# fishaudio/fish-diffusion

Measured on NVIDIA H100. Metric: mel_frames_per_sec_100step_ddpm, higher is better.
Workload: dtype f32 (3x fp16 split-product wgmma, fp32 accumulate)

## Files before the change

### fish_diffusion_b200/_native.py

```python
from __future__ import annotations

import ctypes
import os
import threading
from ctypes import POINTER, c_char_p, c_float, c_int, c_longlong, c_size_t, c_ubyte, c_ulonglong, c_void_p

import torch

_HERE = os.path.dirname(os.path.abspath(__file__))
LIB_PATH = os.environ.get("FISHDIFF_B200_LIB") or os.path.join(_HERE, "libfishdiff_b200.so")

PREC_F16, PREC_BF16 = 0, 1
PREC_SINGLE = 0x10
BACKEND_TC, BACKEND_SIMT = 0, 1
ACT_NONE, ACT_RELU, ACT_LRELU = 0, 1, 2
ABI_VERSION = 3


class NativeError(RuntimeError):
    pass


class ConvDesc(ctypes.Structure):
    _fields_ = [
        ("in_planes", c_void_p), ("w_planes", c_void_p), ("bias", c_void_p), ("addend", c_void_p),
        ("res_f32", c_void_p), ("res_planes", c_void_p), ("row_mask", c_void_p), ("out_f32", c_void_p),
        ("out_planes", c_void_p),
        ("B", c_int), ("T", c_int), ("Cin", c_int), ("N", c_int), ("ntaps", c_int), ("shifts", c_int * 16),
        ("w_inv_scale", c_float), ("post_scale", c_float), ("planes_scale", c_float), ("act_slope", c_float),
        ("out_accum", c_int), ("act", c_int), ("prec", c_int), ("backend", c_int),
    ]


class GemmDesc(ctypes.Structure):
    _fields_ = [
        ("src", c_void_p * 2), ("src_C", c_int * 2), ("w", c_void_p), ("n_total", c_int), ("k_total", c_int),
        ("w_kshift", c_int), ("B", c_int), ("T", c_int), ("num_seg", c_int), ("seg_src", c_int * 16),
        ("seg_shift", c_int * 16), ("seg_coff", c_int * 16), ("seg_klen", c_int * 16),
        ("bias", c_void_p), ("addend", c_void_p), ("res_f32", c_void_p), ("res_planes", c_void_p),
        ("row_mask", c_void_p), ("out_f32", c_void_p), ("out_planes", c_void_p),
        ("w_inv_scale", c_float), ("res_scale", c_float), ("post_scale", c_float), ("planes_scale", c_float),
        ("act_slope", c_float), ("out_accum", c_int), ("act", c_int), ("prec", c_int), ("backend", c_int),
        ("bias_bstride", c_int),
        ("gate_y", c_void_p), ("gate_cs", c_void_p), ("gate_cs_edge", c_void_p), ("gate_cs_scale", c_float),
        ("gate_tile", c_int), ("gate_dil", c_int),
    ]


class ResPairDesc(ctypes.Structure):
    _fields_ = [
        ("in_planes", c_void_p), ("w1", c_void_p), ("w2", c_void_p), ("b1", c_void_p), ("b2", c_void_p),
        ("out_planes", c_void_p),
        ("B", c_int), ("T", c_int), ("C", c_int), ("k1", c_int), ("d1", c_int), ("k2", c_int),
        ("w1_inv_scale", c_float), ("w2_inv_scale", c_float), ("in_slope", c_float), ("out_slope", c_float),
        ("planes_scale", c_float), ("prec", c_int), ("kmask1", c_ulonglong), ("kmask2", c_ulonglong),
    ]


class WaveNetFwdDesc(ctypes.Structure):
    _fields_ = [
        ("x_planes", c_void_p), ("cond_planes", c_void_p), ("steps", c_void_p), ("x_mask", c_void_p), ("out", c_void_p),
        ("w_in", c_void_p), ("b_in", c_void_p), ("w_in_inv", c_float),
        ("mlp_w0", c_void_p), ("mlp_b0", c_void_p), ("mlp_w1", c_void_p), ("mlp_b1", c_void_p),
        ("wd", c_void_p), ("bd", c_void_p), ("w1p_f32", c_void_p), ("bias_sum", c_void_p),
        ("w1", c_void_p), ("w1_lstride", c_longlong), ("w2", c_void_p), ("w2_lstride", c_longlong),
        ("b2", c_void_p), ("b2_lstride", c_longlong),
        ("w_skip", c_void_p), ("b_skip", c_void_p), ("w_skip_inv", c_float),
        ("w_out", c_void_p), ("b_out", c_void_p), ("w_out_inv", c_float),
        ("w1_inv", c_float * 64), ("w2_inv", c_float * 64), ("dilation", c_int * 64),
        ("xr", c_void_p), ("z", c_void_p), ("skip_planes", c_void_p), ("skip_f32", c_void_p),
        ("s", c_void_p), ("mlp_ws", c_void_p), ("gb", c_void_p), ("gb_ws", c_void_p),
        ("B", c_int), ("T", c_int), ("M", c_int), ("C", c_int), ("E", c_int), ("L", c_int), ("Bs", c_int),
        ("gate_tile", c_int), ("prec", c_int), ("backend", c_int),
        ("cond_proj", c_void_p),
    ]


class WaveNetBwdDesc(ctypes.Structure):
    _fields_ = [
        ("x_planes", c_void_p), ("y_planes", c_void_p), ("z_planes", c_void_p), ("cond_planes", c_void_p),
        ("dx_next", c_void_p), ("dskip", c_void_p), ("w2t", c_void_p), ("w1t", c_void_p), ("wct", c_void_p),
        ("w2t_inv", c_float), ("w1t_inv", c_float), ("wct_inv", c_float),
        ("dx_out", c_void_p), ("dx_f32", c_void_p), ("d_cond", c_void_p), ("gw1", c_void_p), ("gw2", c_void_p),
        ("cs_dy", c_void_p), ("cs_edge", c_void_p), ("cs_dx", c_void_p), ("dy", c_void_p),
        ("part1", c_void_p), ("part2", c_void_p), ("splits1", c_int), ("splits2", c_int),
        ("B", c_int), ("T", c_int), ("C", c_int), ("E", c_int), ("dilation", c_int), ("gate_tile", c_int),
        ("inv_S", c_float), ("prec", c_int), ("backend", c_int),
    ]


class WgradDesc(ctypes.Structure):
    _fields_ = [
        ("row_src", c_void_p * 2), ("row_C", c_int * 2), ("col_src", c_void_p * 2), ("col_C", c_int * 2),
        ("num_row_seg", c_int), ("row_seg_src", c_int * 2), ("row_seg_coff", c_int * 2), ("row_seg_width", c_int * 2),
        ("num_col_seg", c_int), ("col_seg_src", c_int * 8), ("col_seg_shift", c_int * 8), ("col_seg_coff", c_int * 8),
        ("col_seg_width", c_int * 8),
        ("B", c_int), ("T", c_int), ("splits", c_int), ("part", c_void_p), ("acc_scale", c_float), ("prec", c_int),
        ("backend", c_int),
    ]


_SIGS = {
    "fd_gemm_cl_fwd": (c_int, [POINTER(GemmDesc), c_void_p]),
    "fd_wavenet_pack_layers": (c_int, [c_void_p] * 10 + [c_int, c_int, c_int, c_int, c_int, c_void_p]),
    "fd_wgrad_cl": (c_int, [POINTER(WgradDesc), c_void_p]),
    "fd_wavenet_block_bwd": (c_int, [POINTER(WaveNetBwdDesc), c_void_p]),
    "fd_wavenet_block_fwd_train": (c_int, [c_void_p] * 10 + [c_int, c_void_p, c_void_p, c_void_p, c_float] +
                                   [c_int] * 6 + [c_float, c_float, c_int, c_int, c_int, c_void_p]),
    "fd_wavenet_gate_bias_from_d": (c_int, [c_void_p] * 6 + [c_int, c_int, c_int, c_int, c_void_p]),
    "fd_relu_bwd": (c_int, [c_void_p] * 3 + [c_longlong, c_float, c_int, c_void_p]),
    "fd_lrelu_bwd": (c_int, [c_void_p] * 5 + [c_longlong, c_float, c_float, c_int, c_void_p]),
    "fd_colsum": (c_int, [c_void_p] * 3 + [c_int, c_int, c_int, c_float, c_int, c_void_p]),
    "fd_reduce_batch": (c_int, [c_void_p, c_void_p, c_int, c_longlong, c_float, c_void_p]),
    "fd_abi_version": (c_int, []),
    "fd_last_error": (c_char_p, []),
    "fd_set_device": (None, [c_int]),
    "fd_launch_count": (c_longlong, []),
    "fd_tc_supported_linear": (c_int, [c_int, c_int, c_int]),
    "fd_prof_enable": (None, [c_int]),
    "fd_prof_collect": (c_int, [POINTER(ctypes.c_double), POINTER(c_longlong), c_int]),
    "fd_split_ncw": (c_int, [c_void_p, c_void_p, c_void_p, c_int, c_int, c_int, c_int, c_void_p]),
    "fd_split_nwc": (c_int, [c_void_p, c_void_p, c_void_p, c_int, c_int, c_int, c_float, c_int, c_void_p]),
    "fd_mrf_finish": (c_int, [POINTER(c_void_p), c_int, c_void_p, c_longlong, c_float, c_float, c_float, c_int, c_void_p]),
    "fd_transpose_nwc_to_ncw": (c_int, [c_void_p, c_void_p, c_int, c_int, c_int, c_void_p]),
    "fd_transpose_ncw_to_nwc": (c_int, [c_void_p, c_void_p, c_int, c_int, c_int, c_void_p]),
    "fd_pack_weight": (c_int, [c_void_p, c_void_p, c_longlong, c_float, c_int, c_void_p]),
    "fd_wavenet_step_mlp": (c_int, [c_void_p] * 7 + [c_int, c_int, c_void_p]),
    "fd_wavenet_gate_bias": (c_int, [c_void_p] * 9 + [c_int, c_int, c_int, c_int, c_void_p]),
    "fd_wavenet_block_fwd": (c_int, [c_void_p] * 8 + [c_int, c_void_p, c_void_p, c_void_p, c_float] + [c_int] * 6 +
                             [c_float, c_float, c_int, c_int, c_int, c_void_p]),
    "fd_wavenet_fwd": (c_int, [POINTER(WaveNetFwdDesc), c_void_p]),
    "fd_wavenet_cond_proj": (c_int, [POINTER(WaveNetFwdDesc), c_void_p]),
    "fd_conv_cl_fwd": (c_int, [POINTER(ConvDesc), c_void_p]),
    "fd_respair_supported": (c_int, [c_int, c_int, c_int, c_int]),
    "fd_respair_fwd": (c_int, [POINTER(ResPairDesc), c_void_p]),
    "fd_ddpm_step": (c_int, [c_void_p] * 5 + [c_longlong] + [c_float] * 7 + [c_ulonglong, c_ulonglong, c_ulonglong, c_int,
                                                                               c_void_p]),
    "fd_lincomb": (c_int, [c_void_p, c_void_p, POINTER(c_void_p), POINTER(c_float), c_int, c_longlong, c_int, c_void_p]),
    "fd_affine_cl": (c_int, [c_void_p] * 4 + [c_int, c_longlong, c_int, c_void_p]),
    "fd_q_sample": (c_int, [c_void_p] * 5 + [c_int, c_longlong, c_void_p]),
    "fd_randn": (c_int, [c_void_p, c_longlong, c_ulonglong, c_ulonglong, c_ulonglong, c_void_p]),
    "fd_sinegen_ws_bytes": (c_size_t, [c_int, c_longlong]),
    "fd_sinegen_fwd": (c_int, [c_void_p] * 7 + [c_int, c_int, c_int, c_int, c_float, c_float, c_float, c_ulonglong,
                                                c_void_p]),
    "fd_source_conv_fwd": (c_int, [c_void_p] * 4 + [c_int, c_longlong, c_int, c_int, c_int, c_int, c_void_p]),
    "fd_conv_post_fwd": (c_int, [c_void_p] * 4 + [c_int, c_longlong, c_int, c_int, c_int, c_void_p]),
    "fd_reflect_pad_split": (c_int, [c_void_p, c_void_p, c_int, c_longlong, c_int, c_int, c_void_p]),
    "fd_stft_mag_fwd": (c_int, [c_void_p] * 3 + [c_int, c_longlong, c_int, c_int, c_int, c_int, c_float, c_float, c_int,
                                                 c_int, c_void_p]),
    "fd_stft_mag_eps_fwd": (c_int, [c_void_p] * 3 + [c_int, c_longlong, c_int, c_int, c_int, c_int, c_float, c_float, c_float,
                                                     c_int, c_int, c_void_p]),
    "fd_log_clamp": (c_int, [c_void_p, c_void_p, c_longlong, c_float, c_float, c_void_p]),
    "fd_resample_out_len": (c_longlong, [c_longlong, c_int, c_int]),
    "fd_resample_fwd": (c_int, [c_void_p] * 6 + [c_int, c_longlong, c_longlong, c_int, c_int, c_int, c_int, c_void_p]),
}

EXPORTS = tuple(_SIGS)
_lib = None


def lib():
    global _lib
    if _lib is None:
        if not os.path.exists(LIB_PATH):
            raise NativeError(
                f"{LIB_PATH} not found: build it with `python -c 'import __graft_entry__ as g; g.build()'` "
                "(nvcc, sm_90a).  fish_diffusion_b200 has no CPU or PyTorch fallback.")
        l = ctypes.CDLL(LIB_PATH)
        for name, (res, args) in _SIGS.items():
            fn = getattr(l, name)
            fn.restype = res
            fn.argtypes = args
        if l.fd_abi_version() != ABI_VERSION:
            raise NativeError(f"ABI mismatch: library {l.fd_abi_version()} != binding {ABI_VERSION}")
        _lib = l
    return _lib


def last_error() -> str:
    return (lib().fd_last_error() or b"").decode("utf-8", "replace")


def check(rc: int, what: str):
    if rc != 0:
        raise NativeError(f"{what} failed (rc={rc}): {last_error()}")


def ptr(t):
    if t is None:
        return None
    assert t.is_contiguous(), "native kernels need contiguous tensors"
    return t.data_ptr()


_tls = threading.local()


def stream_ptr(device=None):
    if device is None or getattr(device, "index", None) is None:
        idx = torch.cuda.current_device()
    else:
        idx = device.index
    if getattr(_tls, "dev", None) != idx:
        lib().fd_set_device(idx)
        _tls.dev = idx
    return torch.cuda.current_stream(idx).cuda_stream


def require_cuda(t, name="tensor"):
    if not t.is_cuda:
        raise NativeError(f"{name} is on {t.device}: fish_diffusion_b200 runs on CUDA (sm_90a) only, there is no CPU path")


def launch_count() -> int:
    return int(lib().fd_launch_count())


def prec_code(precision: str) -> int:
    p = precision.lower()
    if p.endswith("x1"):
        p = p[:-2]
    if p in ("f16", "fp16", "half"):
        return PREC_F16
    if p in ("bf16", "bfloat16"):
        return PREC_BF16
    raise ValueError(f"unknown precision {precision!r} (use 'f16', 'bf16', 'f16x1' or 'bf16x1')")

# ... 200 lines not shown
```

### fish_diffusion_b200/csrc/fd_api.cu

```cuda
#include <atomic>
#include <cstdarg>
#include <cstdio>
#include <cmath>
#include <cstring>
#include "fd_common.cuh"
#include "fd_host.h"

namespace {
thread_local char g_err[1024] = "";
std::atomic<long long> g_launches{0};

void set_prec(FdTapGemm& p, int prec) { p.prec = prec & 0xF; p.single = (prec & FD_SINGLE) ? 1 : 0; }
void init_desc(FdTapGemm& p) { memset(&p, 0, sizeof(p)); p.acc_scale = 1.f; p.post_scale = 1.f; p.planes_scale = 1.f; p.res_scale = 1.f; }

void set_src(FdTapGemm& p, int i, const uint16_t* ptr, int C) {
  p.src[i] = ptr;
  p.src_C[i] = C;
  p.src_rs[i] = C;
  p.src_bs[i] = (long long)p.T * C;
  p.src_ps[i] = (long long)p.B * p.T * C;
}

constexpr int PROF_MAX = 1 << 16;
bool g_prof_on = false;
int g_prof_n = 0;
cudaEvent_t* g_prof_ev = nullptr;
int g_prof_kind[PROF_MAX];

}

void fd_prof_begin(int kind, cudaStream_t st) {
  if (!g_prof_on || g_prof_n >= PROF_MAX) return;
  if (g_prof_ev == nullptr) {
    g_prof_ev = new cudaEvent_t[2 * PROF_MAX];
    for (int i = 0; i < 2 * PROF_MAX; ++i) g_prof_ev[i] = nullptr;
  }
  if (g_prof_ev[2 * g_prof_n] == nullptr) {
    cudaEventCreate(&g_prof_ev[2 * g_prof_n]);
    cudaEventCreate(&g_prof_ev[2 * g_prof_n + 1]);
  }
  g_prof_kind[g_prof_n] = kind;
  cudaEventRecord(g_prof_ev[2 * g_prof_n], st);
}
void fd_prof_end(cudaStream_t st) {
  if (!g_prof_on || g_prof_n >= PROF_MAX) return;
  cudaEventRecord(g_prof_ev[2 * g_prof_n + 1], st);
  ++g_prof_n;
}

namespace {

int run(const FdTapGemm& p, int backend, cudaStream_t st) {
  int rc;
  fd_prof_begin(p.epi * 2 + (backend == FD_BACKEND_TC ? 0 : 1), st);
  if (backend == FD_BACKEND_TC) {
    rc = fd_tapgemm_tc_launch(p, st);
  } else if (backend == FD_BACKEND_SIMT) {
    rc = fd_tapgemm_simt_launch(p, st);
  } else {
    fd_set_error("unknown backend %d", backend);
    return -2;
  }
  fd_prof_end(st);
  if (rc == 0) fd_count_launch(1);
  return rc;
}
}

void fd_count_launch(int n) { g_launches.fetch_add(n, std::memory_order_relaxed); }

namespace { thread_local int g_target_dev = -1; int g_sms[FD_MAX_DEVICES] = {0}; }

FdDeviceGuard::FdDeviceGuard() {
  if (g_target_dev < 0) return;
  if (cudaGetDevice(&prev) != cudaSuccess) { prev = -1; return; }
  if (prev != g_target_dev && cudaSetDevice(g_target_dev) == cudaSuccess) switched = true;
}
FdDeviceGuard::~FdDeviceGuard() {
  if (switched) cudaSetDevice(prev);
}
int fd_current_device() {
  int dev = 0;
  if (cudaGetDevice(&dev) != cudaSuccess || dev < 0 || dev >= FD_MAX_DEVICES) dev = 0;
  return dev;
}
int fd_device_sms(int dev) {
  if (g_sms[dev] == 0) {
    int n = 0;
    if (cudaDeviceGetAttribute(&n, cudaDevAttrMultiProcessorCount, dev) != cudaSuccess || n <= 0) n = 132;
    g_sms[dev] = n;
  }
  return g_sms[dev];
}

extern "C" {

void fd_set_error(const char* fmt, ...) {
  va_list ap;
  va_start(ap, fmt);
  vsnprintf(g_err, sizeof(g_err), fmt, ap);
  va_end(ap);
}

const char* fd_last_error(void) { return g_err; }
void fd_set_device(int device) { g_target_dev = (device >= 0 && device < FD_MAX_DEVICES) ? device : -1; }
int fd_abi_version(void) { return FD_ABI_VERSION; }
long long fd_launch_count(void) { return g_launches.load(std::memory_order_relaxed); }

void fd_prof_enable(int on) {
  g_prof_on = on != 0;
  g_prof_n = 0;
}

int fd_prof_collect(double* ms_sum, long long* count, int nkinds) {
  FD_CHECK_CUDA(cudaDeviceSynchronize());
  for (int k = 0; k < nkinds; ++k) { ms_sum[k] = 0.0; count[k] = 0; }
  for (int i = 0; i < g_prof_n; ++i) {
    float ms = 0.f;
    FD_CHECK_CUDA(cudaEventElapsedTime(&ms, g_prof_ev[2 * i], g_prof_ev[2 * i + 1]));
    const int k = g_prof_kind[i];
    if (k < nkinds) { ms_sum[k] += ms; count[k] += 1; }
  }
  const int n = g_prof_n;
  g_prof_n = 0;
  return n >= PROF_MAX ? 1 : 0;
}

int fd_tc_supported_linear(int n_total, int k_seg, int num_seg) {
  FdTapGemm p;
  init_desc(p);
  p.B = 1; p.T = 128; p.n_total = n_total; p.num_seg = num_seg; p.k_total = k_seg * num_seg;
  p.epi = FD_EPI_LINEAR;
  if (num_seg < 1 || num_seg > FD_MAX_SEG) return 0;
  for (int s = 0; s < num_seg; ++s) { p.seg[s].src = 0; p.seg[s].k_len = k_seg; }
  set_src(p, 0, reinterpret_cast<const uint16_t*>(16), k_seg);
  return fd_tapgemm_tc_supported(p);
}

static int wavenet_block(const uint16_t* x_planes, uint16_t* x_out_planes, const uint16_t* cond_planes,
                         const float* cond_proj, uint16_t* z_planes, uint16_t* y_planes, const uint16_t* w1,
                         const uint16_t* w2,
                         const float* gb_full, const float* gb_lo, const float* gb_hi, int gb_bstride, const float* b2,
                         float* skip_f32, uint16_t* skip_planes, float skip_scale, int B, int T, int C, int E,
                         int dilation, int gate_tile, float w1_inv_scale, float w2_inv_scale, int flags, int prec,
                         int backend, void* stream);

int fd_wavenet_block_fwd(uint16_t* x_planes, const uint16_t* cond_planes, uint16_t* z_planes, const uint16_t* w1,
                         const uint16_t* w2, const float* gb_full, const float* gb_lo, const float* gb_hi,
                         int gb_bstride, const float* b2, float* skip_f32, uint16_t* skip_planes, float skip_scale,
                         int B, int T, int C, int E, int dilation, int gate_tile, float w1_inv_scale,
                         float w2_inv_scale, int flags, int prec, int backend, void* stream) {
  FD_DEVICE_GUARD();
  return wavenet_block(x_planes, nullptr, cond_planes, nullptr, z_planes, nullptr, w1, w2, gb_full, gb_lo, gb_hi, gb_bstride, b2,
                       skip_f32, skip_planes, skip_scale, B, T, C, E, dilation, gate_tile, w1_inv_scale, w2_inv_scale,
                       flags, prec, backend, stream);
}

int fd_wavenet_block_fwd_train(const uint16_t* x_planes, uint16_t* x_out_planes, const uint16_t* cond_planes,
                               uint16_t* z_planes, uint16_t* y_planes, const uint16_t* w1, const uint16_t* w2,
                               const float* gb_full, const float* gb_lo, const float* gb_hi, int gb_bstride,
                               const float* b2, float* skip_f32, uint16_t* skip_planes, float skip_scale, int B, int T,
                               int C, int E, int dilation, int gate_tile, float w1_inv_scale, float w2_inv_scale,
                               int flags, int prec, int backend, void* stream) {
  FD_DEVICE_GUARD();
  FD_REQUIRE(x_out_planes != nullptr && y_planes != nullptr, "fd_wavenet_block_fwd_train: x_out / y planes required");
  return wavenet_block(x_planes, x_out_planes, cond_planes, nullptr, z_planes, y_planes, w1, w2, gb_full, gb_lo, gb_hi,
                       gb_bstride, b2, skip_f32, skip_planes, skip_scale, B, T, C, E, dilation, gate_tile, w1_inv_scale,
                       w2_inv_scale, flags, prec, backend, stream);
}

static int wavenet_block(const uint16_t* x_planes, uint16_t* x_out_planes, const uint16_t* cond_planes,
                         const float* cond_proj, uint16_t* z_planes, uint16_t* y_planes, const uint16_t* w1,
                         const uint16_t* w2,
                         const float* gb_full, const float* gb_lo, const float* gb_hi, int gb_bstride, const float* b2,
                         float* skip_f32, uint16_t* skip_planes, float skip_scale, int B, int T, int C, int E,
                         int dilation, int gate_tile, float w1_inv_scale, float w2_inv_scale, int flags, int prec,
                         int backend, void* stream) {
  FD_REQUIRE(B > 0 && T > 0 && C > 0 && E > 0 && dilation > 0, "fd_wavenet_block_fwd: bad shape");
  FD_REQUIRE(C % 8 == 0 && E % 8 == 0, "fd_wavenet_block_fwd: C=%d, E=%d must be multiples of 8", C, E);
  cudaStream_t st = (cudaStream_t)stream;
  FdTapGemm p;
  init_desc(p);
  p.B = B; p.T = T; set_prec(p, prec);
  p.n_total = 2 * C; p.k_total = 3 * C + E; p.num_seg = cond_proj != nullptr ? 3 : 4;
  p.seg[0] = FdSeg{0, -dilation, 0, C};
  p.seg[1] = FdSeg{0, 0, 0, C};
  p.seg[2] = FdSeg{0, dilation, 0, C};
  p.seg[3] = FdSeg{1, 0, 0, E};
  set_src(p, 0, x_planes, C);
  if (cond_proj == nullptr) set_src(p, 1, cond_planes, E);
  p.addend = cond_proj;
  p.w = w1; p.acc_scale = w1_inv_scale;
  p.epi = FD_EPI_GATE;
  p.gbias_full = gb_full; p.gbias_lo = gb_lo; p.gbias_hi = gb_hi; p.gbias_bstride = gb_bstride;
  p.dil = dilation; p.gate_tile = gate_tile; p.C = C;
  p.out_planes = z_planes;
  p.y_planes = y_planes;
  int rc = run(p, backend, st);
  if (rc) return rc;
  FdTapGemm q;
  init_desc(q);
  q.B = B; q.T = T; set_prec(q, prec);
  q.n_total = 2 * C; q.k_total = C; q.num_seg = 1;
  q.seg[0] = FdSeg{0, 0, 0, C};
  set_src(q, 0, z_planes, C);
  q.w = w2; q.acc_scale = w2_inv_scale;
  q.epi = FD_EPI_RES_SKIP;
  q.bias = b2; q.bias_bstride = 0;
  q.x_planes = const_cast<uint16_t*>(x_planes); q.x_out_planes = x_out_planes; q.skip_f32 = skip_f32; q.skip_planes = skip_planes; q.skip_scale = skip_scale;
  q.first_layer = flags & 1; q.last_layer = (flags >> 1) & 1; q.C = C;
  return run(q, backend, st);
}

int fd_wavenet_fwd(const fd_wavenet_fwd_desc* d, void* stream) {
  FD_DEVICE_GUARD();
  FD_REQUIRE(d != nullptr, "fd_wavenet_fwd: null descriptor");
  FD_REQUIRE(d->L >= 1 && d->L <= 64, "fd_wavenet_fwd: L=%d out of range (1..64)", d->L);
  FD_REQUIRE(d->Bs == 1 || d->Bs == d->B, "fd_wavenet_fwd: Bs=%d must be 1 or B=%d", d->Bs, d->B);
  const int B = d->B, T = d->T, M = d->M, C = d->C, E = d->E, L = d->L, Bs = d->Bs;
  int rc = fd_wavenet_step_mlp(d->steps, d->mlp_w0, d->mlp_b0, d->mlp_w1, d->mlp_b1, d->s, d->mlp_ws, Bs, C, stream);
  if (rc) return rc;
  float* gb_full = d->gb;
  float* gb_lo = d->gb + (size_t)L * Bs * 2 * C;
  float* gb_hi = d->gb + (size_t)2 * L * Bs * 2 * C;
  rc = fd_wavenet_gate_bias(d->s, d->wd, d->bd, d->w1p_f32, d->bias_sum, gb_full, gb_lo, gb_hi, d->gb_ws, L, Bs, C,
                            3 * C + E, stream);
  if (rc) return rc;
  fd_conv_desc cd;
  memset(&cd, 0, sizeof(cd));
  cd.B = B; cd.T = T; cd.ntaps = 1; cd.shifts[0] = 0;
  cd.post_scale = 1.f; cd.planes_scale = 1.f; cd.prec = d->prec; cd.backend = d->backend;
  cd.in_planes = d->x_planes; cd.w_planes = d->w_in; cd.bias = d->b_in; cd.row_mask = d->x_mask;
  cd.out_planes = d->xr; cd.Cin = M; cd.N = C; cd.w_inv_scale = d->w_in_inv; cd.act = 1;
  rc = fd_conv_cl_fwd(&cd, stream);
  if (rc) return rc;
  const int gb_stride = Bs > 1 ? 2 * C : 0;
  const float skip_scale = 1.f / sqrtf((float)L);
  for (int l = 0; l < L; ++l) {
    const int flags = (l == 0 ? 1 : 0) | (l == L - 1 ? 2 : 0);
    const size_t go = (size_t)l * Bs * 2 * C;
    const float* cp = d->cond_proj != nullptr ? d->cond_proj + (size_t)l * B * T * 2 * C : nullptr;
    rc = wavenet_block(d->xr, nullptr, d->cond_planes, cp, d->z, nullptr, d->w1 + (size_t)l * d->w1_lstride,
                       d->w2 + (size_t)l * d->w2_lstride, gb_full + go, gb_lo + go, gb_hi + go, gb_stride,
                       d->b2 + (size_t)l * d->b2_lstride, d->skip_f32, d->skip_planes, skip_scale, B, T, C, E,
                       d->dilation[l], d->gate_tile, d->w1_inv[l], d->w2_inv[l], flags, d->prec, d->backend, stream);
    if (rc) return rc;
  }
  cd.in_planes = d->skip_planes; cd.w_planes = d->w_skip; cd.bias = d->b_skip; cd.row_mask = nullptr;
  cd.out_planes = d->z; cd.out_f32 = nullptr; cd.Cin = C; cd.N = C; cd.w_inv_scale = d->w_skip_inv; cd.act = 1;
  rc = fd_conv_cl_fwd(&cd, stream);
  if (rc) return rc;
  cd.in_planes = d->z; cd.w_planes = d->w_out; cd.bias = d->b_out; cd.row_mask = d->x_mask;
  cd.out_planes = nullptr; cd.out_f32 = d->out; cd.Cin = C; cd.N = M; cd.w_inv_scale = d->w_out_inv; cd.act = 0;
  return fd_conv_cl_fwd(&cd, stream);
}

int fd_wavenet_cond_proj(const fd_wavenet_fwd_desc* d, void* stream) {
  FD_DEVICE_GUARD();
  FD_REQUIRE(d != nullptr, "fd_wavenet_cond_proj: null descriptor");
  FD_REQUIRE(d->cond_proj != nullptr && d->cond_planes != nullptr && d->w1 != nullptr,
             "fd_wavenet_cond_proj: cond_proj, cond_planes and w1 are required");
  FD_REQUIRE(d->L >= 1 && d->L <= 64, "fd_wavenet_cond_proj: L=%d out of range (1..64)", d->L);
  FD_REQUIRE(d->B > 0 && d->T > 0 && d->C > 0 && d->E > 0, "fd_wavenet_cond_proj: bad shape");
  FD_REQUIRE(d->C % 8 == 0 && d->E % 8 == 0, "fd_wavenet_cond_proj: C=%d, E=%d must be multiples of 8", d->C, d->E);
  const int B = d->B, T = d->T, C = d->C, E = d->E;
  FD_REQUIRE((long long)B * T * 2 * C < (1ll << 32),
             "fd_wavenet_cond_proj: B*T*2C = %lld exceeds the 32-bit element offsets of the epilogue",
             (long long)B * T * 2 * C);
  FdTapGemm p;
  init_desc(p);
  p.B = B; p.T = T; set_prec(p, d->prec);
  p.n_total = 2 * C; p.k_total = 3 * C + E; p.num_seg = 1;
  p.seg[0] = FdSeg{0, 0, 0, E};
  set_src(p, 0, d->cond_planes, E);
  p.w_kshift = 3 * C;
  p.epi = FD_EPI_LINEAR;
  for (int l = 0; l < d->L; ++l) {
    p.w = d->w1 + (size_t)l * d->w1_lstride;
    p.acc_scale = d->w1_inv[l];
    p.out_f32 = d->cond_proj + (size_t)l * B * T * 2 * C;
    const int rc = run(p, d->backend, (cudaStream_t)stream);
    if (rc) return rc;
  }
  return 0;
}

int fd_conv_cl_fwd(const fd_conv_desc* d, void* stream) {
  FD_DEVICE_GUARD();
  FD_REQUIRE(d != nullptr, "fd_conv_cl_fwd: null descriptor");
  FD_REQUIRE(d->ntaps >= 1 && d->ntaps <= FD_MAX_SEG, "fd_conv_cl_fwd: ntaps=%d out of range", d->ntaps);
  FD_REQUIRE(d->B > 0 && d->T > 0 && d->Cin > 0 && d->N > 0, "fd_conv_cl_fwd: bad shape");
  FdTapGemm p;
  init_desc(p);
  p.B = d->B; p.T = d->T; set_prec(p, d->prec);
  p.n_total = d->N; p.k_total = d->ntaps * d->Cin; p.num_seg = d->ntaps;
  for (int j = 0; j < d->ntaps; ++j) p.seg[j] = FdSeg{0, d->shifts[j], 0, d->Cin};
  set_src(p, 0, d->in_planes, d->Cin);
  p.w = d->w_planes; p.acc_scale = d->w_inv_scale;
  p.epi = FD_EPI_LINEAR;
  p.bias = d->bias; p.bias_bstride = 0;
  p.addend = d->addend; p.res_f32 = d->res_f32; p.res_planes = d->res_planes;
  p.post_scale = d->post_scale; p.out_f32 = d->out_f32; p.out_accum = d->out_accum;
  p.out_planes = d->out_planes; p.planes_scale = d->planes_scale; p.act = d->act; p.act_slope = d->act_slope;
  p.row_mask = d->row_mask;
  return run(p, d->backend, (cudaStream_t)stream);
}

int fd_stft_mag_eps_fwd(const uint16_t* padded, const uint16_t* dft_w, uint16_t* mag_planes, int B, long long Np,
                    int n_fft, int hop, int frames, int NB, float w_inv_scale, float mag_scale, float mag_eps, int prec,
                    int backend, void* stream) {
  FD_DEVICE_GUARD();
  FD_REQUIRE(n_fft % 64 == 0 && hop % 8 == 0 && NB % 128 == 0, "fd_stft_mag_fwd: n_fft=%d hop=%d NB=%d unsupported",
             n_fft, hop, NB);
  const long long pitch = (Np + 7) / 8 * 8;
  FD_REQUIRE((long long)(frames - 1) * hop + n_fft <= Np, "fd_stft_mag_fwd: frames exceed the padded signal");
  FdTapGemm p;
  init_desc(p);
  p.B = B; p.T = frames; set_prec(p, prec);
  p.n_total = 2 * NB; p.k_total = n_fft; p.num_seg = 1;
  p.seg[0] = FdSeg{0, 0, 0, n_fft};
  p.src[0] = padded; p.src_C[0] = n_fft;
  p.src_rs[0] = hop; p.src_bs[0] = pitch; p.src_ps[0] = (long long)B * pitch;
  p.w = dft_w; p.acc_scale = w_inv_scale;
  p.epi = FD_EPI_MAG; p.gate_tile = 256; p.C = NB; p.mag_scale = mag_scale; p.mag_eps = mag_eps;
  p.out_planes = mag_planes;
  return run(p, backend, (cudaStream_t)stream);
}

int fd_stft_mag_fwd(const uint16_t* padded, const uint16_t* dft_w, uint16_t* mag_planes, int B, long long Np,
                    int n_fft, int hop, int frames, int NB, float w_inv_scale, float mag_scale, int prec,
                    int backend, void* stream) {
  return fd_stft_mag_eps_fwd(padded, dft_w, mag_planes, B, Np, n_fft, hop, frames, NB, w_inv_scale, mag_scale, 1e-9f, prec,
                             backend, stream);
}

int fd_gemm_cl_fwd(const fd_gemm_desc* d, void* stream) {
  FD_DEVICE_GUARD();
  FD_REQUIRE(d != nullptr, "fd_gemm_cl_fwd: null descriptor");
  FD_REQUIRE(d->num_seg >= 1 && d->num_seg <= FD_MAX_SEG, "fd_gemm_cl_fwd: num_seg=%d out of range", d->num_seg);
  FD_REQUIRE(d->B > 0 && d->T > 0 && d->n_total > 0 && d->k_total > 0, "fd_gemm_cl_fwd: bad shape");
  FdTapGemm p;
  init_desc(p);
  p.B = d->B; p.T = d->T; set_prec(p, d->prec);
  p.n_total = d->n_total; p.k_total = d->k_total; p.num_seg = d->num_seg;
  for (int j = 0; j < d->num_seg; ++j) {
    FD_REQUIRE(d->seg_src[j] == 0 || d->seg_src[j] == 1, "fd_gemm_cl_fwd: segment %d has bad source", j);
    p.seg[j] = FdSeg{d->seg_src[j], d->seg_shift[j], d->seg_coff[j], d->seg_klen[j]};
  }
  for (int i = 0; i < 2; ++i)
    if (d->src[i] != nullptr) set_src(p, i, d->src[i], d->src_C[i]);
  FD_REQUIRE(p.src[0] != nullptr, "fd_gemm_cl_fwd: src[0] is null");
  int k_sum = 0;
  for (int j = 0; j < d->num_seg; ++j) k_sum += d->seg_klen[j];
  FD_REQUIRE(d->w_kshift >= 0 && d->w_kshift + k_sum <= d->k_total,
             "fd_gemm_cl_fwd: w_kshift=%d + K=%d exceeds the W row pitch k_total=%d", d->w_kshift, k_sum, d->k_total);
  p.w = d->w; p.acc_scale = d->w_inv_scale; p.w_kshift = d->w_kshift;
  p.epi = FD_EPI_LINEAR;
  p.bias = d->bias; p.bias_bstride = d->bias_bstride;
  if (d->gate_y != nullptr) {
    FD_REQUIRE(d->out_planes != nullptr && d->gate_tile > 0 && d->gate_tile % 8 == 0 && d->n_total % 4 == 0 &&
                   d->n_total % (d->gate_tile / 2) == 0,
               "fd_gemm_cl_fwd: gate backward needs out_planes and a gate tile (n_total=%d, gate_tile=%d)", d->n_total,
               d->gate_tile);
  }
  p.addend = d->addend; p.res_f32 = d->res_f32; p.res_planes = d->res_planes; p.res_scale = d->res_scale;
  p.post_scale = d->post_scale; p.out_f32 = d->out_f32; p.out_accum = d->out_accum;
  p.out_planes = d->out_planes; p.planes_scale = d->planes_scale; p.act = d->act; p.act_slope = d->act_slope;
  p.row_mask = d->row_mask;
  if (d->gate_y != nullptr) {
    p.epi = FD_EPI_GATE_BWD;
    p.y_planes = const_cast<uint16_t*>(d->gate_y); p.gate_tile = d->gate_tile; p.dil = d->gate_dil; p.C = d->n_total;
    p.cs = d->gate_cs; p.cs_edge = d->gate_cs_edge; p.cs_scale = d->gate_cs_scale;
  }
  return run(p, d->backend, (cudaStream_t)stream);
}

}
```

### fish_diffusion_b200/csrc/fd_common.cuh

```cuda
#pragma once
#include <cuda_runtime.h>
#include <cuda_fp16.h>
#include <cuda_bf16.h>
#include <stdint.h>

#define FD_F16 0
#define FD_BF16 1
#define FD_SINGLE 0x10

#define FD_MAX_SEG 16

#define FD_EPI_LINEAR 0
#define FD_EPI_GATE 1
#define FD_EPI_RES_SKIP 2
#define FD_EPI_MAG 3
#define FD_EPI_GATE_BWD 4

#define FD_ACT_NONE 0
#define FD_ACT_RELU 1
#define FD_ACT_LRELU 2

struct FdSeg {
  int src;
  int shift;
  int c_off;
  int k_len;
};

struct FdTapGemm {
  int B, T;
  int n_total;
  int k_total;
  int num_seg;
  int prec;
  int single;
  FdSeg seg[FD_MAX_SEG];
  const uint16_t* src[2];
  int src_C[2];
  long long src_rs[2], src_bs[2], src_ps[2];
  const uint16_t* w;
  float acc_scale;
  int w_kshift;
  int epi;

  const float* bias;
  int bias_bstride;
  const float* addend;
  const float* res_f32;
  const uint16_t* res_planes;
  float res_scale;
  float post_scale;
  float* out_f32;
  int out_accum;
  uint16_t* out_planes;
  float planes_scale;
  int act;
  float act_slope;
  const uint8_t* row_mask;

  const float* gbias_full;
  const float* gbias_lo;
  const float* gbias_hi;
  int gbias_bstride;
  int dil;
  int gate_tile;

  float mag_scale;
  float mag_eps;

  uint16_t* x_planes;
  uint16_t* x_out_planes;
  uint16_t* y_planes;
  float* skip_f32;
  uint16_t* skip_planes;
  float skip_scale;
  int first_layer, last_layer;
  int C;

  float* cs;
  float* cs_edge;
  float cs_scale;
};

#define FD_WGRAD_MAX_COL_SEG 8
struct FdWgradK {
  int B, T, R, Cc;
  int splits, items_per_split;
  int m_tiles, n_tiles;
  int num_row_seg, num_col_seg;
  int row_src[2], row_coff[2], row_start[2], row_width[2];
  int col_src[FD_WGRAD_MAX_COL_SEG], col_shift[FD_WGRAD_MAX_COL_SEG], col_coff[FD_WGRAD_MAX_COL_SEG],
      col_start[FD_WGRAD_MAX_COL_SEG], col_width[FD_WGRAD_MAX_COL_SEG];
  int row_C[2], col_C[2];
  float* part;
  float acc_scale;
};

__device__ __forceinline__ void fd_split(float v, int prec, uint16_t& hi, uint16_t& lo) {
  if (prec == FD_F16) {
    v = fminf(fmaxf(v, -65504.f), 65504.f);
    __half h = __float2half_rn(v);
    __half l = __float2half_rn(v - __half2float(h));
    hi = __half_as_ushort(h);
    lo = __half_as_ushort(l);
  } else {
    __nv_bfloat16 h = __float2bfloat16_rn(v);
    __nv_bfloat16 l = __float2bfloat16_rn(v - __bfloat162float(h));
    hi = __bfloat16_as_ushort(h);
    lo = __bfloat16_as_ushort(l);
  }
}

__device__ __forceinline__ float fd_h2f(uint16_t u, int prec) {
  if (prec == FD_F16) return __half2float(__ushort_as_half(u));
  return __uint_as_float(((uint32_t)u) << 16);
}

__device__ __forceinline__ float fd_combine(uint16_t hi, uint16_t lo, int prec) {
  return fd_h2f(hi, prec) + fd_h2f(lo, prec);
}

__device__ __forceinline__ void fd_combine2(uint32_t hi2, uint32_t lo2, int prec, float& a, float& b) {
  if (prec == FD_F16) {
    const float2 h = __half22float2(*reinterpret_cast<const __half2*>(&hi2));
    const float2 l = __half22float2(*reinterpret_cast<const __half2*>(&lo2));
    a = h.x + l.x; b = h.y + l.y;
  } else {
    a = __uint_as_float(hi2 << 16) + __uint_as_float(lo2 << 16);
    b = __uint_as_float(hi2 & 0xffff0000u) + __uint_as_float(lo2 & 0xffff0000u);
  }
}

__device__ __forceinline__ float fd_act(float w, float slope) { return fmaf(slope, fminf(w, 0.f), fmaxf(w, 0.f)); }

__device__ __forceinline__ float fd_sigmoid(float x) { return __fdividef(1.f, 1.f + __expf(-x)); }
__device__ __forceinline__ float fd_tanh(float x) {
  float ax = fabsf(x);
  if (ax < 0.04f) { float x2 = x * x; return x * (1.f - x2 * (0.33333333f - 0.13333333f * x2)); }
  float e = __expf(2.f * ax);
  float r = 1.f - __fdividef(2.f, e + 1.f);
  return copysignf(r, x);
}

__device__ __forceinline__ void fd_dgate(float dz, float g, float f, float& dg, float& df) {
  const float sg = fd_sigmoid(g), th = fd_tanh(f);
  dg = dz * th * sg * (1.f - sg);
  df = dz * sg * (1.f - th * th);
}

template <int V> struct FdVec16;
template <> struct FdVec16<4> { uint2 v; };
template <> struct FdVec16<8> { uint4 v; };

__device__ __forceinline__ void fd_split2(float a, float b, int prec, uint32_t& hi2, uint32_t& lo2) {
  if (prec == FD_F16) {
    asm("cvt.rn.satfinite.f16x2.f32 %0, %1, %2;" : "=r"(hi2) : "f"(b), "f"(a));
    const float2 hf = __half22float2(*reinterpret_cast<const __half2*>(&hi2));
    asm("cvt.rn.satfinite.f16x2.f32 %0, %1, %2;" : "=r"(lo2) : "f"(b - hf.y), "f"(a - hf.x));
  } else {
    asm("cvt.rn.satfinite.bf16x2.f32 %0, %1, %2;" : "=r"(hi2) : "f"(b), "f"(a));
    const float ha = __uint_as_float(hi2 << 16), hb = __uint_as_float(hi2 & 0xffff0000u);
    asm("cvt.rn.satfinite.bf16x2.f32 %0, %1, %2;" : "=r"(lo2) : "f"(b - hb), "f"(a - ha));
  }
}

template <int V>
__device__ __forceinline__ void fd_store_planes(uint16_t* planes, size_t plane_elems, size_t off,
                                                const float (&y)[V], int prec) {
  uint32_t hi[V / 2], lo[V / 2];
#pragma unroll
  for (int i = 0; i < V / 2; ++i) fd_split2(y[2 * i], y[2 * i + 1], prec, hi[i], lo[i]);
  if (V == 4) {
    *reinterpret_cast<uint2*>(planes + off) = make_uint2(hi[0], hi[1]);
    *reinterpret_cast<uint2*>(planes + plane_elems + off) = make_uint2(lo[0], lo[1]);
  } else {
    *reinterpret_cast<uint4*>(planes + off) = make_uint4(hi[0], hi[1], hi[2 % (V / 2)], hi[3 % (V / 2)]);
    *reinterpret_cast<uint4*>(planes + plane_elems + off) = make_uint4(lo[0], lo[1], lo[2 % (V / 2)], lo[3 % (V / 2)]);
  }
}

template <int V>
__device__ __forceinline__ void fd_load_planes(const uint16_t* planes, size_t plane_elems, size_t off,
                                               float (&y)[V], int prec) {
  uint16_t hi[8], lo[8];
  if (V == 4) {
    uint2 a = *reinterpret_cast<const uint2*>(planes + off);
    uint2 b = *reinterpret_cast<const uint2*>(planes + plane_elems + off);
    hi[0] = a.x & 0xffff; hi[1] = a.x >> 16; hi[2] = a.y & 0xffff; hi[3] = a.y >> 16;
    lo[0] = b.x & 0xffff; lo[1] = b.x >> 16; lo[2] = b.y & 0xffff; lo[3] = b.y >> 16;
  } else {
    uint4 a = *reinterpret_cast<const uint4*>(planes + off);
    uint4 b = *reinterpret_cast<const uint4*>(planes + plane_elems + off);
    hi[0] = a.x & 0xffff; hi[1] = a.x >> 16; hi[2] = a.y & 0xffff; hi[3] = a.y >> 16;
    hi[4] = a.z & 0xffff; hi[5] = a.z >> 16; hi[6] = a.w & 0xffff; hi[7] = a.w >> 16;
    lo[0] = b.x & 0xffff; lo[1] = b.x >> 16; lo[2] = b.y & 0xffff; lo[3] = b.y >> 16;
    lo[4] = b.z & 0xffff; lo[5] = b.z >> 16; lo[6] = b.w & 0xffff; lo[7] = b.w >> 16;
  }
#pragma unroll
  for (int i = 0; i < V; ++i) y[i] = fd_combine(hi[i], lo[i], prec);
}

__device__ __forceinline__ void fd_load_hi8(const uint16_t* planes, size_t off, float (&y)[8], int prec) {
  const uint4 a = *reinterpret_cast<const uint4*>(planes + off);
  const uint32_t w[4] = {a.x, a.y, a.z, a.w};
#pragma unroll
  for (int i = 0; i < 4; ++i) {
    y[2 * i] = fd_h2f((uint16_t)(w[i] & 0xffff), prec);
    y[2 * i + 1] = fd_h2f((uint16_t)(w[i] >> 16), prec);
  }
}

__device__ __forceinline__ void fd_unpack8(const uint4& a, const uint4& b, int prec, float (&y)[8]) {
  const uint32_t ha[4] = {a.x, a.y, a.z, a.w}, lb[4] = {b.x, b.y, b.z, b.w};
#pragma unroll
  for (int i = 0; i < 4; ++i) {
    y[2 * i] = fd_combine((uint16_t)(ha[i] & 0xffff), (uint16_t)(lb[i] & 0xffff), prec);
    y[2 * i + 1] = fd_combine((uint16_t)(ha[i] >> 16), (uint16_t)(lb[i] >> 16), prec);
  }
}
__device__ __forceinline__ void fd_pack8(const float (&y)[8], int prec, uint4& a, uint4& b) {
  uint16_t hi[8], lo[8];
#pragma unroll
  for (int i = 0; i < 8; ++i) fd_split(y[i], prec, hi[i], lo[i]);
  a.x = hi[0] | ((uint32_t)hi[1] << 16); a.y = hi[2] | ((uint32_t)hi[3] << 16);
  a.z = hi[4] | ((uint32_t)hi[5] << 16); a.w = hi[6] | ((uint32_t)hi[7] << 16);
  b.x = lo[0] | ((uint32_t)lo[1] << 16); b.y = lo[2] | ((uint32_t)lo[3] << 16);
  b.z = lo[4] | ((uint32_t)lo[5] << 16); b.w = lo[6] | ((uint32_t)lo[7] << 16);
}

template <int V>
__device__ __forceinline__ void fd_load_f32(const float* p, float (&y)[V]) {
#pragma unroll
  for (int i = 0; i < V; i += 4) {
    float4 q = *reinterpret_cast<const float4*>(p + i);
    y[i] = q.x; y[i + 1] = q.y; y[i + 2] = q.z; y[i + 3] = q.w;
  }
}
template <int V>
__device__ __forceinline__ void fd_store_f32(float* p, const float (&y)[V]) {
#pragma unroll
  for (int i = 0; i < V; i += 4)
    *reinterpret_cast<float4*>(p + i) = make_float4(y[i], y[i + 1], y[i + 2], y[i + 3]);
}

template <int V, int PREC = -1>
__device__ __forceinline__ void fd_epi_linear(const FdTapGemm& p, int b, int t, int n0,
                                              const float (&acc)[V], const float* bias_tile ,
                                              int tile_n0) {
  const int prec = PREC < 0 ? p.prec : PREC;
  const size_t row = (size_t)b * p.T + t;
  const size_t off = row * p.n_total + n0;
  const size_t plane_elems = (size_t)p.B * p.T * p.n_total;
  float y[V];
  const bool masked = p.row_mask != nullptr && p.row_mask[row] != 0;
#pragma unroll
  for (int i = 0; i < V; ++i) y[i] = acc[i] * p.acc_scale;
  if (bias_tile != nullptr) {
#pragma unroll
    for (int i = 0; i < V; ++i) y[i] += bias_tile[n0 - tile_n0 + i];
  }
  if (p.addend != nullptr) {
    float a[V]; fd_load_f32<V>(p.addend + off, a);
#pragma unroll
    for (int i = 0; i < V; ++i) y[i] += a[i];
  }
  if (p.res_f32 != nullptr) {
    float a[V]; fd_load_f32<V>(p.res_f32 + off, a);
#pragma unroll
    for (int i = 0; i < V; ++i) y[i] += a[i];
  }
  if (p.res_planes != nullptr) {
    float a[V]; fd_load_planes<V>(p.res_planes, plane_elems, off, a, prec);
#pragma unroll
    for (int i = 0; i < V; ++i) y[i] += a[i] * p.res_scale;
  }
#pragma unroll
  for (int i = 0; i < V; ++i) y[i] *= p.post_scale;
  if (p.out_f32 != nullptr) {
    if (p.out_accum) {
      float a[V]; fd_load_f32<V>(p.out_f32 + off, a);
#pragma unroll
      for (int i = 0; i < V; ++i) y[i] += a[i];
    }
    if (masked) {
#pragma unroll
      for (int i = 0; i < V; ++i) y[i] = 0.f;
    }
    fd_store_f32<V>(p.out_f32 + off, y);
  }
  if (p.out_planes != nullptr) {
#pragma unroll
    for (int i = 0; i < V; ++i) {
      float v = y[i] * p.planes_scale;
      if (p.act == FD_ACT_RELU) v = fmaxf(v, 0.f);
      else if (p.act == FD_ACT_LRELU) v = v > 0.f ? v : v * p.act_slope;
      y[i] = masked ? 0.f : v;
    }
    fd_store_planes<V>(p.out_planes, plane_elems, off, y, prec);
  }
}

template <int V, int PREC = -1>
__device__ __forceinline__ void fd_epi_gate(const FdTapGemm& p, int b, int t, int zc0, int n_g, int n_f,
                                            const float (&g)[V], const float (&f)[V],
                                            const float* full_g, const float* full_f,
                                            const float* lo_g, const float* lo_f,
                                            const float* hi_g, const float* hi_f) {
  const int prec = PREC < 0 ? p.prec : PREC;
  float z[V], yg8[V], yf8[V], ag[V], af[V];
  const bool e_lo = t < p.dil, e_hi = t + p.dil >= p.T;
  if (p.addend != nullptr) {
    const size_t arow = ((size_t)b * p.T + t) * p.n_total;
    fd_load_f32<V>(p.addend + arow + n_g, ag);
    fd_load_f32<V>(p.addend + arow + n_f, af);
  }
#pragma unroll
  for (int i = 0; i < V; ++i) {
    float yg = g[i] * p.acc_scale + full_g[i];
    float yf = f[i] * p.acc_scale + full_f[i];
    if (p.addend != nullptr) { yg += ag[i]; yf += af[i]; }
    if (e_lo) { yg -= lo_g[i]; yf -= lo_f[i]; }
    if (e_hi) { yg -= hi_g[i]; yf -= hi_f[i]; }
    yg8[i] = yg; yf8[i] = yf;
    z[i] = fd_sigmoid(yg) * fd_tanh(yf);
  }
  if (p.y_planes != nullptr) {
    const int half = p.gate_tile / 2;
    const int ng = (zc0 / half) * p.gate_tile + (zc0 % half);
    const size_t yplane = (size_t)p.B * p.T * p.n_total;
    const size_t yoff = ((size_t)b * p.T + t) * p.n_total;
    fd_store_planes<V>(p.y_planes, yplane, yoff + ng, yg8, prec);
    fd_store_planes<V>(p.y_planes, yplane, yoff + ng + half, yf8, prec);
  }
  const size_t plane_elems = (size_t)p.B * p.T * p.C;
  const size_t off = ((size_t)b * p.T + t) * p.C + zc0;
  fd_store_planes<V>(p.out_planes, plane_elems, off, z, prec);
}

template <int V, int PREC = -1>
__device__ __forceinline__ void fd_epi_mag(const FdTapGemm& p, int b, int t, int zc0,
                                           const float (&re)[V], const float (&im)[V]) {
  const int prec = PREC < 0 ? p.prec : PREC;
  float z[V];
#pragma unroll
  for (int i = 0; i < V; ++i) {
    const float r = re[i] * p.acc_scale, q = im[i] * p.acc_scale;
    z[i] = sqrtf(r * r + q * q + p.mag_eps) * p.mag_scale;
  }
  const size_t plane_elems = (size_t)p.B * p.T * p.C;
  const size_t off = ((size_t)b * p.T + t) * p.C + zc0;
  fd_store_planes<V>(p.out_planes, plane_elems, off, z, prec);
}

template <int V, int PREC = -1>
__device__ __forceinline__ void fd_epi_res_skip(const FdTapGemm& p, int b, int t, int n0,
                                                const float (&acc)[V], const float* bias ) {
  const int prec = PREC < 0 ? p.prec : PREC;
  const size_t row = (size_t)b * p.T + t;
  const size_t plane_elems = (size_t)p.B * p.T * p.C;
  float y[V];
#pragma unroll
  for (int i = 0; i < V; ++i) y[i] = acc[i] * p.acc_scale + bias[i];
  if (n0 < p.C) {
    if (p.last_layer) return;
    const size_t off = row * p.C + n0;
    float x[V];
    fd_load_planes<V>(p.x_planes, plane_elems, off, x, prec);
#pragma unroll
    for (int i = 0; i < V; ++i) x[i] = (x[i] + y[i]) * 0.70710678118654752440f;
    fd_store_planes<V>(p.x_out_planes != nullptr ? p.x_out_planes : p.x_planes, plane_elems, off, x, prec);
  } else {
    const size_t off = row * p.C + (n0 - p.C);
    if (!p.first_layer) {
      float s[V]; fd_load_f32<V>(p.skip_f32 + off, s);
#pragma unroll
      for (int i = 0; i < V; ++i) y[i] += s[i];
    }
    if (p.last_layer) {
#pragma unroll
      for (int i = 0; i < V; ++i) y[i] *= p.skip_scale;
      fd_store_planes<V>(p.skip_planes, plane_elems, off, y, prec);
    } else {
      fd_store_f32<V>(p.skip_f32 + off, y);
    }
  }
}

#ifdef __cplusplus
extern "C" {
#endif
void fd_set_error(const char* fmt, ...);
#ifdef __cplusplus
}
#endif

#define FD_CHECK_CUDA(expr)                                                                    \
  do {                                                                                         \
    cudaError_t _e = (expr);                                                                   \
    if (_e != cudaSuccess) {                                                                   \
      fd_set_error("%s:%d CUDA error %d (%s) in %s", __FILE__, __LINE__, (int)_e,              \
                   cudaGetErrorString(_e), #expr);                                             \
      return -1;                                                                               \
    }                                                                                          \
  } while (0)

#define FD_REQUIRE(cond, ...)                                                                  \
  do {                                                                                         \
    if (!(cond)) {                                                                             \
      fd_set_error(__VA_ARGS__);                                                               \
      return -2;                                                                               \
    }                                                                                          \
  } while (0)

int fd_tapgemm_simt_launch(const FdTapGemm& p, cudaStream_t stream);
int fd_tapgemm_tc_launch(const FdTapGemm& p, cudaStream_t stream);
int fd_tapgemm_tc_supported(const FdTapGemm& p);
int fd_wgrad_simt_launch(const FdWgradK& p, const uint16_t* const* row_ptr, const uint16_t* const* col_ptr, int prec,
                         cudaStream_t stream);
```

### fish_diffusion_b200/csrc/fd_tapgemm_simt.cu

```cuda
#include "fd_common.cuh"

namespace {

constexpr int BM = 128;
constexpr int BK = 16;
constexpr int APITCH = BM + 4;

template <int RUN, int EPI>
__global__ void __launch_bounds__(256) fd_tapgemm_simt_kernel(const FdTapGemm p) {
  constexpr int BN = 2 * RUN;
  constexpr int TXC = RUN / 4;
  constexpr int TYC = 256 / TXC;
  constexpr int RM = BM / TYC;
  constexpr int BPITCH = BN + 4;

  __shared__ float As[BK][APITCH];
  __shared__ float Bs[BK][BPITCH];

  const int tid = threadIdx.x;
  const int tx = tid % TXC, ty = tid / TXC;
  const int tiles_t = (p.T + BM - 1) / BM;
  const int m_tile = blockIdx.x;
  const int b = m_tile / tiles_t;
  const int t0 = (m_tile % tiles_t) * BM;
  const int j = blockIdx.y;

  int run0, run1;
  if (EPI == FD_EPI_GATE || EPI == FD_EPI_MAG) {
    const int half = p.gate_tile / 2;
    const int zc0 = j * RUN;
    run0 = (zc0 / half) * p.gate_tile + (zc0 % half);
    run1 = run0 + half;
  } else {
    run0 = j * BN;
    run1 = run0 + RUN;
  }

  float acc[RM][8];
#pragma unroll
  for (int r = 0; r < RM; ++r)
#pragma unroll
    for (int c = 0; c < 8; ++c) acc[r][c] = 0.f;

  const size_t w_plane = (size_t)p.n_total * p.k_total;
  int koff = 0;
  for (int s = 0; s < p.num_seg; ++s) {
    const FdSeg sg = p.seg[s];
    const uint16_t* src = p.src[sg.src];
    const size_t a_plane = (size_t)p.src_ps[sg.src];
    const size_t a_rs = (size_t)p.src_rs[sg.src], a_bs = (size_t)p.src_bs[sg.src];
    for (int k0 = 0; k0 < sg.k_len; k0 += BK) {
      {
        const int row = tid % BM, kh = tid / BM;
        const int t = t0 + row + sg.shift;
        float v[8];
        const int kk = k0 + kh * 8;
        if (t >= 0 && t < p.T && t0 + row < p.T && kk < sg.k_len) {
          const size_t off = (size_t)b * a_bs + (size_t)t * a_rs + sg.c_off + kk;
          if (p.single) fd_load_hi8(src, off, v, p.prec);
          else fd_load_planes<8>(src, a_plane, off, v, p.prec);
        } else {
#pragma unroll
          for (int i = 0; i < 8; ++i) v[i] = 0.f;
        }
#pragma unroll
        for (int i = 0; i < 8; ++i) As[kh * 8 + i][row] = v[i];
      }
      if (tid < BN * 2) {
        const int nl = tid % BN, kh = tid / BN;
        const int n = nl < RUN ? run0 + nl : run1 + (nl - RUN);
        const int kk = k0 + kh * 8;
        float v[8];
        if (n < p.n_total && kk < sg.k_len) {
          const size_t off = (size_t)n * p.k_total + koff + kk + p.w_kshift;
          if (p.single) fd_load_hi8(p.w, off, v, p.prec);
          else fd_load_planes<8>(p.w, w_plane, off, v, p.prec);
        } else {
#pragma unroll
          for (int i = 0; i < 8; ++i) v[i] = 0.f;
        }
#pragma unroll
        for (int i = 0; i < 8; ++i) Bs[kh * 8 + i][nl] = v[i];
      }
      __syncthreads();
#pragma unroll
      for (int k = 0; k < BK; ++k) {
        float a[RM], bv[8];
#pragma unroll
        for (int r = 0; r < RM; ++r) a[r] = As[k][ty * RM + r];
        float4 b0 = *reinterpret_cast<const float4*>(&Bs[k][tx * 4]);
        float4 b1 = *reinterpret_cast<const float4*>(&Bs[k][RUN + tx * 4]);
        bv[0] = b0.x; bv[1] = b0.y; bv[2] = b0.z; bv[3] = b0.w;
        bv[4] = b1.x; bv[5] = b1.y; bv[6] = b1.z; bv[7] = b1.w;
#pragma unroll
        for (int r = 0; r < RM; ++r)
#pragma unroll
          for (int c = 0; c < 8; ++c) acc[r][c] = fmaf(a[r], bv[c], acc[r][c]);
      }
      __syncthreads();
    }
    koff += sg.k_len;
  }

  if constexpr (EPI == FD_EPI_GATE_BWD) {
    const int half = p.gate_tile / 2;
    const size_t W2 = 2 * (size_t)p.C, plane = (size_t)p.B * p.T * W2;
    const bool edge0 = t0 < p.dil, edge1 = t0 + BM + p.dil > p.T;
#pragma unroll
    for (int h = 0; h < 2; ++h) {
      const int n = (h == 0 ? run0 : run1) + tx * 4;
      const int pg = (n / half) * p.gate_tile + n % half;
      float cs[8] = {}, e0[8] = {}, e1[8] = {};
#pragma unroll
      for (int r = 0; r < RM; ++r) {
        const int t = t0 + ty * RM + r;
        if (t >= p.T || n >= p.n_total) continue;
        const size_t off = ((size_t)b * p.T + t) * W2 + pg;
        float g[4], f[4], dg[4], df[4];
        fd_load_planes<4>(p.y_planes, plane, off, g, p.prec);
        fd_load_planes<4>(p.y_planes, plane, off + half, f, p.prec);
#pragma unroll
        for (int i = 0; i < 4; ++i) fd_dgate(acc[r][4 * h + i] * p.acc_scale, g[i], f[i], dg[i], df[i]);
        fd_store_planes<4>(p.out_planes, plane, off, dg, p.prec);
        fd_store_planes<4>(p.out_planes, plane, off + half, df, p.prec);
#pragma unroll
        for (int i = 0; i < 4; ++i) {
          cs[i] += dg[i]; cs[4 + i] += df[i];
          if (t < p.dil) { e0[i] += dg[i]; e0[4 + i] += df[i]; }
          if (t + p.dil >= p.T) { e1[i] += dg[i]; e1[4 + i] += df[i]; }
        }
      }
#pragma unroll
      for (int o = TXC; o < 32; o *= 2)
#pragma unroll
        for (int i = 0; i < 8; ++i) {
          cs[i] += __shfl_xor_sync(0xffffffffu, cs[i], o);
          if (edge0) e0[i] += __shfl_xor_sync(0xffffffffu, e0[i], o);
          if (edge1) e1[i] += __shfl_xor_sync(0xffffffffu, e1[i], o);
        }
      if (tid % 32 >= TXC || n >= p.n_total) continue;
      const size_t co = (size_t)b * W2 + pg;
#pragma unroll
      for (int i = 0; i < 8; ++i) {
        const size_t c = co + (i < 4 ? i : half + i - 4);
        if (p.cs != nullptr) atomicAdd(p.cs + c, cs[i] * p.cs_scale);
        if (p.cs_edge != nullptr && edge0) atomicAdd(p.cs_edge + c, e0[i] * p.cs_scale);
        if (p.cs_edge != nullptr && edge1) atomicAdd(p.cs_edge + (size_t)p.B * W2 + c, e1[i] * p.cs_scale);
      }
    }
  } else {
#pragma unroll
    for (int r = 0; r < RM; ++r) {
      const int t = t0 + ty * RM + r;
      if (t >= p.T) continue;
      float v0[4] = {acc[r][0], acc[r][1], acc[r][2], acc[r][3]};
      float v1[4] = {acc[r][4], acc[r][5], acc[r][6], acc[r][7]};
      const int n_a = run0 + tx * 4, n_b = run1 + tx * 4;
      if (EPI == FD_EPI_LINEAR) {
        const float* bias = p.bias ? p.bias + (size_t)b * p.bias_bstride : nullptr;
        if (n_a < p.n_total) fd_epi_linear<4>(p, b, t, n_a, v0, bias, 0);
        if (n_b < p.n_total) fd_epi_linear<4>(p, b, t, n_b, v1, bias, 0);
      } else if (EPI == FD_EPI_GATE) {
        if (n_a < p.n_total) {
          const size_t bo = (size_t)b * p.gbias_bstride;
          fd_epi_gate<4>(p, b, t, j * RUN + tx * 4, n_a, n_b, v0, v1,
                         p.gbias_full + bo + n_a, p.gbias_full + bo + n_b,
                         p.gbias_lo + bo + n_a, p.gbias_lo + bo + n_b,
                         p.gbias_hi + bo + n_a, p.gbias_hi + bo + n_b);
        }
      } else if (EPI == FD_EPI_MAG) {
        if (n_a < p.n_total) fd_epi_mag<4>(p, b, t, j * RUN + tx * 4, v0, v1);
      } else {
        const float* bias = p.bias + (size_t)b * p.bias_bstride;
        if (n_a < p.n_total) fd_epi_res_skip<4>(p, b, t, n_a, v0, bias + n_a);
        if (n_b < p.n_total) fd_epi_res_skip<4>(p, b, t, n_b, v1, bias + n_b);
      }
    }
  }
}

template <int RUN>
int launch_run(const FdTapGemm& p, cudaStream_t stream) {
  const int tiles_t = (p.T + BM - 1) / BM;
  dim3 grid(p.B * tiles_t, 1, 1), block(256);
  if (p.epi == FD_EPI_GATE) {
    grid.y = (p.n_total / 2 + RUN - 1) / RUN;
    fd_tapgemm_simt_kernel<RUN, FD_EPI_GATE><<<grid, block, 0, stream>>>(p);
  } else if (p.epi == FD_EPI_MAG) {
    grid.y = (p.n_total / 2 + RUN - 1) / RUN;
    fd_tapgemm_simt_kernel<RUN, FD_EPI_MAG><<<grid, block, 0, stream>>>(p);
  } else if (p.epi == FD_EPI_RES_SKIP) {
    grid.y = (p.n_total + 2 * RUN - 1) / (2 * RUN);
    fd_tapgemm_simt_kernel<RUN, FD_EPI_RES_SKIP><<<grid, block, 0, stream>>>(p);
  } else if (p.epi == FD_EPI_GATE_BWD) {
    grid.y = (p.n_total + 2 * RUN - 1) / (2 * RUN);
    fd_tapgemm_simt_kernel<RUN, FD_EPI_GATE_BWD><<<grid, block, 0, stream>>>(p);
  } else {
    grid.y = (p.n_total + 2 * RUN - 1) / (2 * RUN);
    fd_tapgemm_simt_kernel<RUN, FD_EPI_LINEAR><<<grid, block, 0, stream>>>(p);
  }
  FD_CHECK_CUDA(cudaGetLastError());
  return 0;
}

constexpr int WG_R = 64, WG_C = 64, WG_T = 16;

__global__ void __launch_bounds__(256) fd_wgrad_simt_kernel(const FdWgradK p, const uint16_t* row0,
                                                            const uint16_t* row1, const uint16_t* col0,
                                                            const uint16_t* col1, int prec, int single) {
  static_assert(WG_R == WG_C, "rows and columns share the staging code");
  __shared__ __align__(16) float Rs[WG_T][WG_R + 4];
  __shared__ __align__(16) float Cs[WG_T][WG_C + 4];
  const int tid = threadIdx.x;
  const int s = blockIdx.z, r0 = blockIdx.y * WG_R, c0 = blockIdx.x * WG_C;

  const bool is_col = tid >= 128;
  const int grp = tid % 8, tl = (tid % 128) / 8;
  const int i = (is_col ? c0 : r0) + grp * 8;
  const uint16_t* src = nullptr;
  int C = 0, ch = 0, shift = 0;
  if (!is_col) {
    for (int g = 0; g < p.num_row_seg; ++g)
      if (i >= p.row_start[g] && i < p.row_start[g] + p.row_width[g]) {
        src = p.row_src[g] == 0 ? row0 : row1;
        C = p.row_C[p.row_src[g]]; ch = p.row_coff[g] + (i - p.row_start[g]);
      }
  } else {
    for (int g = 0; g < p.num_col_seg; ++g)
      if (i >= p.col_start[g] && i < p.col_start[g] + p.col_width[g]) {
        src = p.col_src[g] == 0 ? col0 : col1;
        C = p.col_C[p.col_src[g]]; ch = p.col_coff[g] + (i - p.col_start[g]); shift = p.col_shift[g];
      }
  }
  const size_t plane = (size_t)p.B * p.T * C;
  float* const dst = is_col ? &Cs[tl][grp * 8] : &Rs[tl][grp * 8];

  const int tx = tid % 16, ty = tid / 16;
  float acc[4][4];
#pragma unroll
  for (int r = 0; r < 4; ++r)
#pragma unroll
    for (int c = 0; c < 4; ++c) acc[r][c] = 0.f;

  const int b_end = min(p.B, (s + 1) * p.items_per_split);
  for (int b = s * p.items_per_split; b < b_end; ++b) {
    for (int t0 = 0; t0 < p.T; t0 += WG_T) {
      const int t = t0 + tl, ts = t + shift;
      float v[8];
      if (src != nullptr && t < p.T && ts >= 0 && ts < p.T) {
        const size_t off = ((size_t)b * p.T + ts) * C + ch;
        if (single) fd_load_hi8(src, off, v, prec);
        else fd_load_planes<8>(src, plane, off, v, prec);
      } else {
#pragma unroll
        for (int k = 0; k < 8; ++k) v[k] = 0.f;
      }
      *reinterpret_cast<float4*>(dst) = make_float4(v[0], v[1], v[2], v[3]);
      *reinterpret_cast<float4*>(dst + 4) = make_float4(v[4], v[5], v[6], v[7]);
      __syncthreads();
#pragma unroll
      for (int k = 0; k < WG_T; ++k) {
        const float4 a = *reinterpret_cast<const float4*>(&Rs[k][ty * 4]);
        const float4 c = *reinterpret_cast<const float4*>(&Cs[k][tx * 4]);
        const float av[4] = {a.x, a.y, a.z, a.w}, cv[4] = {c.x, c.y, c.z, c.w};
#pragma unroll
        for (int r = 0; r < 4; ++r)
#pragma unroll
          for (int cc = 0; cc < 4; ++cc) acc[r][cc] = fmaf(av[r], cv[cc], acc[r][cc]);
      }
      __syncthreads();
    }
  }

  const int col = c0 + tx * 4;
  if (col >= p.Cc) return;
  float* const out = p.part + (size_t)s * p.R * p.Cc;
#pragma unroll
  for (int r = 0; r < 4; ++r) {
    const int row = r0 + ty * 4 + r;
    if (row < p.R)
      *reinterpret_cast<float4*>(out + (size_t)row * p.Cc + col) = make_float4(
          acc[r][0] * p.acc_scale, acc[r][1] * p.acc_scale, acc[r][2] * p.acc_scale, acc[r][3] * p.acc_scale);
  }
}

}

int fd_tapgemm_simt_launch(const FdTapGemm& p, cudaStream_t stream) {
  FD_REQUIRE(p.n_total % 4 == 0, "tapgemm(simt): n_total=%d must be a multiple of 4", p.n_total);
  FD_REQUIRE(p.k_total % 8 == 0 && p.w_kshift % 8 == 0,
             "tapgemm(simt): k_total=%d and w_kshift=%d must be multiples of 8", p.k_total, p.w_kshift);
  for (int s = 0; s < p.num_seg; ++s) {
    FD_REQUIRE(p.seg[s].k_len % 8 == 0 && p.seg[s].c_off % 8 == 0 && p.src_rs[p.seg[s].src] % 8 == 0 &&
                   p.src_bs[p.seg[s].src] % 8 == 0 && p.src_ps[p.seg[s].src] % 8 == 0,
               "tapgemm(simt): segment %d needs k_len/c_off/strides multiples of 8", s);
  }
  if (p.epi == FD_EPI_GATE || p.epi == FD_EPI_MAG) {
    const int half = p.gate_tile / 2;
    FD_REQUIRE(half > 0 && p.n_total % p.gate_tile == 0, "tapgemm(simt): bad gate_tile %d", p.gate_tile);
    if (half % 64 == 0) return launch_run<64>(p, stream);
    FD_REQUIRE(half % 16 == 0, "tapgemm(simt): gate_tile/2=%d must be a multiple of 16", half);
    return launch_run<16>(p, stream);
  }
  if (p.epi == FD_EPI_RES_SKIP) {
    FD_REQUIRE(p.C % 4 == 0 && p.n_total == 2 * p.C, "tapgemm(simt): res/skip needs n_total == 2C");
  }
  if (p.n_total >= 96) return launch_run<64>(p, stream);
  return launch_run<16>(p, stream);
}

int fd_wgrad_simt_launch(const FdWgradK& p, const uint16_t* const* row_ptr, const uint16_t* const* col_ptr, int prec,
                         cudaStream_t stream) {
  dim3 grid((p.Cc + WG_C - 1) / WG_C, (p.R + WG_R - 1) / WG_R, p.splits);
  fd_wgrad_simt_kernel<<<grid, 256, 0, stream>>>(p, row_ptr[0], row_ptr[1], col_ptr[0], col_ptr[1], prec & 0xF,
                                                 (prec & FD_SINGLE) != 0);
  FD_CHECK_CUDA(cudaGetLastError());
  return 0;
}
```

### fish_diffusion_b200/csrc/fd_tapgemm_tc.cu

```cuda
#include <cuda.h>
#include "fd_common.cuh"
#include "fd_host.h"
#include "fd_tc_ptx.cuh"

namespace {

constexpr int BLOCK_M = 128;

constexpr int ring_stages(int stage_bytes, int bias_floats) {
  return fd_tc_ring_stages(1024  + bias_floats * 4 + 2 * FD_TC_MAX_STAGES * 8 + FD_TC_SCRATCH_BYTES,
                           stage_bytes);
}

template <int BLOCK_N, int BLOCK_K, int EPI, int NPL>
struct Cfg {
  static constexpr bool PP = EPI == FD_EPI_GATE || EPI == FD_EPI_RES_SKIP;
  static constexpr int ROWS = PP ? 64 : BLOCK_M;
  static constexpr int A_BYTES = ROWS * BLOCK_K * 2;
  static constexpr int W_BYTES = BLOCK_N * BLOCK_K * 2;
  static constexpr int GROUP = BLOCK_K >= 64 || PP ? 1 : 64 / BLOCK_K;
  static constexpr int SUB_BYTES = NPL * (A_BYTES + W_BYTES);
  static constexpr int STAGE_BYTES = GROUP * SUB_BYTES;
  static constexpr int TX_BYTES = SUB_BYTES;
  static constexpr int SWIZZLE_BYTES = BLOCK_K * 2;
  static constexpr uint32_t SWIZZLE_MODE = swizzle_mode_for(SWIZZLE_BYTES);
  static constexpr uint32_t SBO = 8 * SWIZZLE_BYTES;
  static constexpr int BIAS_FLOATS = (EPI == FD_EPI_GATE ? 3 : 1) * BLOCK_N;
  static constexpr int BIAS_TOTAL = (PP ? 2 : 1) * BIAS_FLOATS;
  static constexpr int NUM_STAGES = ring_stages(STAGE_BYTES, BIAS_TOTAL);
  static constexpr int SMEM_BYTES = 1024  + NUM_STAGES * STAGE_BYTES + BIAS_TOTAL * 4 +
                                    2 * NUM_STAGES * 8 + FD_TC_SCRATCH_BYTES;
  static_assert(NUM_STAGES >= 2, "pipeline needs at least two stages");
  static_assert(SMEM_BYTES <= FD_TC_SMEM_BUDGET, "shared memory");
};

template <int BLOCK_N, int EPI>
__device__ __forceinline__ void stage_bias(const FdTapGemm& p, int b, int n0, float* bias_s, int i0, int step) {
  if (EPI == FD_EPI_GATE) {
    const size_t bo = (size_t)b * p.gbias_bstride + n0;
    for (int i = i0; i < BLOCK_N; i += step) {
      bias_s[i] = p.gbias_full[bo + i];
      bias_s[BLOCK_N + i] = p.gbias_lo[bo + i];
      bias_s[2 * BLOCK_N + i] = p.gbias_hi[bo + i];
    }
  } else {
    for (int i = i0; i < BLOCK_N; i += step)
      bias_s[i] = p.bias ? p.bias[(size_t)b * p.bias_bstride + n0 + i] : 0.f;
  }
}
template <int EPI>
__device__ __forceinline__ long long bias_key(const FdTapGemm& p, int b, int n0) {
  return EPI == FD_EPI_GATE ? (long long)b * p.gbias_bstride + n0 : (long long)b * p.bias_bstride + n0;
}

template <int BLOCK_N, int EPI, int PREC>
__device__ __forceinline__ void tile_epilogue(const FdTapGemm& p, const float* acc, int b, int n_tile, int rw0,
                                              const float* bias_s, uint32_t my_scratch, int lane) {
  const int n0 = n_tile * BLOCK_N;
  if (EPI == FD_EPI_GATE || EPI == FD_EPI_MAG) {
    constexpr int HALF = BLOCK_N / 2;
    const uint32_t sb = smem_u32(bias_s);
    const int r = lane >> 1, sub = lane & 1;
    const int t = rw0 + r;
    const bool valid = t < p.T;
    const bool e_lo = t < p.dil, e_hi = t + p.dil >= p.T;
    const bool edge_any = __any_sync(0xffffffffu, valid && (e_lo || e_hi));
    const size_t zplane = (size_t)p.B * p.T * p.C, zrow = ((size_t)b * p.T + t) * p.C + (size_t)n_tile * HALF;
    const size_t yplane = (size_t)p.B * p.T * p.n_total, yrow = ((size_t)b * p.T + t) * p.n_total;
    const int halfg = p.gate_tile / 2;
#pragma unroll
    for (int c = 0; c < HALF; c += 16) {
      frag_to_scratch<16>(my_scratch, acc, c, 0, lane);
      frag_to_scratch<16>(my_scratch, acc, HALF + c, 16, lane);
      __syncwarp();
      float g[8], f[8];
      {
        const float4 g0 = scratch_ld4(my_scratch, r, 2 * sub), g1 = scratch_ld4(my_scratch, r, 2 * sub + 1);
        const float4 f0 = scratch_ld4(my_scratch, r, 4 + 2 * sub), f1 = scratch_ld4(my_scratch, r, 5 + 2 * sub);
        g[0] = g0.x; g[1] = g0.y; g[2] = g0.z; g[3] = g0.w; g[4] = g1.x; g[5] = g1.y; g[6] = g1.z; g[7] = g1.w;
        f[0] = f0.x; f[1] = f0.y; f[2] = f0.z; f[3] = f0.w; f[4] = f1.x; f[5] = f1.y; f[6] = f1.z; f[7] = f1.w;
      }
      __syncwarp();
      const int cc = c + 8 * sub;
      if (valid) {
        if (EPI == FD_EPI_MAG) {
          fd_epi_mag<8, PREC>(p, b, t, n_tile * HALF + cc, g, f);
        } else {
          float yg[8], yf[8], z[8];
          {
            float4 c0, c1, d0, d1;
            if (p.addend != nullptr) {
              const float* ad = p.addend + yrow + n0 + cc;
              c0 = __ldcs(reinterpret_cast<const float4*>(ad));
              c1 = __ldcs(reinterpret_cast<const float4*>(ad + 4));
              d0 = __ldcs(reinterpret_cast<const float4*>(ad + HALF));
              d1 = __ldcs(reinterpret_cast<const float4*>(ad + HALF + 4));
            }
            const float4 a0 = lds128(sb + 4u * cc), a1 = lds128(sb + 4u * cc + 16u);
            const float4 b0 = lds128(sb + 4u * (HALF + cc)), b1 = lds128(sb + 4u * (HALF + cc) + 16u);
            const float bg[8] = {a0.x, a0.y, a0.z, a0.w, a1.x, a1.y, a1.z, a1.w};
            const float bf[8] = {b0.x, b0.y, b0.z, b0.w, b1.x, b1.y, b1.z, b1.w};
#pragma unroll
            for (int i = 0; i < 8; ++i) {
              yg[i] = g[i] * p.acc_scale + bg[i];
              yf[i] = f[i] * p.acc_scale + bf[i];
            }
            if (p.addend != nullptr) {
              const float cg[8] = {c0.x, c0.y, c0.z, c0.w, c1.x, c1.y, c1.z, c1.w};
              const float cf[8] = {d0.x, d0.y, d0.z, d0.w, d1.x, d1.y, d1.z, d1.w};
#pragma unroll
              for (int i = 0; i < 8; ++i) { yg[i] += cg[i]; yf[i] += cf[i]; }
            }
          }
          if (edge_any) {
#pragma unroll
            for (int e = 0; e < 2; ++e) {
              if (e == 0 ? e_lo : e_hi) {
                const uint32_t eb = sb + 4u * ((1 + e) * BLOCK_N + cc);
                const float4 a0 = lds128(eb), a1 = lds128(eb + 16u);
                const float4 b0 = lds128(eb + 4u * HALF), b1 = lds128(eb + 4u * HALF + 16u);
                const float eg[8] = {a0.x, a0.y, a0.z, a0.w, a1.x, a1.y, a1.z, a1.w};
                const float ef[8] = {b0.x, b0.y, b0.z, b0.w, b1.x, b1.y, b1.z, b1.w};
#pragma unroll
                for (int i = 0; i < 8; ++i) { yg[i] -= eg[i]; yf[i] -= ef[i]; }
              }
            }
          }
#pragma unroll
          for (int i = 0; i < 8; ++i) z[i] = fd_sigmoid(yg[i]) * fd_tanh(yf[i]);
          if (p.y_planes != nullptr) {
            const int zc0 = n_tile * HALF + cc;
            const int ng = p.gate_tile == BLOCK_N ? n_tile * BLOCK_N + cc : (zc0 / halfg) * p.gate_tile + (zc0 % halfg);
            fd_store_planes<8>(p.y_planes, yplane, yrow + ng, yg, PREC);
            fd_store_planes<8>(p.y_planes, yplane, yrow + ng + halfg, yf, PREC);
          }
          fd_store_planes<8>(p.out_planes, zplane, zrow + cc, z, PREC);
        }
      }
    }
  } else if (BLOCK_N >= 64) {
    const uint32_t bias_addr = smem_u32(bias_s);
    const int j4 = (lane & 7) * 4, rsub = lane >> 3;
    const int rbase = rw0 + rsub;
    const int nrows = rbase < p.T ? min(4, (p.T - rbase + 3) / 4) : 0;
    const uint32_t rowbase = (uint32_t)b * (uint32_t)p.T;
#pragma unroll
    for (int c = 0; c < BLOCK_N; c += 32) {
      const int col = c + j4;
      const int n = n0 + col;
      frag_to_scratch<32>(my_scratch, acc, c, 0, lane);
      __syncwarp();
      float4 a[4];
#pragma unroll
      for (int pp = 0; pp < 4; ++pp) a[pp] = scratch_ld4(my_scratch, 4 * pp + rsub, lane & 7);
      __syncwarp();
      if (EPI == FD_EPI_GATE_BWD) {
        const int half_g = p.gate_tile / 2;
        const uint32_t pg = (uint32_t)((n / half_g) * p.gate_tile + (n % half_g));
        const uint32_t W2 = 2u * (uint32_t)p.C;
        const size_t yplane = (size_t)p.B * p.T * W2;
        const uint16_t* const y_lo = p.y_planes + yplane;
        uint16_t* const o_lo = p.out_planes + yplane;
        float sg4[4] = {0.f, 0.f, 0.f, 0.f}, sf4[4] = {0.f, 0.f, 0.f, 0.f};
        float e0g[4] = {0.f, 0.f, 0.f, 0.f}, e0f[4] = {0.f, 0.f, 0.f, 0.f}, e1g[4] = {0.f, 0.f, 0.f, 0.f}, e1f[4] = {0.f, 0.f, 0.f, 0.f};
        uint2 gh[4], gl[4], fh[4], fl[4];
        uint32_t eo4[4];
#pragma unroll
        for (int pp = 0; pp < 4; ++pp) {
          eo4[pp] = (rowbase + (uint32_t)min(rbase + pp * 4, p.T - 1)) * W2 + pg;
          gh[pp] = *reinterpret_cast<const uint2*>(p.y_planes + eo4[pp]);
          gl[pp] = *reinterpret_cast<const uint2*>(y_lo + eo4[pp]);
          fh[pp] = *reinterpret_cast<const uint2*>(p.y_planes + eo4[pp] + half_g);
          fl[pp] = *reinterpret_cast<const uint2*>(y_lo + eo4[pp] + half_g);
        }
#pragma unroll
        for (int pp = 0; pp < 4; ++pp) {
          if (pp >= nrows) break;
          float g[4], f[4];
          fd_combine2(gh[pp].x, gl[pp].x, PREC, g[0], g[1]);
          fd_combine2(gh[pp].y, gl[pp].y, PREC, g[2], g[3]);
          fd_combine2(fh[pp].x, fl[pp].x, PREC, f[0], f[1]);
          fd_combine2(fh[pp].y, fl[pp].y, PREC, f[2], f[3]);
          const float dzv[4] = {a[pp].x * p.acc_scale, a[pp].y * p.acc_scale, a[pp].z * p.acc_scale, a[pp].w * p.acc_scale};
          float dg[4], df[4];
#pragma unroll
          for (int i = 0; i < 4; ++i) fd_dgate(dzv[i], g[i], f[i], dg[i], df[i]);
          uint32_t h0, l0, h1, l1;
          fd_split2(dg[0], dg[1], PREC, h0, l0);
          fd_split2(dg[2], dg[3], PREC, h1, l1);
          *reinterpret_cast<uint2*>(p.out_planes + eo4[pp]) = make_uint2(h0, h1);
          *reinterpret_cast<uint2*>(o_lo + eo4[pp]) = make_uint2(l0, l1);
          fd_split2(df[0], df[1], PREC, h0, l0);
          fd_split2(df[2], df[3], PREC, h1, l1);
          *reinterpret_cast<uint2*>(p.out_planes + eo4[pp] + half_g) = make_uint2(h0, h1);
          *reinterpret_cast<uint2*>(o_lo + eo4[pp] + half_g) = make_uint2(l0, l1);
          if (p.cs != nullptr) {
            const int tt = rbase + pp * 4;
            const bool in0 = tt < p.dil, in1 = tt + p.dil >= p.T;
#pragma unroll
            for (int i = 0; i < 4; ++i) {
              sg4[i] += dg[i]; sf4[i] += df[i];
              if (in0) { e0g[i] += dg[i]; e0f[i] += df[i]; }
              if (in1) { e1g[i] += dg[i]; e1f[i] += df[i]; }
            }
          }
        }
        if (p.cs != nullptr) {
          const bool edge0 = rw0 < p.dil, edge1 = rw0 + 16 + p.dil > p.T;
#pragma unroll
          for (int i = 0; i < 4; ++i) {
            sg4[i] += __shfl_xor_sync(0xffffffffu, sg4[i], 8); sg4[i] += __shfl_xor_sync(0xffffffffu, sg4[i], 16);
            sf4[i] += __shfl_xor_sync(0xffffffffu, sf4[i], 8); sf4[i] += __shfl_xor_sync(0xffffffffu, sf4[i], 16);
            if (edge0) {
              e0g[i] += __shfl_xor_sync(0xffffffffu, e0g[i], 8); e0g[i] += __shfl_xor_sync(0xffffffffu, e0g[i], 16);
              e0f[i] += __shfl_xor_sync(0xffffffffu, e0f[i], 8); e0f[i] += __shfl_xor_sync(0xffffffffu, e0f[i], 16);
            }
            if (edge1) {
              e1g[i] += __shfl_xor_sync(0xffffffffu, e1g[i], 8); e1g[i] += __shfl_xor_sync(0xffffffffu, e1g[i], 16);
              e1f[i] += __shfl_xor_sync(0xffffffffu, e1f[i], 8); e1f[i] += __shfl_xor_sync(0xffffffffu, e1f[i], 16);
            }
// ... 27 lines not shown
          eo[pp] = (rowbase + (uint32_t)min(rbase + pp * 4, p.T - 1)) * (uint32_t)p.C + cn;
        if (is_res) {
          if (!p.last_layer) {
            const uint16_t* const xlo = p.x_planes + plane;
            uint16_t* const xo = p.x_out_planes != nullptr ? p.x_out_planes : p.x_planes;
            uint16_t* const xo_lo = xo + plane;
            uint2 h2[4], l2[4];
#pragma unroll
            for (int pp = 0; pp < 4; ++pp) {
              h2[pp] = *reinterpret_cast<const uint2*>(p.x_planes + eo[pp]);
              l2[pp] = *reinterpret_cast<const uint2*>(xlo + eo[pp]);
            }
#pragma unroll
            for (int pp = 0; pp < 4; ++pp) {
              if (pp >= nrows) break;
              float x0, x1, x2, x3;
              fd_combine2(h2[pp].x, l2[pp].x, PREC, x0, x1);
              fd_combine2(h2[pp].y, l2[pp].y, PREC, x2, x3);
              x0 = (x0 + (a[pp].x * p.acc_scale + bias4.x)) * 0.70710678118654752440f;
              x1 = (x1 + (a[pp].y * p.acc_scale + bias4.y)) * 0.70710678118654752440f;
              x2 = (x2 + (a[pp].z * p.acc_scale + bias4.z)) * 0.70710678118654752440f;
              x3 = (x3 + (a[pp].w * p.acc_scale + bias4.w)) * 0.70710678118654752440f;
              uint32_t h0, l0, h1, l1;
              fd_split2(x0, x1, PREC, h0, l0);
              fd_split2(x2, x3, PREC, h1, l1);
              *reinterpret_cast<uint2*>(xo + eo[pp]) = make_uint2(h0, h1);
              *reinterpret_cast<uint2*>(xo_lo + eo[pp]) = make_uint2(l0, l1);
            }
          }
        } else {
          float4 sk[4];
          if (!p.first_layer) {
#pragma unroll
            for (int pp = 0; pp < 4; ++pp) sk[pp] = *reinterpret_cast<const float4*>(p.skip_f32 + eo[pp]);
          }
          uint16_t* const sk_lo = p.skip_planes + plane;
#pragma unroll
          for (int pp = 0; pp < 4; ++pp) {
            if (pp >= nrows) break;
            float y0 = a[pp].x * p.acc_scale + bias4.x, y1 = a[pp].y * p.acc_scale + bias4.y;
            float y2 = a[pp].z * p.acc_scale + bias4.z, y3 = a[pp].w * p.acc_scale + bias4.w;
            if (!p.first_layer) { y0 += sk[pp].x; y1 += sk[pp].y; y2 += sk[pp].z; y3 += sk[pp].w; }
            if (p.last_layer) {
              uint32_t h0, l0, h1, l1;
              fd_split2(y0 * p.skip_scale, y1 * p.skip_scale, PREC, h0, l0);
              fd_split2(y2 * p.skip_scale, y3 * p.skip_scale, PREC, h1, l1);
              *reinterpret_cast<uint2*>(p.skip_planes + eo[pp]) = make_uint2(h0, h1);
              *reinterpret_cast<uint2*>(sk_lo + eo[pp]) = make_uint2(l0, l1);
            } else {
              *reinterpret_cast<float4*>(p.skip_f32 + eo[pp]) = make_float4(y0, y1, y2, y3);
            }
          }
        }
      } else {
        const float4 bias4 = lds128(bias_addr + 4u * col);
        uint32_t eo[4];
#pragma unroll
        for (int pp = 0; pp < 4; ++pp)
          eo[pp] = (rowbase + (uint32_t)min(rbase + pp * 4, p.T - 1)) * (uint32_t)p.n_total + (uint32_t)n;
        float4 pre[4];
#pragma unroll
        for (int pp = 0; pp < 4; ++pp) pre[pp] = make_float4(0.f, 0.f, 0.f, 0.f);
        if (p.addend != nullptr) {
#pragma unroll
          for (int pp = 0; pp < 4; ++pp) {
            const float4 t4 = *reinterpret_cast<const float4*>(p.addend + eo[pp]);
            pre[pp].x += t4.x; pre[pp].y += t4.y; pre[pp].z += t4.z; pre[pp].w += t4.w;
          }
        }
        if (p.res_f32 != nullptr) {
#pragma unroll
          for (int pp = 0; pp < 4; ++pp) {
            const float4 t4 = *reinterpret_cast<const float4*>(p.res_f32 + eo[pp]);
            pre[pp].x += t4.x; pre[pp].y += t4.y; pre[pp].z += t4.z; pre[pp].w += t4.w;
          }
        }
        if (p.res_planes != nullptr) {
          const uint16_t* const lo_base = p.res_planes + (size_t)p.B * p.T * p.n_total;
#pragma unroll
          for (int pp = 0; pp < 4; ++pp) {
            const uint2 h2 = *reinterpret_cast<const uint2*>(p.res_planes + eo[pp]);
            const uint2 l2 = *reinterpret_cast<const uint2*>(lo_base + eo[pp]);
            float r0, r1, r2, r3;
            fd_combine2(h2.x, l2.x, PREC, r0, r1);
            fd_combine2(h2.y, l2.y, PREC, r2, r3);
            pre[pp].x += p.res_scale * r0; pre[pp].y += p.res_scale * r1;
            pre[pp].z += p.res_scale * r2; pre[pp].w += p.res_scale * r3;
          }
        }
        uint32_t mkbits = 0;
        if (p.row_mask != nullptr) {
#pragma unroll
          for (int pp = 0; pp < 4; ++pp)
            if (p.row_mask[rowbase + (uint32_t)min(rbase + pp * 4, p.T - 1)] != 0) mkbits |= 1u << pp;
        }
#pragma unroll
        for (int pp = 0; pp < 4; ++pp) {
          a[pp].x = (a[pp].x * p.acc_scale + bias4.x + pre[pp].x) * p.post_scale;
          a[pp].y = (a[pp].y * p.acc_scale + bias4.y + pre[pp].y) * p.post_scale;
          a[pp].z = (a[pp].z * p.acc_scale + bias4.z + pre[pp].z) * p.post_scale;
          a[pp].w = (a[pp].w * p.acc_scale + bias4.w + pre[pp].w) * p.post_scale;
        }
        if (p.out_f32 != nullptr && p.out_accum) {
#pragma unroll
          for (int pp = 0; pp < 4; ++pp) {
            const float4 o4 = *reinterpret_cast<const float4*>(p.out_f32 + eo[pp]);
            a[pp].x += o4.x; a[pp].y += o4.y; a[pp].z += o4.z; a[pp].w += o4.w;
          }
        }
        const float slope = p.act == FD_ACT_NONE ? 1.f : p.act == FD_ACT_RELU ? 0.f : p.act_slope;
        uint16_t* const out_lo = p.out_planes + (size_t)p.B * p.T * p.n_total;
#pragma unroll
        for (int pp = 0; pp < 4; ++pp) {
          if (pp >= nrows) break;
          if ((mkbits >> pp) & 1u) a[pp] = make_float4(0.f, 0.f, 0.f, 0.f);
          if (p.out_f32 != nullptr) *reinterpret_cast<float4*>(p.out_f32 + eo[pp]) = a[pp];
          if (p.out_planes != nullptr) {
            uint32_t h0, l0, h1, l1;
            fd_split2(fd_act(a[pp].x * p.planes_scale, slope), fd_act(a[pp].y * p.planes_scale, slope), PREC, h0, l0);
            fd_split2(fd_act(a[pp].z * p.planes_scale, slope), fd_act(a[pp].w * p.planes_scale, slope), PREC, h1, l1);
            *reinterpret_cast<uint2*>(p.out_planes + eo[pp]) = make_uint2(h0, h1);
            *reinterpret_cast<uint2*>(out_lo + eo[pp]) = make_uint2(l0, l1);
          }
        }
      }
    }
  } else {
    constexpr int PER = BLOCK_N / 2;
    frag_to_scratch<BLOCK_N>(my_scratch, acc, 0, 0, lane);
    __syncwarp();
    const int r = lane >> 1, sub = lane & 1;
    float v[PER];
#pragma unroll
    for (int q4 = 0; q4 < PER / 4; ++q4) {
      const float4 x = scratch_ld4(my_scratch, r, sub * (PER / 4) + q4);
      v[4 * q4] = x.x; v[4 * q4 + 1] = x.y; v[4 * q4 + 2] = x.z; v[4 * q4 + 3] = x.w;
    }
    __syncwarp();
    const int t = rw0 + r;
    if (t < p.T) {
#pragma unroll
      for (int h = 0; h < PER / 8; ++h) {
        float v8[8];
#pragma unroll
        for (int i = 0; i < 8; ++i) v8[i] = v[h * 8 + i];
        const int cc = sub * PER + h * 8;
        if (EPI == FD_EPI_LINEAR) fd_epi_linear<8, PREC>(p, b, t, n0 + cc, v8, bias_s, n0);
        else fd_epi_res_skip<8, PREC>(p, b, t, n0 + cc, v8, bias_s + cc);
      }
    }
  }
}

template <int BLOCK_N, int BLOCK_K, int EPI, int PREC, int NPL>
__global__ void __launch_bounds__(FD_TC_THREADS, 1)
fd_tapgemm_tc_kernel(const __grid_constant__ CUtensorMap tm_src0, const __grid_constant__ CUtensorMap tm_src1,
                     const __grid_constant__ CUtensorMap tm_w, const FdTapGemm p) {
  using C = Cfg<BLOCK_N, BLOCK_K, EPI, NPL>;
  static_assert(!C::PP, "GATE / RES_SKIP run the ping-pong schedule");
  using MMA = Wgmma<BLOCK_N, PREC>;
  extern __shared__ uint8_t smem_raw[];
  uint8_t* smem = reinterpret_cast<uint8_t*>((reinterpret_cast<uintptr_t>(smem_raw) + 1023) & ~(uintptr_t)1023);
  uint8_t* stage_base = smem;
  float* bias_s = reinterpret_cast<float*>(smem + C::NUM_STAGES * C::STAGE_BYTES);
  uint64_t* full_bar = reinterpret_cast<uint64_t*>(bias_s + C::BIAS_TOTAL);
  uint64_t* empty_bar = full_bar + C::NUM_STAGES;
  float* scratch_s = reinterpret_cast<float*>(empty_bar + C::NUM_STAGES);

  const int warp = threadIdx.x / 32;
  const int lane = threadIdx.x % 32;

  const int tiles_t = (p.T + BLOCK_M - 1) / BLOCK_M;
  const int num_m_tiles = p.B * tiles_t;
  const int num_n_tiles = p.n_total / BLOCK_N;
  const int num_tiles = num_m_tiles * num_n_tiles;
  int total_k_blocks = 0;
  for (int sI = 0; sI < p.num_seg; ++sI) total_k_blocks += p.seg[sI].k_len / BLOCK_K;

  if (threadIdx.x == 0) {
    for (int i = 0; i < C::NUM_STAGES; ++i) { mbar_init(&full_bar[i], 1); mbar_init(&empty_bar[i], FD_TC_CONSUMER_THREADS / 32); }
    fence_barrier_init();
  }
  if (warp == FD_TC_PRODUCER_WARP && lane == 0) {
    prefetch_tmap(&tm_src0);
    prefetch_tmap(&tm_src1);
    prefetch_tmap(&tm_w);
  }
  __syncthreads();

  if (warp >= FD_TC_PRODUCER_WARP) {
    producer_regs();
    if (warp == FD_TC_PRODUCER_WARP && lane == 0) {
      int stage = 0; uint32_t phase = 0;
      for (int tile = blockIdx.x; tile < num_tiles; tile += gridDim.x) {
        const int m_tile = tile / num_n_tiles;
        const int n_tile = (tile % num_n_tiles + m_tile) % num_n_tiles;
        const int b = m_tile / tiles_t, t0 = (m_tile % tiles_t) * BLOCK_M;
        const int n0 = n_tile * BLOCK_N;
        int s = 0, k0 = 0, koff = 0;
        for (int kb = 0; kb < total_k_blocks; kb += C::GROUP) {
          const int nb = min(C::GROUP, total_k_blocks - kb);
          mbar_wait(&empty_bar[stage], phase ^ 1);
          uint8_t* st = stage_base + stage * C::STAGE_BYTES;
          mbar_expect_tx(&full_bar[stage], nb * C::TX_BYTES);
          for (int g = 0; g < nb; ++g) {
            const FdSeg sg = p.seg[s];
            const CUtensorMap* tm = sg.src == 0 ? &tm_src0 : &tm_src1;
            uint8_t* sub = st + g * C::SUB_BYTES;
            tma_load_4d(sub, tm, &full_bar[stage], sg.c_off + k0, t0 + sg.shift, b, 0);
            const int kw = koff + k0 + p.w_kshift;
            tma_load_3d(sub + NPL * C::A_BYTES, &tm_w, &full_bar[stage], kw, n0, 0);
            k0 += BLOCK_K;
            if (k0 >= sg.k_len) { koff += sg.k_len; k0 = 0; ++s; }
          }
          if (++stage == C::NUM_STAGES) { stage = 0; phase ^= 1; }
        }
      }
    }
    return;
  }

  consumer_regs();
  const int wg = warp / 4;
  const int wq = warp % 4;
  const uint32_t my_scratch = smem_u32(scratch_s) + warp * FD_TC_SCRATCH_WARP_BYTES;
  float acc[BLOCK_N / 2];
  int stage = 0; uint32_t phase = 0;
  long long staged_key = -1;
  for (int tile = blockIdx.x; tile < num_tiles; tile += gridDim.x) {
    const int m_tile = tile / num_n_tiles;
    const int n_tile = (tile % num_n_tiles + m_tile) % num_n_tiles;
    const int b = m_tile / tiles_t, t0 = (m_tile % tiles_t) * BLOCK_M;
    const int n0 = n_tile * BLOCK_N;

    if (EPI == FD_EPI_LINEAR && bias_key<EPI>(p, b, n0) != staged_key) {
      staged_key = bias_key<EPI>(p, b, n0);
      asm volatile("bar.sync 1, %0;" ::"r"(FD_TC_CONSUMER_THREADS) : "memory");
      stage_bias<BLOCK_N, EPI>(p, b, n0, bias_s, threadIdx.x, FD_TC_CONSUMER_THREADS);
      asm volatile("bar.sync 1, %0;" ::"r"(FD_TC_CONSUMER_THREADS) : "memory");
    }

#pragma unroll
    for (int i = 0; i < BLOCK_N / 2; ++i) acc[i] = 0.f;
    int prev_stage = -1;
    for (int kb = 0; kb < total_k_blocks; kb += C::GROUP) {
      const int nb = min(C::GROUP, total_k_blocks - kb);
      mbar_wait(&full_bar[stage], phase);
      wg_fence_operand(acc);
      wg_fence();
      for (int g = 0; g < nb; ++g) {
        const uint32_t st = smem_u32(stage_base + stage * C::STAGE_BYTES + g * C::SUB_BYTES);
        const uint32_t wg_a = wg * 64 * C::SWIZZLE_BYTES;
        const uint64_t a_hi = make_smem_desc(st + wg_a, 16, C::SBO, C::SWIZZLE_MODE);
        const uint64_t a_lo = make_smem_desc(st + C::A_BYTES + wg_a, 16, C::SBO, C::SWIZZLE_MODE);
        const uint64_t w_hi = make_smem_desc(st + NPL * C::A_BYTES, 16, C::SBO, C::SWIZZLE_MODE);
        const uint64_t w_lo = make_smem_desc(st + NPL * C::A_BYTES + C::W_BYTES, 16, C::SBO, C::SWIZZLE_MODE);
#pragma unroll
        for (int k = 0; k < BLOCK_K / 16; ++k) {
          const uint64_t adv = (uint64_t)((k * 32) >> 4);
          if (NPL == 2) {
            MMA::template ss<0, 0>(acc, a_lo + adv, w_hi + adv, 1u);
            MMA::template ss<0, 0>(acc, a_hi + adv, w_lo + adv, 1u);
            MMA::template ss<0, 0>(acc, a_hi + adv, w_hi + adv, 1u);
          } else {
            MMA::template ss<0, 0>(acc, a_hi + adv, w_hi + adv, 1u);
          }
        }
      }
      wg_commit();
      wg_wait<1>();
      wg_fence_operand(acc);
      if (prev_stage >= 0 && lane == 0) mbar_arrive(&empty_bar[prev_stage]);
      prev_stage = stage;
      if (++stage == C::NUM_STAGES) { stage = 0; phase ^= 1; }
    }
    wg_wait<0>();
    wg_fence_operand(acc);
    if (prev_stage >= 0 && lane == 0) mbar_arrive(&empty_bar[prev_stage]);

    tile_epilogue<BLOCK_N, EPI, PREC>(p, acc, b, n_tile, t0 + wg * 64 + wq * 16, bias_s, my_scratch, lane);
  }
}

template <int BLOCK_N, int BLOCK_K, int EPI, int PREC, int NPL>
__global__ void __launch_bounds__(FD_TC_THREADS, 1)
fd_tapgemm_pp_kernel(const __grid_constant__ CUtensorMap tm_src0, const __grid_constant__ CUtensorMap tm_src1,
                     const __grid_constant__ CUtensorMap tm_w, const FdTapGemm p) {
  using C = Cfg<BLOCK_N, BLOCK_K, EPI, NPL>;
  static_assert(C::PP && C::GROUP == 1, "ping-pong schedule: GATE / RES_SKIP, one k-block per stage");
  using MMA = Wgmma<BLOCK_N, PREC>;
  extern __shared__ uint8_t smem_raw[];
  uint8_t* smem = reinterpret_cast<uint8_t*>((reinterpret_cast<uintptr_t>(smem_raw) + 1023) & ~(uintptr_t)1023);
  uint8_t* stage_base = smem;
  float* bias_s = reinterpret_cast<float*>(smem + C::NUM_STAGES * C::STAGE_BYTES);
  uint64_t* full_bar = reinterpret_cast<uint64_t*>(bias_s + C::BIAS_TOTAL);
  uint64_t* empty_bar = full_bar + C::NUM_STAGES;
  float* scratch_s = reinterpret_cast<float*>(empty_bar + C::NUM_STAGES);

  const int warp = threadIdx.x / 32;
  const int lane = threadIdx.x % 32;
  const int rank = (int)cluster_ctarank();
  const int pair = blockIdx.x / 2, num_pairs = gridDim.x / 2;

  const int tiles_t = (p.T + 63) / 64;
  const int num_m_tiles = p.B * tiles_t;
  const int num_n_tiles = p.n_total / BLOCK_N;
  const int num_units = (num_m_tiles + 1) / 2 * num_n_tiles;
  int total_k_blocks = 0;
  for (int sI = 0; sI < p.num_seg; ++sI) total_k_blocks += p.seg[sI].k_len / BLOCK_K;

  if (threadIdx.x == 0) {
    for (int i = 0; i < C::NUM_STAGES; ++i) { mbar_init(&full_bar[i], 1); mbar_init(&empty_bar[i], 2 * 4); }
    fence_barrier_init();
  }
  if (warp == FD_TC_PRODUCER_WARP && lane == 0) {
    prefetch_tmap(&tm_src0);
    prefetch_tmap(&tm_src1);
    prefetch_tmap(&tm_w);
  }
  cluster_sync();

  if (warp >= FD_TC_PRODUCER_WARP) {
    producer_regs();
    if (warp == FD_TC_PRODUCER_WARP && lane == 0) {
      int stage = 0; uint32_t phase = 0;
      for (int u = pair; u < num_units; u += num_pairs) {
        const int m_pair = u / num_n_tiles;
        const int n_tile = (u % num_n_tiles + m_pair) % num_n_tiles;
        const int m_tile = min(2 * m_pair + rank, num_m_tiles - 1);
        const int b = m_tile / tiles_t, t0 = (m_tile % tiles_t) * 64;
        const int n0 = n_tile * BLOCK_N;
        int s = 0, k0 = 0, koff = 0;
#pragma unroll 1
        for (int kb = 0; kb < total_k_blocks; ++kb) {
          mbar_wait(&empty_bar[stage], phase ^ 1);
          uint8_t* st = stage_base + stage * C::STAGE_BYTES;
          mbar_expect_tx(&full_bar[stage], C::TX_BYTES);
          const FdSeg sg = p.seg[s];
          tma_load_4d(st, sg.src == 0 ? &tm_src0 : &tm_src1, &full_bar[stage], sg.c_off + k0, t0 + sg.shift, b, 0);
          tma_load_3d_multicast(st + NPL * C::A_BYTES + rank * (NPL * C::W_BYTES / 2), &tm_w, &full_bar[stage],
                                koff + k0 + p.w_kshift, n0 + (NPL == 1 ? rank * (BLOCK_N / 2) : 0),
                                NPL == 2 ? rank : 0, 0x3);
          k0 += BLOCK_K;
          if (k0 >= sg.k_len) { koff += sg.k_len; k0 = 0; ++s; }
          if (++stage == C::NUM_STAGES) { stage = 0; phase ^= 1; }
        }
      }
    }
  } else {
    consumer_regs();
    const int wg = warp / 4;
    const int wq = warp % 4;
    const uint32_t my_scratch = smem_u32(scratch_s) + warp * FD_TC_SCRATCH_WARP_BYTES;
    float* my_bias = bias_s + wg * C::BIAS_FLOATS;
    float acc[BLOCK_N / 2];
    int stage = 0; uint32_t phase = 0;
    auto advance = [&](int n) {
      stage += n;
      phase ^= (uint32_t)(stage / C::NUM_STAGES) & 1u;
      stage %= C::NUM_STAGES;
    };
    auto release = [&](int st) {
      if (lane == 0) { mbar_arrive_cluster(&empty_bar[st], 0); mbar_arrive_cluster(&empty_bar[st], 1); }
    };
    if (wg == 1) advance(total_k_blocks);
    long long staged_key = -1;
    for (int u = pair + wg * num_pairs; u < num_units; u += 2 * num_pairs) {
      const int m_pair = u / num_n_tiles;
      const int n_tile = (u % num_n_tiles + m_pair) % num_n_tiles;
      const int m_tile = 2 * m_pair + rank;
      const bool valid = m_tile < num_m_tiles;
      const int b = m_tile / tiles_t, t0 = (m_tile % tiles_t) * 64;
      const int n0 = n_tile * BLOCK_N;

      if (valid && bias_key<EPI>(p, b, n0) != staged_key) {
        staged_key = bias_key<EPI>(p, b, n0);
        wg == 0 ? named_bar_sync<3, 128>() : named_bar_sync<4, 128>();
        stage_bias<BLOCK_N, EPI>(p, b, n0, my_bias, threadIdx.x % 128, 128);
        wg == 0 ? named_bar_sync<3, 128>() : named_bar_sync<4, 128>();
      }

      if (u != pair) wg == 0 ? named_bar_sync<1, 256>() : named_bar_sync<2, 256>();
      const bool pass = u + num_pairs < num_units;
#pragma unroll
      for (int i = 0; i < BLOCK_N / 2; ++i) acc[i] = 0.f;
      int prev_stage = -1;
      for (int kb = 0; kb < total_k_blocks; ++kb) {
        mbar_wait(&full_bar[stage], phase);
        wg_fence_operand(acc);
        wg_fence();
        const uint32_t st = smem_u32(stage_base + stage * C::STAGE_BYTES);
        const uint64_t a_hi = make_smem_desc(st, 16, C::SBO, C::SWIZZLE_MODE);
        const uint64_t a_lo = make_smem_desc(st + C::A_BYTES, 16, C::SBO, C::SWIZZLE_MODE);
        const uint64_t w_hi = make_smem_desc(st + NPL * C::A_BYTES, 16, C::SBO, C::SWIZZLE_MODE);
        const uint64_t w_lo = make_smem_desc(st + NPL * C::A_BYTES + C::W_BYTES, 16, C::SBO, C::SWIZZLE_MODE);
#pragma unroll
        for (int k = 0; k < BLOCK_K / 16; ++k) {
          const uint64_t adv = (uint64_t)((k * 32) >> 4);
          if (NPL == 2) {
            MMA::template ss<0, 0>(acc, a_lo + adv, w_hi + adv, 1u);
            MMA::template ss<0, 0>(acc, a_hi + adv, w_lo + adv, 1u);
            MMA::template ss<0, 0>(acc, a_hi + adv, w_hi + adv, 1u);
          } else {
            MMA::template ss<0, 0>(acc, a_hi + adv, w_hi + adv, 1u);
          }
        }
        wg_commit();
        if (kb == total_k_blocks - 1 && pass)
          wg == 0 ? named_bar_arrive<2, 256>() : named_bar_arrive<1, 256>();
        wg_wait<1>();
        wg_fence_operand(acc);
        if (prev_stage >= 0) release(prev_stage);
        prev_stage = stage;
        advance(1);
      }
      wg_wait<0>();
      wg_fence_operand(acc);
      if (prev_stage >= 0) release(prev_stage);
      advance(total_k_blocks);

      if (valid) tile_epilogue<BLOCK_N, EPI, PREC>(p, acc, b, n_tile, t0 + wq * 16, my_bias, my_scratch, lane);
    }
  }
  __syncwarp();
  cluster_sync();
}

template <int BLOCK_T>
struct GateTCfg {
  static constexpr int BLOCK_K = 32;
  static constexpr int ROW_BYTES = BLOCK_K * 2;
  static constexpr int ACT_ROWS = BLOCK_T + 16;
  static constexpr int MAX_DIL = (ACT_ROWS - BLOCK_T) / 2;
  static constexpr int ACT_PLANE = ACT_ROWS * ROW_BYTES;
  static constexpr int W_PLANE = 64 * ROW_BYTES;
  static constexpr int W_OFF = 2 * ACT_PLANE;
  static constexpr int STAGE_BYTES = W_OFF + 3 * 2 * W_PLANE;
  static constexpr uint32_t SWIZZLE_MODE = swizzle_mode_for(ROW_BYTES);
  static constexpr uint32_t SBO = 8 * ROW_BYTES;
  static constexpr int NUM_STAGES =
      fd_tc_ring_stages(1024  + 2 * FD_TC_MAX_STAGES * 8 + FD_TC_SCRATCH_BYTES, STAGE_BYTES);
  static constexpr int SMEM_BYTES = 1024 + NUM_STAGES * STAGE_BYTES + 2 * NUM_STAGES * 8 + FD_TC_SCRATCH_BYTES;
  static_assert(ACT_ROWS <= 256, "one TMA box per plane");
  static_assert(ACT_PLANE % 512 == 0 && STAGE_BYTES % 1024 == 0, "planes start on 64 B swizzle atoms");
  static_assert(NUM_STAGES >= 3, "ring depth");
  static_assert(SMEM_BYTES <= FD_TC_SMEM_BUDGET, "shared memory");
};

template <int BLOCK_T, int PREC>
__device__ __forceinline__ void gate_t_epilogue(const FdTapGemm& p, const float* acc, int b, int t0, int ch,
                                                uint32_t my_scratch, int lane) {
  const int half = p.gate_tile / 2;
  const int e = lane >> 2, q4 = lane & 3;
  const int n_g = (ch / half) * p.gate_tile + ch % half + e, n_f = n_g + half;
  const size_t bo = (size_t)b * p.gbias_bstride;
  const float bg = p.gbias_full[bo + n_g], bf = p.gbias_full[bo + n_f];
  const float lg = p.gbias_lo[bo + n_g], lf = p.gbias_lo[bo + n_f];
  const float hg = p.gbias_hi[bo + n_g], hf = p.gbias_hi[bo + n_f];
  const size_t row0 = (size_t)b * p.T;
  const size_t zplane = (size_t)p.B * p.T * p.C;
  constexpr int NG = BLOCK_T / 8;
  auto load_addend = [&](int c0, float (&a)[16]) {
#pragma unroll
    for (int i = 0; i < 16; ++i) a[i] = 0.f;
    if (p.addend == nullptr) return;
#pragma unroll
    for (int ci = 0; ci < 4; ++ci) {
      if (c0 + ci < NG) {
#pragma unroll
        for (int s = 0; s < 2; ++s) {
          const int t = min(t0 + 8 * (c0 + ci) + 2 * q4 + s, p.T - 1);
          const float* ad = p.addend + (row0 + t) * p.n_total;
          a[4 * ci + 2 * s] = __ldcs(ad + n_g);
          a[4 * ci + 2 * s + 1] = __ldcs(ad + n_f);
        }
      }
    }
  };
  float a_next[16];
  load_addend(0, a_next);
#pragma unroll
  for (int c0 = 0; c0 < NG; c0 += 4) {
    float a_cur[16];
#pragma unroll
    for (int i = 0; i < 16; ++i) a_cur[i] = a_next[i];
    if (c0 + 4 < NG) load_addend(c0 + 4, a_next);
#pragma unroll
    for (int ci = 0; ci < 4; ++ci) {
      if (c0 + ci < NG) {
#pragma unroll
        for (int s = 0; s < 2; ++s) {
          const int tl = 8 * ci + 2 * q4 + s;
          const int t = t0 + 8 * c0 + tl;
          float yg = acc[4 * (c0 + ci) + s] * p.acc_scale + bg + a_cur[4 * ci + 2 * s];
          float yf = acc[4 * (c0 + ci) + 2 + s] * p.acc_scale + bf + a_cur[4 * ci + 2 * s + 1];
          if (t < p.dil) { yg -= lg; yf -= lf; }
          if (t + p.dil >= p.T) { yg -= hg; yf -= hf; }
          sts32(my_scratch + 4u * (tl * 8 + (((e >> 2) ^ ((tl >> 2) & 1)) << 2) + (e & 3)),
                fd_sigmoid(yg) * fd_tanh(yf));
        }
      }
    }
    __syncwarp();
    const int t = t0 + 8 * c0 + lane;
    if (lane < 8 * min(4, NG - c0) && t < p.T) {
      const uint32_t sw = (uint32_t)((lane >> 2) & 1);
      const float4 z0 = lds128(my_scratch + 4u * (lane * 8 + (sw << 2)));
      const float4 z1 = lds128(my_scratch + 4u * (lane * 8 + ((sw ^ 1u) << 2)));
      const float z[8] = {z0.x, z0.y, z0.z, z0.w, z1.x, z1.y, z1.z, z1.w};
      fd_store_planes<8>(p.out_planes, zplane, (row0 + t) * p.C + ch, z, PREC);
    }
    __syncwarp();
  }
}

template <int BLOCK_T, int PREC>
__global__ void __launch_bounds__(FD_TC_THREADS, 1)
fd_gate_t_kernel(const __grid_constant__ CUtensorMap tm_x, const __grid_constant__ CUtensorMap tm_w, const FdTapGemm p) {
  using C = GateTCfg<BLOCK_T>;
  using MMA = Wgmma<BLOCK_T, PREC>;
  extern __shared__ uint8_t smem_raw[];
  uint8_t* smem = reinterpret_cast<uint8_t*>((reinterpret_cast<uintptr_t>(smem_raw) + 1023) & ~(uintptr_t)1023);
  uint8_t* stage_base = smem;
  uint64_t* full_bar = reinterpret_cast<uint64_t*>(smem + C::NUM_STAGES * C::STAGE_BYTES);
  uint64_t* empty_bar = full_bar + C::NUM_STAGES;
  float* scratch_s = reinterpret_cast<float*>(empty_bar + C::NUM_STAGES);

  const int warp = threadIdx.x / 32;
  const int lane = threadIdx.x % 32;
  const int rank = (int)cluster_ctarank();
  const int pair = blockIdx.x / 2, num_pairs = gridDim.x / 2;

  const int d = p.dil;
  const int tiles_t = (p.T + BLOCK_T - 1) / BLOCK_T;
  const int num_wp = p.n_total / 128;
  const int num_units = p.B * tiles_t * num_wp;
  const int k_blocks = p.C / C::BLOCK_K;

  if (threadIdx.x == 0) {
    for (int i = 0; i < C::NUM_STAGES; ++i) { mbar_init(&full_bar[i], 1); mbar_init(&empty_bar[i], 2 * 4); }
    fence_barrier_init();
  }
  if (warp == FD_TC_PRODUCER_WARP && lane == 0) {
    prefetch_tmap(&tm_x);
    prefetch_tmap(&tm_w);
  }
  cluster_sync();

  if (warp >= FD_TC_PRODUCER_WARP) {
    producer_regs();
    if (warp == FD_TC_PRODUCER_WARP && lane == 0) {
      const uint32_t tx = 2u * (uint32_t)(BLOCK_T + 2 * d) * C::ROW_BYTES + 3 * 2 * C::W_PLANE;
      const int half = p.gate_tile / 2;
      int stage = 0; uint32_t phase = 0;
      for (int u = pair; u < num_units; u += num_pairs) {
        const int tt = u / num_wp, wt = 2 * (u % num_wp) + rank;
        const int b = tt / tiles_t, t0 = (tt % tiles_t) * BLOCK_T;
        const int ch = wt * 32;
        const int g0 = ((ch / half) * p.gate_tile + ch % half) / 8;
#pragma unroll 1
        for (int kb = 0; kb < k_blocks; ++kb) {
          mbar_wait(&empty_bar[stage], phase ^ 1);
          uint8_t* st = stage_base + stage * C::STAGE_BYTES;
          mbar_expect_tx(&full_bar[stage], tx);
          tma_load_4d_multicast(st + rank * C::ACT_PLANE, &tm_x, &full_bar[stage], kb * C::BLOCK_K, t0 - d, b, rank,
                                0x3);
#pragma unroll 1
          for (int j = 0; j < 3; ++j)
            tma_load_5d(st + C::W_OFF + j * 2 * C::W_PLANE, &tm_w, &full_bar[stage], j * p.C + kb * C::BLOCK_K, 0, 0,
                        g0, 0);
          if (++stage == C::NUM_STAGES) { stage = 0; phase ^= 1; }
        }
      }
    }
  } else {
    consumer_regs();
    const int wg = warp / 4;
    const int wq = warp % 4;
    const uint32_t my_scratch = smem_u32(scratch_s) + warp * FD_TC_SCRATCH_WARP_BYTES;
    float acc[BLOCK_T / 2];
    int stage = 0; uint32_t phase = 0;
    auto advance = [&](int n) {
      stage += n;
      phase ^= (uint32_t)(stage / C::NUM_STAGES) & 1u;
      stage %= C::NUM_STAGES;
    };
    auto release = [&](int st) {
      if (lane == 0) { mbar_arrive_cluster(&empty_bar[st], 0); mbar_arrive_cluster(&empty_bar[st], 1); }
    };
    if (wg == 1) advance(k_blocks);
    for (int u = pair + wg * num_pairs; u < num_units; u += 2 * num_pairs) {
      const int tt = u / num_wp, wt = 2 * (u % num_wp) + rank;
      const int b = tt / tiles_t, t0 = (tt % tiles_t) * BLOCK_T;

      if (u != pair) wg == 0 ? named_bar_sync<1, 256>() : named_bar_sync<2, 256>();
      const bool pass = u + num_pairs < num_units;
#pragma unroll
      for (int i = 0; i < BLOCK_T / 2; ++i) acc[i] = 0.f;
      int prev_stage = -1;
      for (int kb = 0; kb < k_blocks; ++kb) {
        mbar_wait(&full_bar[stage], phase);
        wg_fence_operand(acc);
        wg_fence();
        const uint32_t st = smem_u32(stage_base + stage * C::STAGE_BYTES);
#pragma unroll
        for (int j = 0; j < 3; ++j) {
          const uint32_t xa = st + (uint32_t)(j * d * C::ROW_BYTES);
          const uint64_t x_hi = make_smem_desc(xa, 16, C::SBO, C::SWIZZLE_MODE);
          const uint64_t x_lo = make_smem_desc(xa + C::ACT_PLANE, 16, C::SBO, C::SWIZZLE_MODE);
          const uint32_t wa = st + C::W_OFF + j * 2 * C::W_PLANE;
          const uint64_t w_hi = make_smem_desc(wa, 16, C::SBO, C::SWIZZLE_MODE);
          const uint64_t w_lo = make_smem_desc(wa + C::W_PLANE, 16, C::SBO, C::SWIZZLE_MODE);
#pragma unroll
          for (int k = 0; k < C::BLOCK_K / 16; ++k) {
            const uint64_t adv = (uint64_t)((k * 32) >> 4);
            MMA::template ss<0, 0>(acc, w_hi + adv, x_lo + adv, 1u);
            MMA::template ss<0, 0>(acc, w_lo + adv, x_hi + adv, 1u);
            MMA::template ss<0, 0>(acc, w_hi + adv, x_hi + adv, 1u);
          }
        }
        wg_commit();
        if (kb == k_blocks - 1 && pass) wg == 0 ? named_bar_arrive<2, 256>() : named_bar_arrive<1, 256>();
        wg_wait<1>();
        wg_fence_operand(acc);
        if (prev_stage >= 0) release(prev_stage);
        prev_stage = stage;
        advance(1);
      }
      wg_wait<0>();
      wg_fence_operand(acc);
      if (prev_stage >= 0) release(prev_stage);
      advance(k_blocks);

      gate_t_epilogue<BLOCK_T, PREC>(p, acc, b, t0, wt * 32 + wq * 8, my_scratch, lane);
    }
  }
  __syncwarp();
  cluster_sync();
}

int gate_t_block(const FdTapGemm& p) {
  if (p.epi != FD_EPI_GATE || p.single || p.y_planes != nullptr || p.num_seg != 3 || p.w_kshift != 0) return 0;
  if (p.C % GateTCfg<200>::BLOCK_K != 0 || p.n_total != 2 * p.C || p.src_C[0] != p.C) return 0;
  if ((p.gate_tile != 256 && p.gate_tile != 128) || p.n_total % p.gate_tile != 0) return 0;
  for (int s = 0; s < 3; ++s)
    if (p.seg[s].src != 0 || p.seg[s].shift != (s - 1) * p.dil || p.seg[s].c_off != 0 || p.seg[s].k_len != p.C)
      return 0;
  int best = 0;
  long long best_pad = 0;
  for (const int bt : {200, 240}) {
    if (p.dil > (bt == 200 ? GateTCfg<200>::MAX_DIL : GateTCfg<240>::MAX_DIL)) continue;
    const long long pad = (long long)(p.T + bt - 1) / bt * bt;
    if (best == 0 || pad < best_pad || (pad == best_pad && bt > best)) { best = bt; best_pad = pad; }
  }
  return best;
}

template <int BLOCK_T, int PREC>
int launch_gate_t(const FdTapGemm& p, cudaStream_t stream) {
  using C = GateTCfg<BLOCK_T>;
  CUtensorMap tmx, tmw;
  int rc = planes_map(&tmx, p.src[0], p.src_C[0], p.T, p.B, p.src_rs[0], p.src_bs[0], p.src_ps[0], C::BLOCK_K,
                      BLOCK_T + 2 * p.dil, 1, "gate_t x");
  if (rc) return rc;
  const int half = p.gate_tile / 2;
  const cuuint64_t K = (cuuint64_t)p.k_total;
  const cuuint64_t dims[5] = {K, 8, 2, (cuuint64_t)p.n_total / 8, 2};
  const cuuint64_t strides[4] = {K * 2, (cuuint64_t)half * K * 2, 8 * K * 2, (cuuint64_t)p.n_total * K * 2};
  const cuuint32_t box[5] = {(cuuint32_t)C::BLOCK_K, 8, 2, 4, 2};
  rc = encode_tiled(&tmw, p.w, 5, dims, strides, box, "gate_t w");
  if (rc) return rc;
  const int units = p.B * ((p.T + BLOCK_T - 1) / BLOCK_T) * (p.n_total / 128);
  return fd_tc_launch<fd_gate_t_kernel<BLOCK_T, PREC>>(C::SMEM_BYTES, 2 * units, stream, false, 2, tmx, tmw, p);
}

template <int BLOCK_N, int BLOCK_K, int EPI, int PREC, int NPL>
int launch_inst(const FdTapGemm& p, cudaStream_t stream) {
  using C = Cfg<BLOCK_N, BLOCK_K, EPI, NPL>;
  CUtensorMap tm0, tm1, tmw;
  int rc = planes_map(&tm0, p.src[0], p.src_C[0], p.T, p.B, p.src_rs[0], p.src_bs[0], p.src_ps[0], BLOCK_K, C::ROWS,
                      NPL, "tapgemm src0");
  if (rc) return rc;
  if (p.src[1] != nullptr) {
    rc = planes_map(&tm1, p.src[1], p.src_C[1], p.T, p.B, p.src_rs[1], p.src_bs[1], p.src_ps[1], BLOCK_K, C::ROWS, NPL,
                    "tapgemm src1");
    if (rc) return rc;
  } else {
    tm1 = tm0;
  }
  const int m_tiles = p.B * ((p.T + C::ROWS - 1) / C::ROWS), n_tiles = p.n_total / BLOCK_N;
  if constexpr (C::PP) {
    rc = weights_map(&tmw, p.w, p.n_total, p.k_total, BLOCK_K, NPL == 2 ? BLOCK_N : BLOCK_N / 2, 1, "tapgemm w");
    if (rc) return rc;
    return fd_tc_launch<fd_tapgemm_pp_kernel<BLOCK_N, BLOCK_K, EPI, PREC, NPL>>(
        C::SMEM_BYTES, 2 * ((m_tiles + 1) / 2 * n_tiles), stream, false, 2, tm0, tm1, tmw, p);
  } else {
    rc = weights_map(&tmw, p.w, p.n_total, p.k_total, BLOCK_K, BLOCK_N, NPL, "tapgemm w");
    if (rc) return rc;
    return fd_tc_launch<fd_tapgemm_tc_kernel<BLOCK_N, BLOCK_K, EPI, PREC, NPL>>(C::SMEM_BYTES, m_tiles * n_tiles,
                                                                              stream, false, 1, tm0, tm1, tmw, p);
  }
}

template <int BLOCK_N, int BLOCK_K, int EPI>
int launch_cfg(const FdTapGemm& p, cudaStream_t stream) {
  if (p.single) {
    return p.prec == FD_F16 ? launch_inst<BLOCK_N, BLOCK_K, EPI, FD_F16, 1>(p, stream)
                            : launch_inst<BLOCK_N, BLOCK_K, EPI, FD_BF16, 1>(p, stream);
  }
  return p.prec == FD_F16 ? launch_inst<BLOCK_N, BLOCK_K, EPI, FD_F16, 2>(p, stream)
                          : launch_inst<BLOCK_N, BLOCK_K, EPI, FD_BF16, 2>(p, stream);
}

template <int BLOCK_N, int BLOCK_K>
int launch_epi(const FdTapGemm& p, cudaStream_t stream) {
  if (p.epi == FD_EPI_GATE) return launch_cfg<BLOCK_N, BLOCK_K, FD_EPI_GATE>(p, stream);
  if (p.epi == FD_EPI_MAG) return launch_cfg<BLOCK_N, BLOCK_K, FD_EPI_MAG>(p, stream);
  if (p.epi == FD_EPI_RES_SKIP) return launch_cfg<BLOCK_N, BLOCK_K, FD_EPI_RES_SKIP>(p, stream);
  if (p.epi == FD_EPI_GATE_BWD) return launch_cfg<BLOCK_N, BLOCK_K, FD_EPI_GATE_BWD>(p, stream);
  return launch_cfg<BLOCK_N, BLOCK_K, FD_EPI_LINEAR>(p, stream);
}

void pick_cfg(const FdTapGemm& p, int* bn, int* bk) {
  *bn = 0; *bk = 0;
  bool all64 = true, all32 = true, all16 = true;
  for (int s = 0; s < p.num_seg; ++s) {
    if (p.seg[s].c_off % 16 != 0) return;
    all64 &= p.seg[s].k_len % 64 == 0;
    all32 &= p.seg[s].k_len % 32 == 0;
    all16 &= p.seg[s].k_len % 16 == 0;
  }
  const int k = all64 ? 64 : all32 ? 32 : all16 ? 16 : 0;
  if (k == 0) return;
  const int npl = p.single ? 1 : 2;
  auto wavenet_bk = [&](int n) {
    return ring_stages(npl * (64 + n) * 64 * 2, 2 * (p.epi == FD_EPI_GATE ? 3 : 1) * n) < 3 ? 32 : 64;
  };
  if (p.epi == FD_EPI_GATE || p.epi == FD_EPI_MAG) {
    const int n = p.gate_tile;
    if ((n != 256 && n != 128) || p.n_total % n != 0 || k != 64) return;
    *bn = n; *bk = p.epi == FD_EPI_GATE ? wavenet_bk(n) : 64;
    return;
  }
  int n = 256;
  while (n >= 16 && (p.n_total % n != 0 || (p.epi == FD_EPI_RES_SKIP && p.C % n != 0))) n >>= 1;
  if (n < 16) return;
  if (k == 64) {
    if (n < 64) return;
    *bn = n; *bk = p.epi == FD_EPI_RES_SKIP ? wavenet_bk(n) : 64;
  } else if (k == 32) {
    if (p.epi != FD_EPI_LINEAR || n < 32) return;
    *bn = n > 64 ? 64 : n; *bk = 32;
  } else {
    if (p.epi != FD_EPI_LINEAR) return;
    *bn = n > 32 ? 32 : n; *bk = 16;
  }
}

}

int fd_tapgemm_tc_supported(const FdTapGemm& p) {
  int bn, bk;
  pick_cfg(p, &bn, &bk);
  if (bn == 0) return 0;
  for (int s = 0; s < 2; ++s)
    if (p.src[s] != nullptr && (p.src_rs[s] % 8 != 0 || p.src_bs[s] % 8 != 0 || p.src_ps[s] % 8 != 0)) return 0;
  if (p.k_total % 8 != 0) return 0;
  return 1;
}

int fd_tapgemm_tc_launch(const FdTapGemm& p, cudaStream_t stream) {
  int bn, bk;
  pick_cfg(p, &bn, &bk);
  const long long width = p.epi == FD_EPI_GATE_BWD ? 2ll * p.n_total : p.n_total;
  FD_REQUIRE((long long)p.B * p.T * width < (1ll << 32),
             "tapgemm(tc): B*T*%lld = %lld exceeds the 32-bit element offsets of the epilogue", width,
             (long long)p.B * p.T * width);
  FD_REQUIRE(bn != 0 && fd_tapgemm_tc_supported(p),
             "tapgemm(tc): no tensor-core instantiation for n_total=%d k_total=%d epi=%d", p.n_total, p.k_total,
             p.epi);
  if (const int bt = gate_t_block(p)) {
    if (bt == 200) return p.prec == FD_F16 ? launch_gate_t<200, FD_F16>(p, stream) : launch_gate_t<200, FD_BF16>(p, stream);
    return p.prec == FD_F16 ? launch_gate_t<240, FD_F16>(p, stream) : launch_gate_t<240, FD_BF16>(p, stream);
  }
  if (bk == 64) {
    if (bn == 256) return launch_epi<256, 64>(p, stream);
    if (bn == 128) return launch_epi<128, 64>(p, stream);
    if (p.epi == FD_EPI_GATE_BWD) return launch_cfg<64, 64, FD_EPI_GATE_BWD>(p, stream);
    if (p.epi == FD_EPI_RES_SKIP) return launch_cfg<64, 64, FD_EPI_RES_SKIP>(p, stream);
    return launch_cfg<64, 64, FD_EPI_LINEAR>(p, stream);
  }
  if (p.epi == FD_EPI_GATE || p.epi == FD_EPI_RES_SKIP) {
    FD_REQUIRE(bk == 32 && bn == 256 && !p.single, "tapgemm(tc): no BLOCK_K=%d instantiation of epi=%d", bk, p.epi);
    if (p.epi == FD_EPI_GATE)
      return p.prec == FD_F16 ? launch_inst<256, 32, FD_EPI_GATE, FD_F16, 2>(p, stream)
                              : launch_inst<256, 32, FD_EPI_GATE, FD_BF16, 2>(p, stream);
    return p.prec == FD_F16 ? launch_inst<256, 32, FD_EPI_RES_SKIP, FD_F16, 2>(p, stream)
                            : launch_inst<256, 32, FD_EPI_RES_SKIP, FD_BF16, 2>(p, stream);
  }
  if (bk == 32) {
    FD_REQUIRE(p.epi == FD_EPI_LINEAR, "tapgemm(tc): BLOCK_K=32 only instantiated for the linear epilogue");
    if (bn == 64) return launch_cfg<64, 32, FD_EPI_LINEAR>(p, stream);
    return launch_cfg<32, 32, FD_EPI_LINEAR>(p, stream);
  }
  FD_REQUIRE(p.epi == FD_EPI_LINEAR, "tapgemm(tc): BLOCK_K=16 only instantiated for the linear epilogue");
  if (bn == 32) return launch_cfg<32, 16, FD_EPI_LINEAR>(p, stream);
  return launch_cfg<16, 16, FD_EPI_LINEAR>(p, stream);
}
```

### fish_diffusion_b200/csrc/fd_tc_ptx.cuh

```cuda
#pragma once
#include <cuda.h>
#include <cuda_runtime.h>
#include <stdint.h>
#include "fd_common.cuh"
#include "fd_host.h"

namespace {

__device__ __forceinline__ uint32_t smem_u32(const void* p) {
  return static_cast<uint32_t>(__cvta_generic_to_shared(p));
}
__device__ __forceinline__ void mbar_init(uint64_t* bar, uint32_t count) {
  asm volatile("mbarrier.init.shared::cta.b64 [%0], %1;" ::"r"(smem_u32(bar)), "r"(count));
}
__device__ __forceinline__ void mbar_expect_tx(uint64_t* bar, uint32_t bytes) {
  asm volatile("mbarrier.arrive.expect_tx.shared::cta.b64 _, [%0], %1;" ::"r"(smem_u32(bar)), "r"(bytes)
               : "memory");
}
__device__ __forceinline__ void mbar_arrive(uint64_t* bar) {
  asm volatile("mbarrier.arrive.shared::cta.b64 _, [%0];" ::"r"(smem_u32(bar)) : "memory");
}
__device__ __forceinline__ void mbar_wait(uint64_t* bar, uint32_t parity) {
  asm volatile(
      "{\n"
// ... 535 lines not shown
        "wgmma.mma_async.sync.aligned.m64n200k16.f32.bf16.bf16 {"
        "%0, %1, %2, %3, %4, %5, %6, %7, %8, %9, %10, %11, %12, %13, %14, %15,"
        "%16, %17, %18, %19, %20, %21, %22, %23, %24, %25, %26, %27, %28, %29, %30, %31,"
        "%32, %33, %34, %35, %36, %37, %38, %39, %40, %41, %42, %43, %44, %45, %46, %47,"
        "%48, %49, %50, %51, %52, %53, %54, %55, %56, %57, %58, %59, %60, %61, %62, %63,"
        "%64, %65, %66, %67, %68, %69, %70, %71, %72, %73, %74, %75, %76, %77, %78, %79,"
        "%80, %81, %82, %83, %84, %85, %86, %87, %88, %89, %90, %91, %92, %93, %94, %95,"
        "%96, %97, %98, %99"
        "}, %100, %101, p, 1, 1, %103, %104;\n}\n"
        : "+f"(d[0]), "+f"(d[1]), "+f"(d[2]), "+f"(d[3]), "+f"(d[4]), "+f"(d[5]), "+f"(d[6]), "+f"(d[7]),
          "+f"(d[8]), "+f"(d[9]), "+f"(d[10]), "+f"(d[11]), "+f"(d[12]), "+f"(d[13]), "+f"(d[14]), "+f"(d[15]),
          "+f"(d[16]), "+f"(d[17]), "+f"(d[18]), "+f"(d[19]), "+f"(d[20]), "+f"(d[21]), "+f"(d[22]), "+f"(d[23]),
          "+f"(d[24]), "+f"(d[25]), "+f"(d[26]), "+f"(d[27]), "+f"(d[28]), "+f"(d[29]), "+f"(d[30]), "+f"(d[31]),
          "+f"(d[32]), "+f"(d[33]), "+f"(d[34]), "+f"(d[35]), "+f"(d[36]), "+f"(d[37]), "+f"(d[38]), "+f"(d[39]),
          "+f"(d[40]), "+f"(d[41]), "+f"(d[42]), "+f"(d[43]), "+f"(d[44]), "+f"(d[45]), "+f"(d[46]), "+f"(d[47]),
          "+f"(d[48]), "+f"(d[49]), "+f"(d[50]), "+f"(d[51]), "+f"(d[52]), "+f"(d[53]), "+f"(d[54]), "+f"(d[55]),
          "+f"(d[56]), "+f"(d[57]), "+f"(d[58]), "+f"(d[59]), "+f"(d[60]), "+f"(d[61]), "+f"(d[62]), "+f"(d[63]),
          "+f"(d[64]), "+f"(d[65]), "+f"(d[66]), "+f"(d[67]), "+f"(d[68]), "+f"(d[69]), "+f"(d[70]), "+f"(d[71]),
          "+f"(d[72]), "+f"(d[73]), "+f"(d[74]), "+f"(d[75]), "+f"(d[76]), "+f"(d[77]), "+f"(d[78]), "+f"(d[79]),
          "+f"(d[80]), "+f"(d[81]), "+f"(d[82]), "+f"(d[83]), "+f"(d[84]), "+f"(d[85]), "+f"(d[86]), "+f"(d[87]),
          "+f"(d[88]), "+f"(d[89]), "+f"(d[90]), "+f"(d[91]), "+f"(d[92]), "+f"(d[93]), "+f"(d[94]), "+f"(d[95]),
          "+f"(d[96]), "+f"(d[97]), "+f"(d[98]), "+f"(d[99])
        : "l"(da), "l"(db), "r"(scale_d), "n"(TA), "n"(TB));
  }
};
template <> struct Wgmma<240, FD_F16> {
  template <int TA, int TB>
  static __device__ __forceinline__ void ss(float* d, uint64_t da, uint64_t db, uint32_t scale_d) {
    asm volatile(
        "{\n.reg .pred p;\nsetp.ne.b32 p, %122, 0;\n"
        "wgmma.mma_async.sync.aligned.m64n240k16.f32.f16.f16 {"
        "%0, %1, %2, %3, %4, %5, %6, %7, %8, %9, %10, %11, %12, %13, %14, %15,"
        "%16, %17, %18, %19, %20, %21, %22, %23, %24, %25, %26, %27, %28, %29, %30, %31,"
        "%32, %33, %34, %35, %36, %37, %38, %39, %40, %41, %42, %43, %44, %45, %46, %47,"
        "%48, %49, %50, %51, %52, %53, %54, %55, %56, %57, %58, %59, %60, %61, %62, %63,"
        "%64, %65, %66, %67, %68, %69, %70, %71, %72, %73, %74, %75, %76, %77, %78, %79,"
        "%80, %81, %82, %83, %84, %85, %86, %87, %88, %89, %90, %91, %92, %93, %94, %95,"
        "%96, %97, %98, %99, %100, %101, %102, %103, %104, %105, %106, %107, %108, %109, %110, %111,"
        "%112, %113, %114, %115, %116, %117, %118, %119"
        "}, %120, %121, p, 1, 1, %123, %124;\n}\n"
        : "+f"(d[0]), "+f"(d[1]), "+f"(d[2]), "+f"(d[3]), "+f"(d[4]), "+f"(d[5]), "+f"(d[6]), "+f"(d[7]),
          "+f"(d[8]), "+f"(d[9]), "+f"(d[10]), "+f"(d[11]), "+f"(d[12]), "+f"(d[13]), "+f"(d[14]), "+f"(d[15]),
          "+f"(d[16]), "+f"(d[17]), "+f"(d[18]), "+f"(d[19]), "+f"(d[20]), "+f"(d[21]), "+f"(d[22]), "+f"(d[23]),
          "+f"(d[24]), "+f"(d[25]), "+f"(d[26]), "+f"(d[27]), "+f"(d[28]), "+f"(d[29]), "+f"(d[30]), "+f"(d[31]),
          "+f"(d[32]), "+f"(d[33]), "+f"(d[34]), "+f"(d[35]), "+f"(d[36]), "+f"(d[37]), "+f"(d[38]), "+f"(d[39]),
          "+f"(d[40]), "+f"(d[41]), "+f"(d[42]), "+f"(d[43]), "+f"(d[44]), "+f"(d[45]), "+f"(d[46]), "+f"(d[47]),
          "+f"(d[48]), "+f"(d[49]), "+f"(d[50]), "+f"(d[51]), "+f"(d[52]), "+f"(d[53]), "+f"(d[54]), "+f"(d[55]),
          "+f"(d[56]), "+f"(d[57]), "+f"(d[58]), "+f"(d[59]), "+f"(d[60]), "+f"(d[61]), "+f"(d[62]), "+f"(d[63]),
          "+f"(d[64]), "+f"(d[65]), "+f"(d[66]), "+f"(d[67]), "+f"(d[68]), "+f"(d[69]), "+f"(d[70]), "+f"(d[71]),
          "+f"(d[72]), "+f"(d[73]), "+f"(d[74]), "+f"(d[75]), "+f"(d[76]), "+f"(d[77]), "+f"(d[78]), "+f"(d[79]),
          "+f"(d[80]), "+f"(d[81]), "+f"(d[82]), "+f"(d[83]), "+f"(d[84]), "+f"(d[85]), "+f"(d[86]), "+f"(d[87]),
          "+f"(d[88]), "+f"(d[89]), "+f"(d[90]), "+f"(d[91]), "+f"(d[92]), "+f"(d[93]), "+f"(d[94]), "+f"(d[95]),
          "+f"(d[96]), "+f"(d[97]), "+f"(d[98]), "+f"(d[99]), "+f"(d[100]), "+f"(d[101]), "+f"(d[102]), "+f"(d[103]),
          "+f"(d[104]), "+f"(d[105]), "+f"(d[106]), "+f"(d[107]), "+f"(d[108]), "+f"(d[109]), "+f"(d[110]), "+f"(d[111]),
          "+f"(d[112]), "+f"(d[113]), "+f"(d[114]), "+f"(d[115]), "+f"(d[116]), "+f"(d[117]), "+f"(d[118]), "+f"(d[119])
        : "l"(da), "l"(db), "r"(scale_d), "n"(TA), "n"(TB));
  }
};
template <> struct Wgmma<240, FD_BF16> {
  template <int TA, int TB>
  static __device__ __forceinline__ void ss(float* d, uint64_t da, uint64_t db, uint32_t scale_d) {
    asm volatile(
        "{\n.reg .pred p;\nsetp.ne.b32 p, %122, 0;\n"
        "wgmma.mma_async.sync.aligned.m64n240k16.f32.bf16.bf16 {"
        "%0, %1, %2, %3, %4, %5, %6, %7, %8, %9, %10, %11, %12, %13, %14, %15,"
        "%16, %17, %18, %19, %20, %21, %22, %23, %24, %25, %26, %27, %28, %29, %30, %31,"
        "%32, %33, %34, %35, %36, %37, %38, %39, %40, %41, %42, %43, %44, %45, %46, %47,"
        "%48, %49, %50, %51, %52, %53, %54, %55, %56, %57, %58, %59, %60, %61, %62, %63,"
        "%64, %65, %66, %67, %68, %69, %70, %71, %72, %73, %74, %75, %76, %77, %78, %79,"
        "%80, %81, %82, %83, %84, %85, %86, %87, %88, %89, %90, %91, %92, %93, %94, %95,"
        "%96, %97, %98, %99, %100, %101, %102, %103, %104, %105, %106, %107, %108, %109, %110, %111,"
        "%112, %113, %114, %115, %116, %117, %118, %119"
        "}, %120, %121, p, 1, 1, %123, %124;\n}\n"
        : "+f"(d[0]), "+f"(d[1]), "+f"(d[2]), "+f"(d[3]), "+f"(d[4]), "+f"(d[5]), "+f"(d[6]), "+f"(d[7]),
          "+f"(d[8]), "+f"(d[9]), "+f"(d[10]), "+f"(d[11]), "+f"(d[12]), "+f"(d[13]), "+f"(d[14]), "+f"(d[15]),
          "+f"(d[16]), "+f"(d[17]), "+f"(d[18]), "+f"(d[19]), "+f"(d[20]), "+f"(d[21]), "+f"(d[22]), "+f"(d[23]),
          "+f"(d[24]), "+f"(d[25]), "+f"(d[26]), "+f"(d[27]), "+f"(d[28]), "+f"(d[29]), "+f"(d[30]), "+f"(d[31]),
          "+f"(d[32]), "+f"(d[33]), "+f"(d[34]), "+f"(d[35]), "+f"(d[36]), "+f"(d[37]), "+f"(d[38]), "+f"(d[39]),
          "+f"(d[40]), "+f"(d[41]), "+f"(d[42]), "+f"(d[43]), "+f"(d[44]), "+f"(d[45]), "+f"(d[46]), "+f"(d[47]),
          "+f"(d[48]), "+f"(d[49]), "+f"(d[50]), "+f"(d[51]), "+f"(d[52]), "+f"(d[53]), "+f"(d[54]), "+f"(d[55]),
          "+f"(d[56]), "+f"(d[57]), "+f"(d[58]), "+f"(d[59]), "+f"(d[60]), "+f"(d[61]), "+f"(d[62]), "+f"(d[63]),
          "+f"(d[64]), "+f"(d[65]), "+f"(d[66]), "+f"(d[67]), "+f"(d[68]), "+f"(d[69]), "+f"(d[70]), "+f"(d[71]),
          "+f"(d[72]), "+f"(d[73]), "+f"(d[74]), "+f"(d[75]), "+f"(d[76]), "+f"(d[77]), "+f"(d[78]), "+f"(d[79]),
          "+f"(d[80]), "+f"(d[81]), "+f"(d[82]), "+f"(d[83]), "+f"(d[84]), "+f"(d[85]), "+f"(d[86]), "+f"(d[87]),
          "+f"(d[88]), "+f"(d[89]), "+f"(d[90]), "+f"(d[91]), "+f"(d[92]), "+f"(d[93]), "+f"(d[94]), "+f"(d[95]),
          "+f"(d[96]), "+f"(d[97]), "+f"(d[98]), "+f"(d[99]), "+f"(d[100]), "+f"(d[101]), "+f"(d[102]), "+f"(d[103]),
          "+f"(d[104]), "+f"(d[105]), "+f"(d[106]), "+f"(d[107]), "+f"(d[108]), "+f"(d[109]), "+f"(d[110]), "+f"(d[111]),
          "+f"(d[112]), "+f"(d[113]), "+f"(d[114]), "+f"(d[115]), "+f"(d[116]), "+f"(d[117]), "+f"(d[118]), "+f"(d[119])
        : "l"(da), "l"(db), "r"(scale_d), "n"(TA), "n"(TB));
  }
};


constexpr int FD_TC_SCRATCH_WARP_BYTES = 16 * 32 * 4;
constexpr int FD_TC_SCRATCH_BYTES = (FD_TC_CONSUMER_THREADS / 32) * FD_TC_SCRATCH_WARP_BYTES;
template <int CW>
__device__ __forceinline__ void frag_to_scratch(uint32_t scratch, const float* d, int c0, int off, int lane) {
#pragma unroll
  for (int i = 0; i < CW / 2; i += 2) {
    const int row = (lane >> 2) + 8 * ((i >> 1) & 1);
    const int col = off + 8 * (i >> 2) + 2 * (lane & 3);
    sts64(scratch + row * 128 + (((col >> 2) ^ (row & 7)) << 4) + (col & 3) * 4, d[c0 / 2 + i], d[c0 / 2 + i + 1]);
  }
}
__device__ __forceinline__ float4 scratch_ld4(uint32_t scratch, int row, int chunk) {
  return lds128(scratch + row * 128 + ((chunk ^ (row & 7)) << 4));
}

typedef CUresult (*PFN_tmapEncodeTiled)(CUtensorMap*, CUtensorMapDataType, cuuint32_t, void*, const cuuint64_t*,
                                        const cuuint64_t*, const cuuint32_t*, const cuuint32_t*,
                                        CUtensorMapInterleave, CUtensorMapSwizzle, CUtensorMapL2promotion,
                                        CUtensorMapFloatOOBfill);

PFN_tmapEncodeTiled get_encode() {
  static PFN_tmapEncodeTiled fn = nullptr;
  if (fn == nullptr) {
    void* ptr = nullptr;
    cudaDriverEntryPointQueryResult qres;
    if (cudaGetDriverEntryPoint("cuTensorMapEncodeTiled", &ptr, cudaEnableDefault, &qres) == cudaSuccess &&
        qres == cudaDriverEntryPointSuccess)
      fn = reinterpret_cast<PFN_tmapEncodeTiled>(ptr);
  }
  return fn;
}

int encode_tiled(CUtensorMap* m, const uint16_t* ptr, int rank, const cuuint64_t* dims, const cuuint64_t* strides,
                 const cuuint32_t* box, const char* what) {
  PFN_tmapEncodeTiled enc = get_encode();
  FD_REQUIRE(enc != nullptr, "cuTensorMapEncodeTiled not available from the driver");
  const CUtensorMapSwizzle sw = tma_swizzle_for((int)box[0] * 2);
  FD_REQUIRE(sw != CU_TENSOR_MAP_SWIZZLE_NONE, "tensor map (%s): box rows of %u bytes (wgmma swizzles 128, 64 or 32)",
             what, box[0] * 2);
  FD_REQUIRE(rank >= 1 && rank <= 5, "tensor map (%s): rank %d (1..5)", what, rank);
  const cuuint32_t estr[5] = {1, 1, 1, 1, 1};
  CUresult r = enc(m, CU_TENSOR_MAP_DATA_TYPE_UINT16, (cuuint32_t)rank, const_cast<uint16_t*>(ptr), dims, strides, box,
                   estr, CU_TENSOR_MAP_INTERLEAVE_NONE, sw, CU_TENSOR_MAP_L2_PROMOTION_L2_256B,
                   CU_TENSOR_MAP_FLOAT_OOB_FILL_NONE);
  FD_REQUIRE(r == CUDA_SUCCESS, "cuTensorMapEncodeTiled(%s) failed: %d (dims %llu x %llu x %llu x %llu, box %u x %u x %u x %u, ptr %p)",
             what, (int)r, (unsigned long long)dims[0], (unsigned long long)dims[1], (unsigned long long)dims[2],
             rank >= 4 ? (unsigned long long)dims[3] : 1ull, box[0], box[1], box[2], rank >= 4 ? box[3] : 1u,
             (const void*)ptr);
  return 0;
}

int planes_map(CUtensorMap* m, const uint16_t* ptr, int C, int T, int B, long long row_stride, long long item_stride,
               long long plane_stride, int box_c, int box_rows, int box_planes, const char* what) {
  const cuuint64_t dims[4] = {(cuuint64_t)C, (cuuint64_t)T, (cuuint64_t)B, 2};
  const cuuint64_t strides[3] = {(cuuint64_t)row_stride * 2, (cuuint64_t)item_stride * 2, (cuuint64_t)plane_stride * 2};
  const cuuint32_t box[4] = {(cuuint32_t)box_c, (cuuint32_t)box_rows, 1, (cuuint32_t)box_planes};
  return encode_tiled(m, ptr, 4, dims, strides, box, what);
}

int weights_map(CUtensorMap* m, const uint16_t* ptr, int N, int K, int box_k, int box_n, int box_planes,
                const char* what) {
  const cuuint64_t dims[3] = {(cuuint64_t)K, (cuuint64_t)N, 2};
  const cuuint64_t strides[2] = {(cuuint64_t)K * 2, (cuuint64_t)N * K * 2};
  const cuuint32_t box[3] = {(cuuint32_t)box_k, (cuuint32_t)box_n, (cuuint32_t)box_planes};
  return encode_tiled(m, ptr, 3, dims, strides, box, what);
}

template <auto Kern, typename... Args>
int fd_tc_launch(int smem_bytes, int work_units, cudaStream_t stream, bool max_carveout, int cluster,
                 const Args&... args) {
  static bool attr_set[FD_MAX_DEVICES] = {false};
  static int max_grid[FD_MAX_DEVICES];
  const int dev = fd_current_device();
  cudaLaunchAttribute attr[1];
  attr[0].id = cudaLaunchAttributeClusterDimension;
  attr[0].val.clusterDim.x = cluster;
  attr[0].val.clusterDim.y = 1;
  attr[0].val.clusterDim.z = 1;
  cudaLaunchConfig_t cfg = {};
  cfg.blockDim = dim3(FD_TC_THREADS);
  cfg.dynamicSmemBytes = smem_bytes;
  cfg.stream = stream;
  cfg.attrs = attr;
  cfg.numAttrs = cluster > 1 ? 1 : 0;
  if (!attr_set[dev]) {
    FD_CHECK_CUDA(cudaFuncSetAttribute(Kern, cudaFuncAttributeMaxDynamicSharedMemorySize, smem_bytes));
    if (max_carveout)
      FD_CHECK_CUDA(cudaFuncSetAttribute(Kern, cudaFuncAttributePreferredSharedMemoryCarveout,
                                         cudaSharedmemCarveoutMaxShared));
    const int sms = fd_device_sms(dev);
    max_grid[dev] = sms - sms % cluster;
    if (cluster > 1) {
      int clusters = 0;
      cfg.gridDim = dim3(max_grid[dev]);
      FD_CHECK_CUDA(cudaOccupancyMaxActiveClusters(&clusters, Kern, &cfg));
      FD_REQUIRE(clusters > 0, "no cluster of %d CTAs with %d bytes of shared memory fits on device %d", cluster,
                 smem_bytes, dev);
      if (clusters * cluster < max_grid[dev]) max_grid[dev] = clusters * cluster;
    }
    attr_set[dev] = true;
  }
  const int grid = work_units < max_grid[dev] ? work_units : max_grid[dev];
  cfg.gridDim = dim3(grid - grid % cluster);
  FD_CHECK_CUDA(cudaLaunchKernelEx(&cfg, Kern, args...));
  return 0;
}


}
```

### fish_diffusion_b200/wavenet.py

```python
from __future__ import annotations

import ctypes
import math
import os

import torch
from torch import nn

from . import _native as N
from .registry import DENOISERS


class Mish(nn.Module):

    def forward(self, x):
        raise RuntimeError("fish_diffusion_b200.WaveNet runs its MLP natively")


class DiffusionEmbedding(nn.Module):
    def __init__(self, d_denoiser):
        super().__init__()
        self.dim = d_denoiser


class LinearNorm(nn.Module):

    def __init__(self, in_features, out_features, bias=False):
        super().__init__()
        self.linear = nn.Linear(in_features, out_features, bias)
        nn.init.xavier_uniform_(self.linear.weight)
        if bias:
            nn.init.constant_(self.linear.bias, 0.0)


class ConvNorm(nn.Module):

    def __init__(self, in_channels, out_channels, kernel_size=1, stride=1, padding=None, dilation=1, bias=True):
        super().__init__()
        if padding is None:
            assert kernel_size % 2 == 1
            padding = int(dilation * (kernel_size - 1) / 2)
        self.conv = nn.Conv1d(in_channels, out_channels, kernel_size=kernel_size, stride=stride, padding=padding,
                              dilation=dilation, bias=bias)
        nn.init.kaiming_normal_(self.conv.weight)


class ResidualBlock(nn.Module):

    def __init__(self, d_encoder, residual_channels, use_linear_bias=False, dilation=1):
        super().__init__()
        self.dilation = dilation
        self.conv_layer = ConvNorm(residual_channels, 2 * residual_channels, kernel_size=3, stride=1,
                                   padding=dilation, dilation=dilation)
        self.diffusion_projection = LinearNorm(residual_channels, residual_channels, use_linear_bias)
        self.conditioner_projection = ConvNorm(d_encoder, 2 * residual_channels, kernel_size=1)
        self.output_projection = ConvNorm(residual_channels, 2 * residual_channels, kernel_size=1)


def _gate_half(C: int) -> int:
    for g in (128, 64, 16):
        if C % g == 0:
            return g
    raise ValueError(f"residual_channels={C} must be a multiple of 16")


class WaveNet(nn.Module):

    def __init__(self, mel_channels=128, d_encoder=256, residual_channels=512, residual_layers=20,
                 use_linear_bias=False, dilation_cycle=None, precision="f16", backend="auto"):
        super().__init__()
        self.mel_channels, self.d_encoder = mel_channels, d_encoder
        self.residual_channels, self.n_layers = residual_channels, residual_layers
        self.input_projection = ConvNorm(mel_channels, residual_channels, kernel_size=1)
        self.diffusion_embedding = DiffusionEmbedding(residual_channels)
        self.mlp = nn.Sequential(
            LinearNorm(residual_channels, residual_channels * 4, use_linear_bias),
            Mish(),
            LinearNorm(residual_channels * 4, residual_channels, use_linear_bias),
        )
        self.residual_layers = nn.ModuleList([
            ResidualBlock(d_encoder, residual_channels, use_linear_bias=use_linear_bias,
                          dilation=2 ** (i % dilation_cycle) if dilation_cycle else 1)
            for i in range(residual_layers)
        ])
        self.skip_projection = ConvNorm(residual_channels, residual_channels, kernel_size=1)
        self.output_projection = ConvNorm(residual_channels, mel_channels, kernel_size=1)
        nn.init.zeros_(self.output_projection.conv.weight)

        self.precision = precision
        self.backend = os.environ.get("FD_BACKEND", backend)
        self._pack = None
        self._pack_key = None
        self._pack_static = None
        self._scale_state = None
        self.register_load_state_dict_post_hook(lambda module, incompatible: setattr(module, "_scale_state", None))
        self._ws = {}
        self._graphs = {}
        self.use_graph = os.environ.get("FD_GRAPH", "1") != "0"

    def _resolve_backend(self) -> int:
        if self.backend != "auto":
            return N.backend_code(self.backend)
        C, E, M = self.residual_channels, self.d_encoder, self.mel_channels
        ok = (C % 64 == 0 and E % 64 == 0 and M % 64 == 0 and _gate_half(C) in (128, 64))
        return N.BACKEND_TC if ok else N.BACKEND_SIMT

    def _scales(self, device, lag_ok=False):
        L = self.n_layers
        raw = [self.input_projection.conv.weight, self.skip_projection.conv.weight, self.output_projection.conv.weight]
        for blk in self.residual_layers:
            raw += [blk.conv_layer.conv.weight, blk.conditioner_projection.conv.weight, blk.output_projection.conv.weight]

        def amax_dev():
            return torch.stack(torch._foreach_norm([w.detach() for w in raw], float("inf"))).to(torch.float32)

        st = self._scale_state
        pending = st.get("pending") if (lag_ok and st is not None and st["device"] == str(device)) else None
        if pending is not None:
            pending[0].synchronize()
            amax = pending[1].tolist()
        else:
            amax = amax_dev().tolist()

        def p2(m):
            return 1.0 if m == 0.0 or m != m else float(2.0 ** math.floor(math.log2(64.0 / m)))

        s1 = [p2(max(amax[3 + 3 * l], amax[4 + 3 * l])) for l in range(L)]
        s2 = [p2(amax[5 + 3 * l]) for l in range(L)]
        new = {"device": str(device), "s_in": p2(amax[0]), "s_skip": p2(amax[1]), "s_out": p2(amax[2]), "s1": s1, "s2": s2}
        if st is not None and st["device"] == str(device) and st["s1"] == s1 and st["s2"] == s2:
            new["dev"] = st["dev"]
        else:
            new["dev"] = torch.tensor(s1 + s2, dtype=torch.float32, device=device)
        if lag_ok and device.type == "cuda":
            host = st["pending"][1] if pending is not None else torch.empty(len(raw), dtype=torch.float32).pin_memory()
            host.copy_(amax_dev(), non_blocking=True)
            ev = torch.cuda.Event()
            ev.record(torch.cuda.current_stream(device))
            new["pending"] = (ev, host)
        self._scale_state = new
        return new

    def _packed(self, device, want_bwd=False):
        key = (str(device), self.precision, tuple(p._version for p in self.parameters()),
               tuple(p.data_ptr() for p in self.parameters()))
        if self._pack is not None and self._pack_key == key and (self._pack["has_bwd"] or not want_bwd):
            return self._pack
        prec = N.prec_code(self.precision)
        C, E, M, L = self.residual_channels, self.d_encoder, self.mel_channels, self.n_layers
        KT = 3 * C + E
        half = _gate_half(C)
        gate_tile = 2 * half
        f32 = lambda t: t.detach().to(device=device, dtype=torch.float32)
        sc = self._scales(device, lag_ok=want_bwd)
        s_in, s_skip, s_out, s1, s2 = sc["s_in"], sc["s_skip"], sc["s_out"], sc["s1"], sc["s2"]

        stat = self._pack_static
        has_bwd = bool(want_bwd or (stat is not None and stat["has_bwd"]))
        ptr_key = (str(device), self.precision, has_bwd)
        if stat is None or stat["key"] != ptr_key:
            i16 = dict(dtype=torch.int16, device=device)
            idx = torch.arange(C, device=device).view(C // half, half)
            stat = {"key": ptr_key, "has_bwd": has_bwd,
                    "perm": torch.cat([idx, idx + C], dim=1).reshape(-1),
                    "w1p_f32": torch.empty((L, 2 * C, KT), dtype=torch.float32, device=device),
                    "w1": torch.empty((L, 2, 2 * C, KT), **i16), "w2": torch.empty((L, 2, 2 * C, C), **i16),
                    "w1t": torch.empty((L, 2, C, 6 * C), **i16) if has_bwd else None,
                    "wct": torch.empty((L, 2, E, 2 * C), **i16) if has_bwd else None,
                    "w2t": torch.empty((L, 2, C, 2 * C), **i16) if has_bwd else None}
            self._pack_static = stat
        srcs = [[f32(b.conv_layer.conv.weight).contiguous() for b in self.residual_layers],
                [f32(b.conditioner_projection.conv.weight).contiguous() for b in self.residual_layers],
                [f32(b.output_projection.conv.weight).contiguous() for b in self.residual_layers]]
        src_ptrs = tuple(t.data_ptr() for grp in srcs for t in grp)
        if stat.get("src_ptrs") != src_ptrs:
            stat["src_ptrs"] = src_ptrs
            stat["ptr_table"] = torch.tensor(src_ptrs, dtype=torch.int64).view(3, L).to(device)
        tab = stat["ptr_table"]
        N.check(N.lib().fd_wavenet_pack_layers(
            N.ptr(tab[0]), N.ptr(tab[1]), N.ptr(tab[2]), N.ptr(sc["dev"]), N.ptr(stat["w1p_f32"]), N.ptr(stat["w1"]),
            N.ptr(stat["w2"]), N.ptr(stat["w1t"]), N.ptr(stat["wct"]), N.ptr(stat["w2t"]), L, C, E, half, prec,
            N.stream_ptr(device)), "fd_wavenet_pack_layers")

        def pack(w2d, scale):
            return N.pack_weight(w2d, prec, scale), 1.0 / scale

        pk = {"prec": prec, "mma": N.mma_code(self.precision), "gate_tile": gate_tile,
              "backend": self._resolve_backend(), "perm": stat["perm"], "has_bwd": stat["has_bwd"],
              "s_in": s_in, "s_skip": s_skip, "s_out": s_out, "s1": s1, "s2": s2, "_srcs": srcs}
        pk["w_in"], pk["w_in_inv"] = pack(f32(self.input_projection.conv.weight)[:, :, 0], s_in)
        pk["b_in"] = f32(self.input_projection.conv.bias).contiguous()
        pk["mlp_w0"] = f32(self.mlp[0].linear.weight).contiguous()
        pk["mlp_b0"] = f32(self.mlp[0].linear.bias).contiguous() if self.mlp[0].linear.bias is not None else None
        pk["mlp_w1"] = f32(self.mlp[2].linear.weight).contiguous()
        pk["mlp_b1"] = f32(self.mlp[2].linear.bias).contiguous() if self.mlp[2].linear.bias is not None else None
        blocks = list(self.residual_layers)
        pk["w1p_f32"] = stat["w1p_f32"]
        pk["bias_sum"] = (torch.stack([f32(b.conv_layer.conv.bias) for b in blocks]) +
                          torch.stack([f32(b.conditioner_projection.conv.bias) for b in blocks]))[:, stat["perm"]].contiguous()
        pk["w1"], pk["w1_inv"] = [stat["w1"][l] for l in range(L)], [1.0 / v for v in s1]
        pk["w2"], pk["w2_inv"] = [stat["w2"][l] for l in range(L)], [1.0 / v for v in s2]
        pk["b2"] = torch.stack([f32(b.output_projection.conv.bias) for b in blocks]).contiguous()
        pk["wd"] = torch.stack([f32(b.diffusion_projection.linear.weight) for b in blocks]).contiguous()
        pk["bd"] = (torch.stack([f32(b.diffusion_projection.linear.bias) for b in blocks]).contiguous()
                    if blocks[0].diffusion_projection.linear.bias is not None else None)
        pk["dil"] = [b.dilation for b in blocks]
        pk["w_skip"], pk["w_skip_inv"] = pack(f32(self.skip_projection.conv.weight)[:, :, 0], s_skip)
        pk["b_skip"] = f32(self.skip_projection.conv.bias).contiguous()
        pk["w_out"], pk["w_out_inv"] = pack(f32(self.output_projection.conv.weight)[:, :, 0], s_out)
        pk["b_out"] = f32(self.output_projection.conv.bias).contiguous()
        if stat["has_bwd"]:
            bw = {"w1t": [stat["w1t"][l] for l in range(L)], "w1t_inv": pk["w1_inv"],
                  "wct": [stat["wct"][l] for l in range(L)], "wct_inv": pk["w1_inv"],
                  "w2t": [stat["w2t"][l] for l in range(L)], "w2t_inv": pk["w2_inv"]}
            bw["wot"], bw["wot_inv"] = pack(f32(self.output_projection.conv.weight)[:, :, 0].t().contiguous(), s_out)
            bw["wst"], bw["wst_inv"] = pack(f32(self.skip_projection.conv.weight)[:, :, 0].t().contiguous(), s_skip)
            bw["wit"], bw["wit_inv"] = pack(f32(self.input_projection.conv.weight)[:, :, 0].t().contiguous(), s_in)
            pk["_bwd"] = bw
        self._pack, self._pack_key = pk, key
        return pk

    def _workspace(self, device, B, T, Bs):
        key = (str(device), B, T, Bs)
        ws = self._ws.get(key)
        if ws is None:
            C, M, L = self.residual_channels, self.mel_channels, self.n_layers
            i16 = dict(dtype=torch.int16, device=device)
            f32 = dict(dtype=torch.float32, device=device)
            ws = {
                "xr": torch.empty((2, B, T, C), **i16), "z": torch.empty((2, B, T, C), **i16),
                "skip_planes": torch.empty((2, B, T, C), **i16), "skip_f32": torch.empty((B, T, C), **f32),
                "s": torch.empty((Bs, C), **f32), "mlp_ws": torch.empty((Bs * 5 * C,), **f32),
                "gb": torch.empty((3, L, Bs, 2 * C), **f32), "gb_ws": torch.empty((L * Bs * C,), **f32),
                "steps": torch.empty((Bs,), **f32),
            }
            self._ws = {key: ws}
            self._graphs = {}
        return ws

    def train_param_list(self):
        ps = [self.input_projection.conv.weight, self.input_projection.conv.bias]
        for blk in self.residual_layers:
            ps += [blk.conv_layer.conv.weight, blk.conv_layer.conv.bias, blk.conditioner_projection.conv.weight,
                   blk.conditioner_projection.conv.bias, blk.output_projection.conv.weight,
                   blk.output_projection.conv.bias]
        ps += [self.skip_projection.conv.weight, self.skip_projection.conv.bias, self.output_projection.conv.weight,
               self.output_projection.conv.bias]
        return ps

    def train_param_keys(self):
        keys = [("w1x1", "input_projection.w"), ("b", "input_projection.b")]
        for l in range(self.n_layers):
            keys += [("w3", f"l{l}.w1"), ("b", f"l{l}.b1"), ("w1x1", f"l{l}.wc"), ("b", f"l{l}.b1"),
                     ("w1x1", f"l{l}.w2"), ("b", f"l{l}.b2")]
        keys += [("w1x1", "skip_projection.w"), ("b", "skip_projection.b"), ("w1x1", "output_projection.w"),
                 ("b", "output_projection.b")]
        return keys

    def step_vectors(self, diffusion_step):
        import torch.nn.functional as F
        C = self.residual_channels
        half = C // 2
        emb = math.log(10000) / (half - 1)
        emb = torch.exp(torch.arange(half, device=diffusion_step.device) * -emb)
        emb = diffusion_step[:, None] * emb[None, :]
        s = torch.cat((emb.sin(), emb.cos()), dim=-1)
        s = self.mlp[0].linear(s)
        s = s * torch.tanh(F.softplus(s))
        s = self.mlp[2].linear(s)
        lin = [blk.diffusion_projection.linear for blk in self.residual_layers]
        d = torch.einsum("bc,lkc->blk", s, torch.stack([m.weight for m in lin]))
        if lin[0].bias is not None:
            d = d + torch.stack([m.bias for m in lin])[None]
        return d

    def forward_train_cl(self, x_cl, diffusion_step, cond_cl, x_mask=None, cond_mask=None):
        from .wavenet_train import WaveNetTrainFn
        d = self.step_vectors(diffusion_step)
        masks = None
        if x_mask is not None or cond_mask is not None:
            u8 = lambda m: None if m is None else m.to(device=x_cl.device, dtype=torch.uint8).contiguous()
            masks = (u8(x_mask), u8(cond_mask))
        return WaveNetTrainFn.apply(self, masks, x_cl.contiguous(), cond_cl.contiguous(), d, *self.train_param_list())

    def cond_proj_shape(self, B, T):
        return (self.n_layers, B, T, 2 * self.residual_channels)

    @torch.no_grad()
    def cond_projection(self, cond_planes, out):
        dev = cond_planes.device
        N.require_cuda(cond_planes, "cond_planes")
        _, B, T, E = cond_planes.shape
        if E != self.d_encoder or tuple(out.shape) != self.cond_proj_shape(B, T) or out.dtype != torch.float32 \
                or not out.is_contiguous() or out.device != dev:
            raise ValueError(f"cond_projection: out must be contiguous float32 {self.cond_proj_shape(B, T)} on {dev}")
        pk = self._packed(dev)
        w1s = self._pack_static["w1"]
        d = N.WaveNetFwdDesc()
        d.cond_planes, d.cond_proj = N.ptr(cond_planes), N.ptr(out)
        d.w1, d.w1_lstride = N.ptr(w1s), w1s.stride(0)
        for l in range(self.n_layers):
            d.w1_inv[l] = pk["w1_inv"][l]
        d.B, d.T, d.C, d.E, d.L = B, T, self.residual_channels, E, self.n_layers
        d.prec, d.backend = pk["mma"], pk["backend"]
        N.check(N.lib().fd_wavenet_cond_proj(ctypes.byref(d), N.stream_ptr(dev)), "fd_wavenet_cond_proj")
        return out

    @torch.no_grad()
    def forward_cl(self, x_planes, steps, cond_planes, x_mask=None, out=None, cond_proj=None):
        dev = x_planes.device
        N.require_cuda(x_planes, "x_planes")
        _, B, T, M = x_planes.shape
        C, E, L = self.residual_channels, self.d_encoder, self.n_layers
        assert M == self.mel_channels and tuple(cond_planes.shape) == (2, B, T, E)
        pk = self._packed(dev)
        mma, backend = pk["mma"], pk["backend"]
        steps = steps.to(device=dev, dtype=torch.float32).reshape(-1).contiguous()
        Bs = steps.numel()
        if Bs not in (1, B):
            raise ValueError(f"diffusion_step must have 1 or B={B} entries, got {Bs}")
        ws = self._workspace(dev, B, T, Bs)
        st = N.stream_ptr(dev)
        lib = N.lib()
        if x_mask is not None:
            x_mask = x_mask.to(device=dev, dtype=torch.uint8).contiguous()
        if out is None:
            out = torch.empty((B, T, M), dtype=torch.float32, device=dev)

        steps_buf = ws["steps"]
        steps_buf.copy_(steps, non_blocking=True)
        if cond_proj is not None and tuple(cond_proj.shape) != self.cond_proj_shape(B, T):
            raise ValueError(f"cond_proj must have shape {self.cond_proj_shape(B, T)}")
        d = self._fwd_desc(pk, ws, x_planes, cond_planes, steps_buf, x_mask, out, B, T, Bs)
        d.cond_proj = N.ptr(cond_proj)
        use_graph = self.use_graph and not N.prof_is_on()
        if not use_graph:
            N.check(lib.fd_wavenet_fwd(ctypes.byref(d), st), "fd_wavenet_fwd")
            return out
        key = (x_planes.data_ptr(), cond_planes.data_ptr(), out.data_ptr(), 0 if x_mask is None else x_mask.data_ptr(),
               0 if cond_proj is None else cond_proj.data_ptr(), B, T, Bs, self._pack_key, id(ws))
        ent = self._graphs.get(key)
        if ent is None:
            if len(self._graphs) >= 4:
                self._graphs.clear()
            self._graphs[key] = {"graph": None, "keep": (x_planes, cond_planes, out, x_mask, cond_proj, pk)}
            N.check(lib.fd_wavenet_fwd(ctypes.byref(d), st), "fd_wavenet_fwd")
            return out
        if ent["graph"] is None:
            g = torch.cuda.CUDAGraph()
            cur = torch.cuda.current_stream(dev)
            side = torch.cuda.Stream(device=dev)
            side.wait_stream(cur)
            with torch.cuda.stream(side):
                g.capture_begin()
                try:
                    N.check(lib.fd_wavenet_fwd(ctypes.byref(d), N.stream_ptr(dev)), "fd_wavenet_fwd")
                finally:
                    g.capture_end()
            cur.wait_stream(side)
            ent["graph"] = g
        ent["graph"].replay()
        return out

    def _fwd_desc(self, pk, ws, x_planes, cond_planes, steps, x_mask, out, B, T, Bs):
        C, E, M, L = self.residual_channels, self.d_encoder, self.mel_channels, self.n_layers
        if L > 64:
            raise ValueError("fd_wavenet_fwd supports up to 64 residual layers")
        d = N.WaveNetFwdDesc()
        d.x_planes, d.cond_planes, d.steps, d.x_mask, d.out = (N.ptr(x_planes), N.ptr(cond_planes), N.ptr(steps),
                                                               N.ptr(x_mask), N.ptr(out))
        d.w_in, d.b_in, d.w_in_inv = N.ptr(pk["w_in"]), N.ptr(pk["b_in"]), pk["w_in_inv"]
        d.mlp_w0, d.mlp_b0, d.mlp_w1, d.mlp_b1 = (N.ptr(pk["mlp_w0"]), N.ptr(pk["mlp_b0"]), N.ptr(pk["mlp_w1"]),
                                                  N.ptr(pk["mlp_b1"]))
        d.wd, d.bd, d.w1p_f32, d.bias_sum = N.ptr(pk["wd"]), N.ptr(pk["bd"]), N.ptr(pk["w1p_f32"]), N.ptr(pk["bias_sum"])
        w1s, w2s = self._pack_static["w1"], self._pack_static["w2"]
        d.w1, d.w1_lstride = N.ptr(w1s), w1s.stride(0)
        d.w2, d.w2_lstride = N.ptr(w2s), w2s.stride(0)
        d.b2, d.b2_lstride = N.ptr(pk["b2"]), pk["b2"].stride(0)
        d.w_skip, d.b_skip, d.w_skip_inv = N.ptr(pk["w_skip"]), N.ptr(pk["b_skip"]), pk["w_skip_inv"]
        d.w_out, d.b_out, d.w_out_inv = N.ptr(pk["w_out"]), N.ptr(pk["b_out"]), pk["w_out_inv"]
        for l in range(L):
            d.w1_inv[l], d.w2_inv[l], d.dilation[l] = pk["w1_inv"][l], pk["w2_inv"][l], pk["dil"][l]
        d.xr, d.z, d.skip_planes, d.skip_f32 = N.ptr(ws["xr"]), N.ptr(ws["z"]), N.ptr(ws["skip_planes"]), N.ptr(ws["skip_f32"])
        d.s, d.mlp_ws, d.gb, d.gb_ws = N.ptr(ws["s"]), N.ptr(ws["mlp_ws"]), N.ptr(ws["gb"]), N.ptr(ws["gb_ws"])
        d.B, d.T, d.M, d.C, d.E, d.L, d.Bs = B, T, M, C, E, L, Bs
        d.gate_tile, d.prec, d.backend = pk["gate_tile"], pk["mma"], pk["backend"]
        return d

    def forward(self, x, diffusion_step, conditioner, x_masks=None, cond_masks=None):
        if torch.is_grad_enabled() and (x.requires_grad or conditioner.requires_grad or
                                        any(p.requires_grad for p in self.parameters())):
            x3 = x[:, 0] if x.dim() == 4 else x
            eps = self.forward_train_cl(x3.transpose(1, 2), diffusion_step, conditioner.transpose(1, 2),
                                        x_mask=x_masks, cond_mask=cond_masks).transpose(1, 2)
            return eps[:, None] if x.dim() == 4 else eps
        use_4_dim = x.dim() == 4
        if use_4_dim:
            x = x[:, 0]
        assert x.dim() == 3, f"mel must be 3 dim tensor, but got {x.dim()}"
        N.require_cuda(x, "x")
        prec = N.prec_code(self.precision)
        B, M, T = x.shape
        x_planes = N.split_ncw(x.to(torch.float32), prec)
        cmask = None if cond_masks is None else cond_masks.to(torch.uint8).contiguous()
        cond_planes = N.split_ncw(conditioner.to(torch.float32), prec, mask=cmask)
        eps = self.forward_cl(x_planes, diffusion_step.to(torch.float32), cond_planes, x_mask=x_masks)
        out = torch.empty((B, M, T), dtype=torch.float32, device=x.device)
        N.check(N.lib().fd_transpose_nwc_to_ncw(N.ptr(eps), N.ptr(out), B, T, M, N.stream_ptr(x.device)),
                "fd_transpose_nwc_to_ncw")
        return out[:, None] if use_4_dim else out


DENOISERS.register_module(name="WaveNetDenoiser", module=WaveNet, force=True)
DENOISERS.register_module(name="B200WaveNetDenoiser", module=WaveNet, force=True)
```

### include/fishdiff_b200.h

```cpp
#ifndef FISHDIFF_B200_H
#define FISHDIFF_B200_H

#include <stdint.h>
#include <stddef.h>

#ifdef __cplusplus
extern "C" {
#endif

#define FD_PREC_F16 0
#define FD_PREC_BF16 1
#define FD_PREC_SINGLE 0x10
#define FD_BACKEND_TC 0
#define FD_BACKEND_SIMT 1
#define FD_ABI_VERSION 3

int fd_abi_version(void);
const char* fd_last_error(void);
void fd_set_device(int device);
long long fd_launch_count(void);
void fd_prof_enable(int on);
int fd_prof_collect(double* ms_sum, long long* count, int nkinds);
int fd_tc_supported_linear(int n_total, int k_seg, int num_seg);

int fd_split_ncw(const float* src, const uint8_t* mask, uint16_t* planes, int B, int C, int T, int prec,
                 void* stream);
int fd_split_nwc(const float* src, const uint8_t* mask, uint16_t* planes, int B, int T, int C, float scale,
                 int prec, void* stream);
int fd_mrf_finish(const uint16_t* const* in, int num, uint16_t* out, long long n, float in_slope, float scale,
                  float out_slope, int prec, void* stream);
int fd_transpose_nwc_to_ncw(const float* src, float* dst, int B, int T, int C, void* stream);
int fd_transpose_ncw_to_nwc(const float* src, float* dst, int B, int C, int T, void* stream);
int fd_pack_weight(const float* w, uint16_t* planes, long long n_elems, float scale, int prec, void* stream);

int fd_wavenet_pack_layers(const float* const* conv_w, const float* const* cond_w, const float* const* out_w,
                           const float* scales, float* w1p_f32, uint16_t* w1, uint16_t* w2, uint16_t* w1t, uint16_t* wct,
                           uint16_t* w2t, int L, int C, int E, int gate_half, int prec, void* stream);

int fd_wavenet_step_mlp(const float* steps, const float* w0, const float* b0, const float* w1, const float* b1,
                        float* s_out, float* ws, int Bs, int C, void* stream);
int fd_wavenet_gate_bias(const float* s, const float* wd, const float* bd, const float* w1p, const float* bias_sum,
                         float* gb_full, float* gb_lo, float* gb_hi, float* ws, int L, int Bs, int C, int KT,
                         void* stream);
typedef struct fd_wavenet_fwd_desc {
  const uint16_t* x_planes;
  const uint16_t* cond_planes;
  const float* steps;
  const uint8_t* x_mask;
  float* out;
  const uint16_t* w_in; const float* b_in; float w_in_inv;
  const float* mlp_w0; const float* mlp_b0; const float* mlp_w1; const float* mlp_b1;
  const float* wd; const float* bd; const float* w1p_f32; const float* bias_sum;
  const uint16_t* w1; long long w1_lstride;
  const uint16_t* w2; long long w2_lstride;
  const float* b2; long long b2_lstride;
  const uint16_t* w_skip; const float* b_skip; float w_skip_inv;
  const uint16_t* w_out; const float* b_out; float w_out_inv;
  float w1_inv[64], w2_inv[64];
  int dilation[64];
  uint16_t* xr; uint16_t* z; uint16_t* skip_planes; float* skip_f32;
  float* s; float* mlp_ws; float* gb; float* gb_ws;
  int B, T, M, C, E, L, Bs;
  int gate_tile, prec, backend;
  float* cond_proj;
} fd_wavenet_fwd_desc;
int fd_wavenet_fwd(const fd_wavenet_fwd_desc* d, void* stream);
int fd_wavenet_cond_proj(const fd_wavenet_fwd_desc* d, void* stream);

int fd_wavenet_block_fwd(uint16_t* x_planes, const uint16_t* cond_planes, uint16_t* z_planes,
                         const uint16_t* w1, const uint16_t* w2, const float* gb_full, const float* gb_lo,
                         const float* gb_hi, int gb_bstride, const float* b2, float* skip_f32,
                         uint16_t* skip_planes, float skip_scale, int B, int T, int C, int E, int dilation,
                         int gate_tile, float w1_inv_scale, float w2_inv_scale, int flags, int prec, int backend,
                         void* stream);

typedef struct fd_conv_desc {
  const uint16_t* in_planes;
  const uint16_t* w_planes;
  const float* bias;
  const float* addend;
  const float* res_f32;
  const uint16_t* res_planes;
  const uint8_t* row_mask;
  float* out_f32;
  uint16_t* out_planes;
  int B, T, Cin, N;
  int ntaps;
  int shifts[16];
  float w_inv_scale, post_scale, planes_scale, act_slope;
  int out_accum;
  int act;
  int prec, backend;
} fd_conv_desc;
int fd_conv_cl_fwd(const fd_conv_desc* d, void* stream);

typedef struct fd_respair_desc {
  const uint16_t* in_planes;
  const uint16_t* w1;
  const uint16_t* w2;
  const float* b1;
  const float* b2;
  uint16_t* out_planes;
  int B, T, C;
  int k1, d1, k2;
  float w1_inv_scale, w2_inv_scale;
  float in_slope, out_slope, planes_scale;
  int prec;
  unsigned long long kmask1, kmask2;
} fd_respair_desc;
int fd_respair_supported(int C, int k1, int d1, int k2);
int fd_respair_fwd(const fd_respair_desc* d, void* stream);

int fd_ddpm_step(const float* x, const float* eps, const float* noise, float* x_out, uint16_t* x_planes,
                 long long n, float c_recip, float c_recipm1, float c1, float c2, float sigma, float clip_min,
                 float clip_max, unsigned long long seed, unsigned long long offset, unsigned long long subseq0,
                 int prec, void* stream);
int fd_lincomb(float* out, uint16_t* out_planes, const float* const* host_in_ptrs, const float* host_coefs,
               int nterms, long long n, int prec, void* stream);
int fd_affine_cl(const float* x, float* y, const float* scale, const float* shift, int nparam, long long rows,
                 int C, void* stream);
int fd_q_sample(const float* x, const float* noise, const float* a, const float* s, float* y, int B,
                long long per_item, void* stream);
int fd_randn(float* out, long long n, unsigned long long seed, unsigned long long offset, unsigned long long subseq0,
             void* stream);

size_t fd_sinegen_ws_bytes(int B, long long S);
int fd_sinegen_fwd(const float* f0, const float* lin_w, const float* lin_b, const float* rand_ini,
                   const float* noise, float* har, void* ws, int B, int T, int hop, int H, float sampling_rate,
                   float sine_amp, float noise_std, unsigned long long seed, void* stream);
int fd_source_conv_fwd(const float* har, const float* w , const float* bias , float* out,
                       int B, long long S, int C, int k, int s, int p, void* stream);
int fd_conv_post_fwd(const uint16_t* in_planes, const float* w, const float* bias, float* wav, int B,
                     long long S, int C, int k, int prec, void* stream);

int fd_reflect_pad_split(const float* wav, uint16_t* planes, int B, long long N, int pad, int prec, void* stream);
int fd_stft_mag_fwd(const uint16_t* padded, const uint16_t* dft_w, uint16_t* mag_planes, int B, long long Np,
                    int n_fft, int hop, int frames, int NB, float w_inv_scale, float mag_scale, int prec,
                    int backend, void* stream);
int fd_stft_mag_eps_fwd(const uint16_t* padded, const uint16_t* dft_w, uint16_t* mag_planes, int B, long long Np,
                    int n_fft, int hop, int frames, int NB, float w_inv_scale, float mag_scale, float mag_eps, int prec,
                    int backend, void* stream);
int fd_log_clamp(const float* x, float* y, long long n, float clip, float out_scale, void* stream);

long long fd_resample_out_len(long long n_in, int sr_in, int sr_out);
int fd_resample_fwd(const float* wav, const long long* lens, float* out, const float* bank, const int* first,
                    const int* count, int B, long long n_in, long long n_out, int O, int P, int W, int taps, void* stream);

typedef struct fd_gemm_desc {
  const uint16_t* src[2];
  int src_C[2];
  const uint16_t* w;
  int n_total, k_total, w_kshift;
  int B, T, num_seg;
  int seg_src[16], seg_shift[16], seg_coff[16], seg_klen[16];
  const float* bias;
  const float* addend;
  const float* res_f32;
  const uint16_t* res_planes;
  const uint8_t* row_mask;
  float* out_f32;
  uint16_t* out_planes;
  float w_inv_scale, res_scale, post_scale, planes_scale, act_slope;
  int out_accum, act, prec, backend;
  int bias_bstride;
  const uint16_t* gate_y;
  float* gate_cs;
  float* gate_cs_edge;
  float gate_cs_scale;
  int gate_tile, gate_dil;
} fd_gemm_desc;
int fd_gemm_cl_fwd(const fd_gemm_desc* d, void* stream);

int fd_wavenet_block_fwd_train(const uint16_t* x_planes, uint16_t* x_out_planes, const uint16_t* cond_planes,
                               uint16_t* z_planes, uint16_t* y_planes, const uint16_t* w1, const uint16_t* w2,
                               const float* gb_full, const float* gb_lo, const float* gb_hi, int gb_bstride,
                               const float* b2, float* skip_f32, uint16_t* skip_planes, float skip_scale, int B, int T,
                               int C, int E, int dilation, int gate_tile, float w1_inv_scale, float w2_inv_scale,
                               int flags, int prec, int backend, void* stream);
int fd_wavenet_gate_bias_from_d(const float* d, const float* w1p, const float* bias_sum, float* gb_full, float* gb_lo,
                                float* gb_hi, int L, int Bs, int C, int KT, void* stream);
int fd_relu_bwd(const float* grad, const uint16_t* act_planes, uint16_t* out_planes, long long n, float scale, int prec,
                void* stream);
int fd_lrelu_bwd(const float* grad, const uint16_t* act_planes, const float* addend, float* out_f32,
                 uint16_t* out_planes, long long n, float slope, float scale, int prec, void* stream);
int fd_colsum(const uint16_t* planes, const float* f32, float* out, int B, int T, int N, float scale, int prec,
              void* stream);

typedef struct fd_wgrad_desc {
  const uint16_t* row_src[2];
  int row_C[2];
  const uint16_t* col_src[2];
  int col_C[2];
  int num_row_seg;
  int row_seg_src[2], row_seg_coff[2], row_seg_width[2];
  int num_col_seg;
  int col_seg_src[8], col_seg_shift[8], col_seg_coff[8], col_seg_width[8];
  int B, T, splits;
  float* part;
  float acc_scale;
  int prec;
  int backend;
} fd_wgrad_desc;
int fd_wgrad_cl(const fd_wgrad_desc* d, void* stream);

int fd_reduce_batch(const float* in, float* out, int B, long long n, float scale, void* stream);

typedef struct fd_wavenet_bwd_desc {
  const uint16_t* x_planes;
  const uint16_t* y_planes;
  const uint16_t* z_planes;
  const uint16_t* cond_planes;
  const uint16_t* dx_next;
  const uint16_t* dskip;
  const uint16_t* w2t; const uint16_t* w1t; const uint16_t* wct;
  float w2t_inv, w1t_inv, wct_inv;
  uint16_t* dx_out;
  float* dx_f32;
// ... 17 lines not shown
```

Measured before the change: 22950.

## Batch skip-sum into one chained GEMM over a stored z history

After: 23710, median of 6. 1.03x the previous value.

```diff
diff --git a/fish_diffusion_b200/_native.py b/fish_diffusion_b200/_native.py
--- a/fish_diffusion_b200/_native.py
+++ b/fish_diffusion_b200/_native.py
@@ -14,7 +14,7 @@
 PREC_SINGLE = 0x10
 BACKEND_TC, BACKEND_SIMT = 0, 1
 ACT_NONE, ACT_RELU, ACT_LRELU = 0, 1, 2
-ABI_VERSION = 3
+ABI_VERSION = 4
 
 
 class NativeError(RuntimeError):
@@ -73,6 +73,7 @@
         ("B", c_int), ("T", c_int), ("M", c_int), ("C", c_int), ("E", c_int), ("L", c_int), ("Bs", c_int),
         ("gate_tile", c_int), ("prec", c_int), ("backend", c_int),
         ("cond_proj", c_void_p),
+        ("w_skipsum", c_void_p), ("b_skipsum", c_void_p), ("w_skipsum_inv", c_float), ("G", c_int),
     ]
 
 
diff --git a/fish_diffusion_b200/csrc/fd_api.cu b/fish_diffusion_b200/csrc/fd_api.cu
--- a/fish_diffusion_b200/csrc/fd_api.cu
+++ b/fish_diffusion_b200/csrc/fd_api.cu
@@ -50,7 +50,11 @@
 
 namespace {
 
-int run(const FdTapGemm& p, int backend, cudaStream_t st) {
+int run(const FdTapGemm& desc, int backend, cudaStream_t st) {
+  FdTapGemm p = desc;
+  if (p.w_ps == 0) p.w_ps = (long long)p.n_total * p.k_total;
+  if (p.out_rs == 0) p.out_rs = p.C;
+  if (p.out_ps == 0) p.out_ps = (long long)p.B * p.T * p.C;
   int rc;
   fd_prof_begin(p.epi * 2 + (backend == FD_BACKEND_TC ? 0 : 1), st);
   if (backend == FD_BACKEND_TC) {
@@ -138,8 +142,7 @@
 }
 
 static int wavenet_block(const uint16_t* x_planes, uint16_t* x_out_planes, const uint16_t* cond_planes,
-                         const float* cond_proj, uint16_t* z_planes, uint16_t* y_planes, const uint16_t* w1,
-                         const uint16_t* w2,
+                         uint16_t* z_planes, uint16_t* y_planes, const uint16_t* w1, const uint16_t* w2,
                          const float* gb_full, const float* gb_lo, const float* gb_hi, int gb_bstride, const float* b2,
                          float* skip_f32, uint16_t* skip_planes, float skip_scale, int B, int T, int C, int E,
                          int dilation, int gate_tile, float w1_inv_scale, float w2_inv_scale, int flags, int prec,
@@ -151,7 +154,7 @@
                          int B, int T, int C, int E, int dilation, int gate_tile, float w1_inv_scale,
                          float w2_inv_scale, int flags, int prec, int backend, void* stream) {
   FD_DEVICE_GUARD();
-  return wavenet_block(x_planes, nullptr, cond_planes, nullptr, z_planes, nullptr, w1, w2, gb_full, gb_lo, gb_hi, gb_bstride, b2,
+  return wavenet_block(x_planes, nullptr, cond_planes, z_planes, nullptr, w1, w2, gb_full, gb_lo, gb_hi, gb_bstride, b2,
                        skip_f32, skip_planes, skip_scale, B, T, C, E, dilation, gate_tile, w1_inv_scale, w2_inv_scale,
                        flags, prec, backend, stream);
 }
@@ -164,21 +167,15 @@
                                int flags, int prec, int backend, void* stream) {
   FD_DEVICE_GUARD();
   FD_REQUIRE(x_out_planes != nullptr && y_planes != nullptr, "fd_wavenet_block_fwd_train: x_out / y planes required");
-  return wavenet_block(x_planes, x_out_planes, cond_planes, nullptr, z_planes, y_planes, w1, w2, gb_full, gb_lo, gb_hi,
+  return wavenet_block(x_planes, x_out_planes, cond_planes, z_planes, y_planes, w1, w2, gb_full, gb_lo, gb_hi,
                        gb_bstride, b2, skip_f32, skip_planes, skip_scale, B, T, C, E, dilation, gate_tile, w1_inv_scale,
                        w2_inv_scale, flags, prec, backend, stream);
 }
 
-static int wavenet_block(const uint16_t* x_planes, uint16_t* x_out_planes, const uint16_t* cond_planes,
-                         const float* cond_proj, uint16_t* z_planes, uint16_t* y_planes, const uint16_t* w1,
-                         const uint16_t* w2,
-                         const float* gb_full, const float* gb_lo, const float* gb_hi, int gb_bstride, const float* b2,
-                         float* skip_f32, uint16_t* skip_planes, float skip_scale, int B, int T, int C, int E,
-                         int dilation, int gate_tile, float w1_inv_scale, float w2_inv_scale, int flags, int prec,
-                         int backend, void* stream) {
-  FD_REQUIRE(B > 0 && T > 0 && C > 0 && E > 0 && dilation > 0, "fd_wavenet_block_fwd: bad shape");
-  FD_REQUIRE(C % 8 == 0 && E % 8 == 0, "fd_wavenet_block_fwd: C=%d, E=%d must be multiples of 8", C, E);
-  cudaStream_t st = (cudaStream_t)stream;
+static int gate_gemm(const uint16_t* x_planes, const uint16_t* cond_planes, const float* cond_proj, uint16_t* z_planes,
+                     long long z_rs, long long z_ps, uint16_t* y_planes, const uint16_t* w1, const float* gb_full,
+                     const float* gb_lo, const float* gb_hi, int gb_bstride, int B, int T, int C, int E, int dilation,
+                     int gate_tile, float w1_inv_scale, int prec, int backend, cudaStream_t st) {
   FdTapGemm p;
   init_desc(p);
   p.B = B; p.T = T; set_prec(p, prec);
@@ -194,9 +191,22 @@
   p.epi = FD_EPI_GATE;
   p.gbias_full = gb_full; p.gbias_lo = gb_lo; p.gbias_hi = gb_hi; p.gbias_bstride = gb_bstride;
   p.dil = dilation; p.gate_tile = gate_tile; p.C = C;
-  p.out_planes = z_planes;
+  p.out_planes = z_planes; p.out_rs = z_rs; p.out_ps = z_ps;
   p.y_planes = y_planes;
-  int rc = run(p, backend, st);
+  return run(p, backend, st);
+}
+
+static int wavenet_block(const uint16_t* x_planes, uint16_t* x_out_planes, const uint16_t* cond_planes,
+                         uint16_t* z_planes, uint16_t* y_planes, const uint16_t* w1, const uint16_t* w2,
+                         const float* gb_full, const float* gb_lo, const float* gb_hi, int gb_bstride, const float* b2,
+                         float* skip_f32, uint16_t* skip_planes, float skip_scale, int B, int T, int C, int E,
+                         int dilation, int gate_tile, float w1_inv_scale, float w2_inv_scale, int flags, int prec,
+                         int backend, void* stream) {
+  FD_REQUIRE(B > 0 && T > 0 && C > 0 && E > 0 && dilation > 0, "fd_wavenet_block_fwd: bad shape");
+  FD_REQUIRE(C % 8 == 0 && E % 8 == 0, "fd_wavenet_block_fwd: C=%d, E=%d must be multiples of 8", C, E);
+  cudaStream_t st = (cudaStream_t)stream;
+  int rc = gate_gemm(x_planes, cond_planes, nullptr, z_planes, 0, 0, y_planes, w1, gb_full, gb_lo, gb_hi, gb_bstride,
+                     B, T, C, E, dilation, gate_tile, w1_inv_scale, prec, backend, st);
   if (rc) return rc;
   FdTapGemm q;
   init_desc(q);
@@ -212,11 +222,75 @@
   return run(q, backend, st);
 }
 
+static int wavenet_layers(const fd_wavenet_fwd_desc* d, const float* gb_full, const float* gb_lo, const float* gb_hi,
+                          cudaStream_t st) {
+  const int B = d->B, T = d->T, C = d->C, E = d->E, L = d->L, G = d->G;
+  const long long hist_rs = (long long)G * C, hist_ps = (long long)B * T * G * C;
+  const int gb_stride = d->Bs > 1 ? 2 * C : 0;
+  for (int l = 0; l < L; ++l) {
+    const int slot = l % G;
+    uint16_t* z = d->z + (size_t)slot * C;
+    const size_t go = (size_t)l * d->Bs * 2 * C;
+    const float* cp = d->cond_proj != nullptr ? d->cond_proj + (size_t)l * B * T * 2 * C : nullptr;
+    int rc = gate_gemm(d->xr, d->cond_planes, cp, z, hist_rs, hist_ps, nullptr, d->w1 + (size_t)l * d->w1_lstride,
+                       gb_full + go, gb_lo + go, gb_hi + go, gb_stride, B, T, C, E, d->dilation[l], d->gate_tile,
+                       d->w1_inv[l], d->prec, d->backend, st);
+    if (rc) return rc;
+    if (l < L - 1) {
+      FdTapGemm q;
+      init_desc(q);
+      q.B = B; q.T = T; set_prec(q, d->prec);
+      q.n_total = C; q.k_total = C; q.num_seg = 1;
+      q.seg[0] = FdSeg{0, 0, 0, C};
+      set_src(q, 0, z, C);
+      q.src_rs[0] = hist_rs; q.src_bs[0] = (long long)T * hist_rs; q.src_ps[0] = hist_ps;
+      q.w = d->w2 + (size_t)l * d->w2_lstride; q.w_ps = 2ll * C * C; q.acc_scale = d->w2_inv[l];
+      q.epi = FD_EPI_RES_SKIP;
+      q.bias = d->b2 + (size_t)l * d->b2_lstride;
+      q.x_planes = d->xr; q.C = C;
+      rc = run(q, d->backend, st);
+      if (rc) return rc;
+    }
+    if (slot == G - 1 || l == L - 1) {
+      const int g0 = l - slot;
+      const bool last = l == L - 1;
+      FdTapGemm p;
+      init_desc(p);
+      p.B = B; p.T = T; set_prec(p, d->prec);
+      p.n_total = C; p.k_total = L * C; p.num_seg = 1;
+      p.seg[0] = FdSeg{0, 0, 0, (slot + 1) * C};
+      set_src(p, 0, d->z, G * C);
+      p.w = d->w_skipsum; p.w_kshift = g0 * C; p.acc_scale = d->w_skipsum_inv;
+      p.acc_chain = C;
+      p.epi = FD_EPI_LINEAR;
+      p.bias = g0 == 0 ? d->b_skipsum : nullptr;
+      if (!(g0 == 0 && last)) { p.out_f32 = d->skip_f32; p.out_accum = g0 > 0; }
+      if (last) { p.out_planes = d->skip_planes; p.planes_scale = 1.f / sqrtf((float)L); }
+      rc = run(p, d->backend, st);
+      if (rc) return rc;
+    }
+  }
+  return 0;
+}
+
 int fd_wavenet_fwd(const fd_wavenet_fwd_desc* d, void* stream) {
   FD_DEVICE_GUARD();
   FD_REQUIRE(d != nullptr, "fd_wavenet_fwd: null descriptor");
   FD_REQUIRE(d->L >= 1 && d->L <= 64, "fd_wavenet_fwd: L=%d out of range (1..64)", d->L);
   FD_REQUIRE(d->Bs == 1 || d->Bs == d->B, "fd_wavenet_fwd: Bs=%d must be 1 or B=%d", d->Bs, d->B);
+  FD_REQUIRE(d->G >= 1 && d->G <= d->L, "fd_wavenet_fwd: z history of G=%d layers out of range (1..L=%d)", d->G, d->L);
+  FD_REQUIRE(d->B > 0 && d->T > 0 && d->C > 0 && d->C % 8 == 0 && d->E > 0 && d->E % 8 == 0,
+             "fd_wavenet_fwd: bad shape");
+  FD_REQUIRE(2ll * d->B * d->T * d->G * d->C < (1ll << 32),
+             "fd_wavenet_fwd: z history 2*B*T*G*C = %lld exceeds 32-bit element offsets",
+             2ll * d->B * d->T * d->G * d->C);
+  FD_REQUIRE(d->z != nullptr && d->xr != nullptr && d->skip_planes != nullptr,
+             "fd_wavenet_fwd: workspace xr, z (the z history) and skip_planes are required");
+  FD_REQUIRE(d->w_skipsum != nullptr && d->b_skipsum != nullptr,
+             "fd_wavenet_fwd: the skip-sum pack w_skipsum / b_skipsum is required");
+  FD_REQUIRE(d->G == d->L || d->skip_f32 != nullptr,
+             "fd_wavenet_fwd: skip_f32 is required when the z history holds fewer than L layers (G=%d, L=%d)", d->G,
+             d->L);
   const int B = d->B, T = d->T, M = d->M, C = d->C, E = d->E, L = d->L, Bs = d->Bs;
   int rc = fd_wavenet_step_mlp(d->steps, d->mlp_w0, d->mlp_b0, d->mlp_w1, d->mlp_b1, d->s, d->mlp_ws, Bs, C, stream);
   if (rc) return rc;
@@ -234,23 +308,13 @@
   cd.out_planes = d->xr; cd.Cin = M; cd.N = C; cd.w_inv_scale = d->w_in_inv; cd.act = 1;
   rc = fd_conv_cl_fwd(&cd, stream);
   if (rc) return rc;
-  const int gb_stride = Bs > 1 ? 2 * C : 0;
-  const float skip_scale = 1.f / sqrtf((float)L);
-  for (int l = 0; l < L; ++l) {
-    const int flags = (l == 0 ? 1 : 0) | (l == L - 1 ? 2 : 0);
-    const size_t go = (size_t)l * Bs * 2 * C;
-    const float* cp = d->cond_proj != nullptr ? d->cond_proj + (size_t)l * B * T * 2 * C : nullptr;
-    rc = wavenet_block(d->xr, nullptr, d->cond_planes, cp, d->z, nullptr, d->w1 + (size_t)l * d->w1_lstride,
-                       d->w2 + (size_t)l * d->w2_lstride, gb_full + go, gb_lo + go, gb_hi + go, gb_stride,
-                       d->b2 + (size_t)l * d->b2_lstride, d->skip_f32, d->skip_planes, skip_scale, B, T, C, E,
-                       d->dilation[l], d->gate_tile, d->w1_inv[l], d->w2_inv[l], flags, d->prec, d->backend, stream);
-    if (rc) return rc;
-  }
+  rc = wavenet_layers(d, gb_full, gb_lo, gb_hi, (cudaStream_t)stream);
+  if (rc) return rc;
   cd.in_planes = d->skip_planes; cd.w_planes = d->w_skip; cd.bias = d->b_skip; cd.row_mask = nullptr;
-  cd.out_planes = d->z; cd.out_f32 = nullptr; cd.Cin = C; cd.N = C; cd.w_inv_scale = d->w_skip_inv; cd.act = 1;
+  cd.out_planes = d->xr; cd.out_f32 = nullptr; cd.Cin = C; cd.N = C; cd.w_inv_scale = d->w_skip_inv; cd.act = 1;
   rc = fd_conv_cl_fwd(&cd, stream);
   if (rc) return rc;
-  cd.in_planes = d->z; cd.w_planes = d->w_out; cd.bias = d->b_out; cd.row_mask = d->x_mask;
+  cd.in_planes = d->xr; cd.w_planes = d->w_out; cd.bias = d->b_out; cd.row_mask = d->x_mask;
   cd.out_planes = nullptr; cd.out_f32 = d->out; cd.Cin = C; cd.N = M; cd.w_inv_scale = d->w_out_inv; cd.act = 0;
   return fd_conv_cl_fwd(&cd, stream);
 }
diff --git a/fish_diffusion_b200/csrc/fd_common.cuh b/fish_diffusion_b200/csrc/fd_common.cuh
--- a/fish_diffusion_b200/csrc/fd_common.cuh
+++ b/fish_diffusion_b200/csrc/fd_common.cuh
@@ -39,6 +39,7 @@
   int src_C[2];
   long long src_rs[2], src_bs[2], src_ps[2];
   const uint16_t* w;
+  long long w_ps;
   float acc_scale;
   int w_kshift;
   int epi;
@@ -52,12 +53,14 @@
   float post_scale;
   float* out_f32;
   int out_accum;
+  int acc_chain;
   uint16_t* out_planes;
   float planes_scale;
   int act;
   float act_slope;
   const uint8_t* row_mask;
 
+  long long out_rs, out_ps;
   const float* gbias_full;
   const float* gbias_lo;
   const float* gbias_hi;
@@ -332,9 +335,8 @@
     fd_store_planes<V>(p.y_planes, yplane, yoff + ng, yg8, prec);
     fd_store_planes<V>(p.y_planes, yplane, yoff + ng + half, yf8, prec);
   }
-  const size_t plane_elems = (size_t)p.B * p.T * p.C;
-  const size_t off = ((size_t)b * p.T + t) * p.C + zc0;
-  fd_store_planes<V>(p.out_planes, plane_elems, off, z, prec);
+  const size_t off = ((size_t)b * p.T + t) * p.out_rs + zc0;
+  fd_store_planes<V>(p.out_planes, (size_t)p.out_ps, off, z, prec);
 }
 
 template <int V, int PREC = -1>
diff --git a/fish_diffusion_b200/csrc/fd_tapgemm_simt.cu b/fish_diffusion_b200/csrc/fd_tapgemm_simt.cu
--- a/fish_diffusion_b200/csrc/fd_tapgemm_simt.cu
+++ b/fish_diffusion_b200/csrc/fd_tapgemm_simt.cu
@@ -42,7 +42,7 @@
 #pragma unroll
     for (int c = 0; c < 8; ++c) acc[r][c] = 0.f;
 
-  const size_t w_plane = (size_t)p.n_total * p.k_total;
+  const size_t w_plane = (size_t)p.w_ps;
   int koff = 0;
   for (int s = 0; s < p.num_seg; ++s) {
     const FdSeg sg = p.seg[s];
@@ -303,7 +303,8 @@
     return launch_run<16>(p, stream);
   }
   if (p.epi == FD_EPI_RES_SKIP) {
-    FD_REQUIRE(p.C % 4 == 0 && p.n_total == 2 * p.C, "tapgemm(simt): res/skip needs n_total == 2C");
+    FD_REQUIRE(p.C % 4 == 0 && (p.n_total == 2 * p.C || p.n_total == p.C),
+               "tapgemm(simt): res/skip needs n_total == 2C (or C: residual columns only)");
   }
   if (p.n_total >= 96) return launch_run<64>(p, stream);
   return launch_run<16>(p, stream);
diff --git a/fish_diffusion_b200/csrc/fd_tapgemm_tc.cu b/fish_diffusion_b200/csrc/fd_tapgemm_tc.cu
--- a/fish_diffusion_b200/csrc/fd_tapgemm_tc.cu
+++ b/fish_diffusion_b200/csrc/fd_tapgemm_tc.cu
@@ -18,7 +18,7 @@
   static constexpr int ROWS = PP ? 64 : BLOCK_M;
   static constexpr int A_BYTES = ROWS * BLOCK_K * 2;
   static constexpr int W_BYTES = BLOCK_N * BLOCK_K * 2;
-  static constexpr int GROUP = BLOCK_K >= 64 || PP ? 1 : 64 / BLOCK_K;
+  static constexpr int GROUP = BLOCK_K >= 64 || PP || BLOCK_N == 128 ? 1 : 64 / BLOCK_K;
   static constexpr int SUB_BYTES = NPL * (A_BYTES + W_BYTES);
   static constexpr int STAGE_BYTES = GROUP * SUB_BYTES;
   static constexpr int TX_BYTES = SUB_BYTES;
@@ -65,7 +65,7 @@
     const bool valid = t < p.T;
     const bool e_lo = t < p.dil, e_hi = t + p.dil >= p.T;
     const bool edge_any = __any_sync(0xffffffffu, valid && (e_lo || e_hi));
-    const size_t zplane = (size_t)p.B * p.T * p.C, zrow = ((size_t)b * p.T + t) * p.C + (size_t)n_tile * HALF;
+    const size_t zplane = (size_t)p.out_ps, zrow = ((size_t)b * p.T + t) * p.out_rs + (size_t)n_tile * HALF;
     const size_t yplane = (size_t)p.B * p.T * p.n_total, yrow = ((size_t)b * p.T + t) * p.n_total;
     const int halfg = p.gate_tile / 2;
 #pragma unroll
@@ -399,12 +399,14 @@
   }
 }
 
-template <int BLOCK_N, int BLOCK_K, int EPI, int PREC, int NPL>
+template <int BLOCK_N, int BLOCK_K, int EPI, int PREC, int NPL, bool CHAIN = false>
 __global__ void __launch_bounds__(FD_TC_THREADS, 1)
 fd_tapgemm_tc_kernel(const __grid_constant__ CUtensorMap tm_src0, const __grid_constant__ CUtensorMap tm_src1,
                      const __grid_constant__ CUtensorMap tm_w, const FdTapGemm p) {
   using C = Cfg<BLOCK_N, BLOCK_K, EPI, NPL>;
   static_assert(!C::PP, "GATE / RES_SKIP run the ping-pong schedule");
+  static_assert(!CHAIN || (C::GROUP == 1 && BLOCK_N <= 128), "chained accumulation: one k-block per stage, and "
+                "registers for a second accumulator");
   using MMA = Wgmma<BLOCK_N, PREC>;
   extern __shared__ uint8_t smem_raw[];
   uint8_t* smem = reinterpret_cast<uint8_t*>((reinterpret_cast<uintptr_t>(smem_raw) + 1023) & ~(uintptr_t)1023);
@@ -472,6 +474,8 @@
   const int wq = warp % 4;
   const uint32_t my_scratch = smem_u32(scratch_s) + warp * FD_TC_SCRATCH_WARP_BYTES;
   float acc[BLOCK_N / 2];
+  float sum[CHAIN ? BLOCK_N / 2 : 1];
+  const int chain_kb = CHAIN ? p.acc_chain / BLOCK_K : 0;
   int stage = 0; uint32_t phase = 0;
   long long staged_key = -1;
   for (int tile = blockIdx.x; tile < num_tiles; tile += gridDim.x) {
@@ -489,6 +493,10 @@
 
 #pragma unroll
     for (int i = 0; i < BLOCK_N / 2; ++i) acc[i] = 0.f;
+    if constexpr (CHAIN) {
+#pragma unroll
+      for (int i = 0; i < BLOCK_N / 2; ++i) sum[i] = 0.f;
+    }
     int prev_stage = -1;
     for (int kb = 0; kb < total_k_blocks; kb += C::GROUP) {
       const int nb = min(C::GROUP, total_k_blocks - kb);
@@ -520,12 +528,23 @@
       if (prev_stage >= 0 && lane == 0) mbar_arrive(&empty_bar[prev_stage]);
       prev_stage = stage;
       if (++stage == C::NUM_STAGES) { stage = 0; phase ^= 1; }
+      if constexpr (CHAIN) {
+        if ((kb + 1) % chain_kb == 0 || kb + 1 == total_k_blocks) {
+          wg_wait<0>();
+          wg_fence_operand(acc);
+          if (lane == 0) mbar_arrive(&empty_bar[prev_stage]);
+          prev_stage = -1;
+#pragma unroll
+          for (int i = 0; i < BLOCK_N / 2; ++i) { sum[i] += acc[i]; acc[i] = 0.f; }
+        }
+      }
     }
     wg_wait<0>();
     wg_fence_operand(acc);
     if (prev_stage >= 0 && lane == 0) mbar_arrive(&empty_bar[prev_stage]);
 
-    tile_epilogue<BLOCK_N, EPI, PREC>(p, acc, b, n_tile, t0 + wg * 64 + wq * 16, bias_s, my_scratch, lane);
+    tile_epilogue<BLOCK_N, EPI, PREC>(p, CHAIN ? sum : acc, b, n_tile, t0 + wg * 64 + wq * 16, bias_s, my_scratch,
+                                      lane);
   }
 }
 
@@ -705,7 +724,7 @@
   const float lg = p.gbias_lo[bo + n_g], lf = p.gbias_lo[bo + n_f];
   const float hg = p.gbias_hi[bo + n_g], hf = p.gbias_hi[bo + n_f];
   const size_t row0 = (size_t)b * p.T;
-  const size_t zplane = (size_t)p.B * p.T * p.C;
+  const size_t zplane = (size_t)p.out_ps;
   constexpr int NG = BLOCK_T / 8;
   auto load_addend = [&](int c0, float (&a)[16]) {
 #pragma unroll
@@ -755,7 +774,7 @@
       const float4 z0 = lds128(my_scratch + 4u * (lane * 8 + (sw << 2)));
       const float4 z1 = lds128(my_scratch + 4u * (lane * 8 + ((sw ^ 1u) << 2)));
       const float z[8] = {z0.x, z0.y, z0.z, z0.w, z1.x, z1.y, z1.z, z1.w};
-      fd_store_planes<8>(p.out_planes, zplane, (row0 + t) * p.C + ch, z, PREC);
+      fd_store_planes<8>(p.out_planes, zplane, (row0 + t) * p.out_rs + ch, z, PREC);
     }
     __syncwarp();
   }
@@ -921,7 +940,7 @@
   return fd_tc_launch<fd_gate_t_kernel<BLOCK_T, PREC>>(C::SMEM_BYTES, 2 * units, stream, false, 2, tmx, tmw, p);
 }
 
-template <int BLOCK_N, int BLOCK_K, int EPI, int PREC, int NPL>
+template <int BLOCK_N, int BLOCK_K, int EPI, int PREC, int NPL, bool CHAIN = false>
 int launch_inst(const FdTapGemm& p, cudaStream_t stream) {
   using C = Cfg<BLOCK_N, BLOCK_K, EPI, NPL>;
   CUtensorMap tm0, tm1, tmw;
@@ -937,15 +956,15 @@
   }
   const int m_tiles = p.B * ((p.T + C::ROWS - 1) / C::ROWS), n_tiles = p.n_total / BLOCK_N;
   if constexpr (C::PP) {
-    rc = weights_map(&tmw, p.w, p.n_total, p.k_total, BLOCK_K, NPL == 2 ? BLOCK_N : BLOCK_N / 2, 1, "tapgemm w");
+    rc = weights_map(&tmw, p.w, p.n_total, p.k_total, BLOCK_K, NPL == 2 ? BLOCK_N : BLOCK_N / 2, 1, "tapgemm w", p.w_ps);
     if (rc) return rc;
     return fd_tc_launch<fd_tapgemm_pp_kernel<BLOCK_N, BLOCK_K, EPI, PREC, NPL>>(
         C::SMEM_BYTES, 2 * ((m_tiles + 1) / 2 * n_tiles), stream, false, 2, tm0, tm1, tmw, p);
   } else {
-    rc = weights_map(&tmw, p.w, p.n_total, p.k_total, BLOCK_K, BLOCK_N, NPL, "tapgemm w");
+    rc = weights_map(&tmw, p.w, p.n_total, p.k_total, BLOCK_K, BLOCK_N, NPL, "tapgemm w", p.w_ps);
     if (rc) return rc;
-    return fd_tc_launch<fd_tapgemm_tc_kernel<BLOCK_N, BLOCK_K, EPI, PREC, NPL>>(C::SMEM_BYTES, m_tiles * n_tiles,
-                                                                              stream, false, 1, tm0, tm1, tmw, p);
+    return fd_tc_launch<fd_tapgemm_tc_kernel<BLOCK_N, BLOCK_K, EPI, PREC, NPL, CHAIN>>(
+        C::SMEM_BYTES, m_tiles * n_tiles, stream, false, 1, tm0, tm1, tmw, p);
   }
 }
 
@@ -967,6 +986,8 @@
   if (p.epi == FD_EPI_GATE_BWD) return launch_cfg<BLOCK_N, BLOCK_K, FD_EPI_GATE_BWD>(p, stream);
   return launch_cfg<BLOCK_N, BLOCK_K, FD_EPI_LINEAR>(p, stream);
 }
+
+bool chained(const FdTapGemm& p) { return p.epi == FD_EPI_LINEAR && p.acc_chain != 0 && !p.single; }
 
 void pick_cfg(const FdTapGemm& p, int* bn, int* bk) {
   *bn = 0; *bk = 0;
@@ -995,11 +1016,12 @@
   if (k == 64) {
     if (n < 64) return;
     *bn = n; *bk = p.epi == FD_EPI_RES_SKIP ? wavenet_bk(n) : 64;
+    if (chained(p)) { *bn = n >= 128 ? 128 : 64; if (*bn == 128) *bk = 32; }
   } else if (k == 32) {
-    if (p.epi != FD_EPI_LINEAR || n < 32) return;
+    if (p.epi != FD_EPI_LINEAR || n < 32 || chained(p)) return;
     *bn = n > 64 ? 64 : n; *bk = 32;
   } else {
-    if (p.epi != FD_EPI_LINEAR) return;
+    if (p.epi != FD_EPI_LINEAR || chained(p)) return;
     *bn = n > 32 ? 32 : n; *bk = 16;
   }
 }
@@ -1031,6 +1053,12 @@
     return p.prec == FD_F16 ? launch_gate_t<240, FD_F16>(p, stream) : launch_gate_t<240, FD_BF16>(p, stream);
   }
   if (bk == 64) {
+    if (chained(p)) {
+      FD_REQUIRE(p.acc_chain % 64 == 0, "tapgemm(tc): chained accumulation needs chains of whole 64-wide k-blocks "
+                 "(acc_chain=%d)", p.acc_chain);
+      return p.prec == FD_F16 ? launch_inst<64, 64, FD_EPI_LINEAR, FD_F16, 2, true>(p, stream)
+                              : launch_inst<64, 64, FD_EPI_LINEAR, FD_BF16, 2, true>(p, stream);
+    }
     if (bn == 256) return launch_epi<256, 64>(p, stream);
     if (bn == 128) return launch_epi<128, 64>(p, stream);
     if (p.epi == FD_EPI_GATE_BWD) return launch_cfg<64, 64, FD_EPI_GATE_BWD>(p, stream);
@@ -1045,6 +1073,12 @@
     return p.prec == FD_F16 ? launch_inst<256, 32, FD_EPI_RES_SKIP, FD_F16, 2>(p, stream)
                             : launch_inst<256, 32, FD_EPI_RES_SKIP, FD_BF16, 2>(p, stream);
   }
+  if (bk == 32 && chained(p)) {
+    FD_REQUIRE(p.acc_chain % 32 == 0, "tapgemm(tc): chained accumulation needs chains of whole 32-wide k-blocks "
+               "(acc_chain=%d)", p.acc_chain);
+    return p.prec == FD_F16 ? launch_inst<128, 32, FD_EPI_LINEAR, FD_F16, 2, true>(p, stream)
+                            : launch_inst<128, 32, FD_EPI_LINEAR, FD_BF16, 2, true>(p, stream);
+  }
   if (bk == 32) {
     FD_REQUIRE(p.epi == FD_EPI_LINEAR, "tapgemm(tc): BLOCK_K=32 only instantiated for the linear epilogue");
     if (bn == 64) return launch_cfg<64, 32, FD_EPI_LINEAR>(p, stream);
diff --git a/fish_diffusion_b200/csrc/fd_tc_ptx.cuh b/fish_diffusion_b200/csrc/fd_tc_ptx.cuh
--- a/fish_diffusion_b200/csrc/fd_tc_ptx.cuh
+++ b/fish_diffusion_b200/csrc/fd_tc_ptx.cuh
@@ -711,9 +711,9 @@
 }
 
 int weights_map(CUtensorMap* m, const uint16_t* ptr, int N, int K, int box_k, int box_n, int box_planes,
-                const char* what) {
+                const char* what, long long plane_stride = 0) {
   const cuuint64_t dims[3] = {(cuuint64_t)K, (cuuint64_t)N, 2};
-  const cuuint64_t strides[2] = {(cuuint64_t)K * 2, (cuuint64_t)N * K * 2};
+  const cuuint64_t strides[2] = {(cuuint64_t)K * 2, (cuuint64_t)(plane_stride != 0 ? plane_stride : (long long)N * K) * 2};
   const cuuint32_t box[3] = {(cuuint32_t)box_k, (cuuint32_t)box_n, (cuuint32_t)box_planes};
   return encode_tiled(m, ptr, 3, dims, strides, box, what);
 }
diff --git a/fish_diffusion_b200/wavenet.py b/fish_diffusion_b200/wavenet.py
--- a/fish_diffusion_b200/wavenet.py
+++ b/fish_diffusion_b200/wavenet.py
@@ -55,6 +55,15 @@
         self.diffusion_projection = LinearNorm(residual_channels, residual_channels, use_linear_bias)
         self.conditioner_projection = ConvNorm(d_encoder, 2 * residual_channels, kernel_size=1)
         self.output_projection = ConvNorm(residual_channels, 2 * residual_channels, kernel_size=1)
+
+
+Z_HISTORY_FRACTION = 8
+
+
+def z_history_layers(L: int, B: int, T: int, C: int, total_memory: int) -> int:
+    per_layer = 2 * B * T * C
+    g = min(L, (total_memory // Z_HISTORY_FRACTION) // (2 * per_layer), ((1 << 32) - 1) // per_layer)
+    return max(int(g), 1)
 
 
 def _gate_half(C: int) -> int:
@@ -220,16 +229,27 @@
         self._pack, self._pack_key = pk, key
         return pk
 
+    def _skip_sum_pack(self, pk):
+        if "w_skipsum" not in pk:
+            C = self.residual_channels
+            w = torch.cat([w2[C:, :, 0] for w2 in pk["_srcs"][2]], dim=1)
+            s = N.pow2_scale(w)
+            pk["w_skipsum"], pk["w_skipsum_inv"] = N.pack_weight(w, pk["prec"], s), 1.0 / s
+            pk["b_skipsum"] = pk["b2"][:, C:].sum(dim=0).contiguous()
+        return pk
+
     def _workspace(self, device, B, T, Bs):
         key = (str(device), B, T, Bs)
         ws = self._ws.get(key)
         if ws is None:
             C, M, L = self.residual_channels, self.mel_channels, self.n_layers
+            G = z_history_layers(L, B, T, C, torch.cuda.get_device_properties(device).total_memory)
             i16 = dict(dtype=torch.int16, device=device)
             f32 = dict(dtype=torch.float32, device=device)
             ws = {
-                "xr": torch.empty((2, B, T, C), **i16), "z": torch.empty((2, B, T, C), **i16),
-                "skip_planes": torch.empty((2, B, T, C), **i16), "skip_f32": torch.empty((B, T, C), **f32),
+                "G": G, "xr": torch.empty((2, B, T, C), **i16), "z": torch.empty((2, B, T, G * C), **i16),
+                "skip_planes": torch.empty((2, B, T, C), **i16),
+                "skip_f32": torch.empty((B, T, C), **f32) if G < L else None,
                 "s": torch.empty((Bs, C), **f32), "mlp_ws": torch.empty((Bs * 5 * C,), **f32),
                 "gb": torch.empty((3, L, Bs, 2 * C), **f32), "gb_ws": torch.empty((L * Bs * C,), **f32),
                 "steps": torch.empty((Bs,), **f32),
@@ -313,7 +333,7 @@
         _, B, T, M = x_planes.shape
         C, E, L = self.residual_channels, self.d_encoder, self.n_layers
         assert M == self.mel_channels and tuple(cond_planes.shape) == (2, B, T, E)
-        pk = self._packed(dev)
+        pk = self._skip_sum_pack(self._packed(dev))
         mma, backend = pk["mma"], pk["backend"]
         steps = steps.to(device=dev, dtype=torch.float32).reshape(-1).contiguous()
         Bs = steps.numel()
@@ -379,6 +399,8 @@
         d.b2, d.b2_lstride = N.ptr(pk["b2"]), pk["b2"].stride(0)
         d.w_skip, d.b_skip, d.w_skip_inv = N.ptr(pk["w_skip"]), N.ptr(pk["b_skip"]), pk["w_skip_inv"]
         d.w_out, d.b_out, d.w_out_inv = N.ptr(pk["w_out"]), N.ptr(pk["b_out"]), pk["w_out_inv"]
+        d.w_skipsum, d.b_skipsum, d.w_skipsum_inv = N.ptr(pk["w_skipsum"]), N.ptr(pk["b_skipsum"]), pk["w_skipsum_inv"]
+        d.G = ws["G"]
         for l in range(L):
             d.w1_inv[l], d.w2_inv[l], d.dilation[l] = pk["w1_inv"][l], pk["w2_inv"][l], pk["dil"][l]
         d.xr, d.z, d.skip_planes, d.skip_f32 = N.ptr(ws["xr"]), N.ptr(ws["z"]), N.ptr(ws["skip_planes"]), N.ptr(ws["skip_f32"])
diff --git a/include/fishdiff_b200.h b/include/fishdiff_b200.h
--- a/include/fishdiff_b200.h
+++ b/include/fishdiff_b200.h
@@ -13,7 +13,7 @@
 #define FD_PREC_SINGLE 0x10
 #define FD_BACKEND_TC 0
 #define FD_BACKEND_SIMT 1
-#define FD_ABI_VERSION 3
+#define FD_ABI_VERSION 4
 
 int fd_abi_version(void);
 const char* fd_last_error(void);
@@ -63,6 +63,8 @@
   int B, T, M, C, E, L, Bs;
   int gate_tile, prec, backend;
   float* cond_proj;
+  const uint16_t* w_skipsum; const float* b_skipsum; float w_skipsum_inv;
+  int G;
 } fd_wavenet_fwd_desc;
 int fd_wavenet_fwd(const fd_wavenet_fwd_desc* d, void* stream);
 int fd_wavenet_cond_proj(const fd_wavenet_fwd_desc* d, void* stream);
```
